# software-mansion/smelter

Hardware: NVIDIA H100
Metric: 4K composited frames/sec (16-input grid) per GPU (higher is better)
Workload: dtype f32 math on u8 planes (f16 resampler scratch)

## Files before the change

### include/smelter_b200.h

```cpp
#ifndef SMELTER_B200_H
#define SMELTER_B200_H

#include <stddef.h>
#include <stdint.h>

#ifdef __cplusplus
extern "C" {
#endif

typedef struct smr_renderer smr_renderer;

typedef enum {
    SMR_OK = 0,
    SMR_ERR_INVALID_ARGUMENT = 1,
    SMR_ERR_CUDA = 2,
    SMR_ERR_OUTPUT_NOT_REGISTERED = 3,
    SMR_ERR_SCENE = 4,
    SMR_ERR_UNSUPPORTED = 5,
    SMR_ERR_OUT_OF_MEMORY = 6,
    SMR_ERR_BUFFER_TOO_SMALL = 7
} smr_status;

typedef enum { SMR_MODE_GPU_OPTIMIZED = 0, SMR_MODE_CPU_OPTIMIZED = 1 } smr_rendering_mode;

typedef struct {
    int32_t cuda_device;
    int32_t rendering_mode;
    uint32_t max_layouts_count;
    uint64_t stream_fallback_timeout_ns;
    uint32_t framerate_num, framerate_den;
} smr_options;

typedef enum {
    SMR_COMPONENT_INPUT_STREAM = 0,
    SMR_COMPONENT_VIEW = 1,
    SMR_COMPONENT_TILES = 2,
    SMR_COMPONENT_RESCALER = 3,
    SMR_COMPONENT_SHADER = 4,
    SMR_COMPONENT_WEB_VIEW = 5,
    SMR_COMPONENT_IMAGE = 6,
    SMR_COMPONENT_TEXT = 7
} smr_component_type;

typedef struct { uint8_t r, g, b, a; } smr_rgba;
typedef struct { float top_left, top_right, bottom_right, bottom_left; } smr_border_radius;
typedef struct { float offset_x, offset_y, blur_radius; smr_rgba color; } smr_box_shadow;
typedef struct { float top, right, bottom, left; } smr_padding;
typedef struct { int32_t has_value; float value; } smr_opt_f32;

typedef enum { SMR_INTERP_LINEAR = 0, SMR_INTERP_BOUNCE = 1, SMR_INTERP_CUBIC_BEZIER = 2 } smr_interpolation_kind;
typedef struct {
    int32_t present;
    uint64_t duration_ns;
    int32_t interpolation_kind;
    double x1, y1, x2, y2;
    int32_t should_interrupt;
} smr_transition;

typedef struct {
    int32_t is_absolute;
    smr_opt_f32 width, height;
    int32_t horizontal_from_right; float horizontal_offset;
    int32_t vertical_from_bottom; float vertical_offset;
    float rotation_degrees;
} smr_position;

typedef enum { SMR_DIRECTION_ROW = 0, SMR_DIRECTION_COLUMN = 1 } smr_direction;
typedef enum { SMR_OVERFLOW_VISIBLE = 0, SMR_OVERFLOW_HIDDEN = 1, SMR_OVERFLOW_FIT = 2 } smr_overflow;
typedef enum { SMR_RESCALE_FIT = 0, SMR_RESCALE_FILL = 1 } smr_rescale_mode;
typedef enum { SMR_HALIGN_LEFT = 0, SMR_HALIGN_RIGHT = 1, SMR_HALIGN_JUSTIFIED = 2, SMR_HALIGN_CENTER = 3 } smr_horizontal_align;
typedef enum { SMR_VALIGN_TOP = 0, SMR_VALIGN_CENTER = 1, SMR_VALIGN_BOTTOM = 2, SMR_VALIGN_JUSTIFIED = 3 } smr_vertical_align;

typedef struct smr_component {
    int32_t type;
    const char *id;
    const struct smr_component *children;
    uint32_t children_len;
    const char *input_id;

    smr_position position;
    smr_transition transition;
    smr_border_radius border_radius;
    float border_width;
    smr_rgba border_color;
    const smr_box_shadow *box_shadow;
    uint32_t box_shadow_len;

    int32_t direction;
    int32_t overflow;
    smr_rgba background_color;
    smr_padding padding;

    int32_t rescale_mode;
    int32_t horizontal_align;
    int32_t vertical_align;

    smr_opt_f32 tiles_width, tiles_height;
    uint32_t tile_aspect_ratio_w, tile_aspect_ratio_h;
    float tiles_margin, tiles_padding;
} smr_component;

typedef enum {
    SMR_FRAME_PLANAR_YUV420 = 0,
    SMR_FRAME_PLANAR_YUVJ420 = 1,
    SMR_FRAME_NV12 = 2,
    SMR_FRAME_BGRA = 3,
    SMR_FRAME_ARGB = 4,
    SMR_FRAME_RGBA8 = 5,
    SMR_FRAME_PLANAR_YUV422 = 6,
    SMR_FRAME_PLANAR_YUV444 = 7,
    SMR_FRAME_UYVY422 = 8,
    SMR_FRAME_YUYV422 = 9
} smr_frame_format;

typedef enum { SMR_MEM_HOST = 0, SMR_MEM_DEVICE = 1 } smr_mem_kind;

typedef struct {
    const char *input_id;
    int32_t format;
    uint32_t width, height;
    uint64_t pts_ns;
    const void *planes[3];
    uint32_t pitch[3];
    int32_t mem_kind;
} smr_input_frame;

typedef enum {
    SMR_OUT_PLANAR_YUV420 = 0,
    SMR_OUT_PLANAR_YUV422 = 1,
    SMR_OUT_PLANAR_YUV444 = 2,
    SMR_OUT_RGBA8 = 3,
    SMR_OUT_NV12 = 4
} smr_output_format;

typedef struct {
    const char *output_id;
    void *planes[3];
    uint32_t pitch[3];
    int32_t mem_kind;
    uint32_t width, height;
    int32_t format;
    uint64_t pts_ns;
} smr_output_frame;

#define SMR_MAX_MASKS 20
typedef struct { float radius[4]; float top, left, width, height; } smr_mask;
typedef struct {
    int32_t type;
    float top, left, width, height, rotation_degrees;
    float border_radius[4];
    smr_rgba color, border_color;
    float border_width, blur_radius;
    int32_t child_index;
    float crop_top, crop_left, crop_width, crop_height;
    int32_t masks_len;
    smr_mask masks[SMR_MAX_MASKS];
} smr_render_layout;

typedef struct {
    uint64_t frames_rendered;
    uint64_t kernel_launches;
    uint64_t h2d_bytes, d2h_bytes;
    uint64_t last_render_kernel_launches;
    uint64_t last_render_direct_tiles;
} smr_stats;

typedef enum {
    SMR_KERNEL_CONVERT = 0,
    SMR_KERNEL_WEIGHTS = 1,
    SMR_KERNEL_RESAMPLE_BOX = 2,
    SMR_KERNEL_RESAMPLE_FIRST = 3,
    SMR_KERNEL_RESAMPLE_LAST = 4,
    SMR_KERNEL_COMPOSITE = 5,
    SMR_KERNEL_OUTPUT = 6,
    SMR_KERNEL_FILL = 7,
    SMR_KERNEL_RESAMPLE_FUSED = 8,
    SMR_KERNEL_CLASSES = 9
} smr_kernel_class;
typedef struct {
    double total_ms[SMR_KERNEL_CLASSES];
    uint64_t launches[SMR_KERNEL_CLASSES];
} smr_kernel_times;

smr_status smr_create(const smr_options *opts, smr_renderer **out);
void smr_destroy(smr_renderer *r);

smr_status smr_register_input(smr_renderer *r, const char *input_id);
smr_status smr_unregister_input(smr_renderer *r, const char *input_id);

smr_status smr_update_scene(smr_renderer *r, const char *output_id, uint32_t width, uint32_t height,
                            int32_t output_format, const smr_component *scene_root);
smr_status smr_unregister_output(smr_renderer *r, const char *output_id);

smr_status smr_render(smr_renderer *r, uint64_t pts_ns, const smr_input_frame *inputs, uint32_t n_inputs,
                      smr_output_frame *outputs, uint32_t n_outputs);

#define SMR_TICKS_IN_FLIGHT 4
smr_status smr_render_begin(smr_renderer *r, uint64_t pts_ns, const smr_input_frame *inputs, uint32_t n_inputs,
                            smr_output_frame *outputs, uint32_t n_outputs);
smr_status smr_render_end(smr_renderer *r);

smr_status smr_preprocess_frame(smr_renderer *r, const smr_input_frame *frame, uint32_t out_width, uint32_t out_height,
                                void *rgba, uint32_t pitch, int32_t mem_kind);

smr_status smr_premultiply_rgba8(smr_renderer *r, const smr_input_frame *frame, void *rgba, uint32_t pitch, int32_t mem_kind);

typedef enum { SMR_GLYPH_COLOR = 0, SMR_GLYPH_MASK = 1 } smr_glyph_content;
typedef struct {
    int32_t x, y;
    uint16_t width, height;
    uint16_t atlas_x, atlas_y;
    smr_rgba color;
    int32_t content;
} smr_glyph;
typedef struct { const void *data; uint32_t width, height, pitch; } smr_atlas;
smr_status smr_render_text(smr_renderer *r, uint32_t width, uint32_t height, smr_rgba background, const smr_glyph *glyphs,
                           uint32_t n_glyphs, const smr_atlas *mask_atlas, const smr_atlas *color_atlas, int32_t color_mode,
                           void *rgba, uint32_t pitch, int32_t mem_kind);

smr_status smr_debug_partition(const int32_t *dst_w, const int32_t *dst_h, uint32_t n_jobs, uint32_t max_blocks,
                               int32_t *pieces, uint32_t pieces_cap, uint32_t *n_pieces, int32_t *begin,
                               uint32_t begin_cap, uint32_t *n_blocks);

smr_status smr_debug_tile_plan(const int32_t *boxes, uint32_t n_layers, uint32_t width, uint32_t height, int32_t sorted,
                               int32_t *owner_layer, uint32_t owner_cap, uint32_t *tiles, uint32_t tiles_cap, uint32_t *n_tiles);

smr_status smr_output_plane_sizes(uint32_t width, uint32_t height, int32_t output_format, size_t sizes[3]);

void smr_component_default(int32_t type, smr_component *out);

smr_status smr_debug_layouts(smr_renderer *r, const char *output_id, uint64_t pts_ns,
                             smr_render_layout *out, uint32_t capacity, uint32_t *n_out,
                             uint32_t *root_width, uint32_t *root_height);

smr_status smr_set_layouts(smr_renderer *r, const char *output_id, uint32_t width, uint32_t height, int32_t format,
                           uint32_t root_width, uint32_t root_height, const char *const *child_ids, uint32_t n_children,
                           const smr_render_layout *layouts, uint32_t n_layouts);

smr_status smr_debug_set_inputs(smr_renderer *r, uint64_t pts_ns, const smr_input_frame *inputs, uint32_t n_inputs);

smr_status smr_comm_get_unique_id(uint8_t id[128]);
smr_status smr_comm_init(smr_renderer *r, const uint8_t id[128], int32_t rank, int32_t nranks);
#define SMR_COMM_POOLED 1u
smr_status smr_comm_broadcast_inputs(smr_renderer *r, const smr_input_frame *frames, uint32_t n,
                                     const int32_t *root_ranks);
smr_status smr_comm_exchange_inputs(smr_renderer *r, const smr_input_frame *frames, uint32_t n, const int32_t *root_ranks,
                                    const uint64_t *consumer_masks, uint32_t flags);
#define SMR_COMM_PEER_DIRECT 2u
smr_status smr_peer_pool_alloc(smr_renderer *r, size_t bytes, void **dev_ptr, uint8_t handle[64]);
smr_status smr_peer_pool_open(smr_renderer *r, const uint8_t handle[64], void **dev_ptr);
smr_status smr_peer_pool_close(smr_renderer *r, void *dev_ptr);
smr_status smr_peer_pool_free(smr_renderer *r, void *dev_ptr);
smr_status smr_comm_pull_inputs(smr_renderer *r, const smr_input_frame *frames, const smr_input_frame *peer_frames, uint32_t n,
                                const int32_t *root_ranks, const uint64_t *consumer_masks);
smr_status smr_comm_destroy(smr_renderer *r);

smr_status smr_host_register(void *ptr, size_t bytes);
smr_status smr_host_unregister(void *ptr);

smr_status smr_get_stats(smr_renderer *r, smr_stats *out);
smr_status smr_set_profiling(smr_renderer *r, int32_t enabled);
smr_status smr_get_kernel_times(smr_renderer *r, smr_kernel_times *out);
void *smr_cuda_stream(smr_renderer *r);
const char *smr_last_error(smr_renderer *r);
const char *smr_version(void);

#ifdef __cplusplus
}
#endif
#endif
```

### smelter_b200/_ffi.py

```python
import ctypes as C
import os

_HERE = os.path.dirname(os.path.abspath(__file__))
LIB_PATH = os.environ.get("SMR_LIB_PATH") or os.path.join(_HERE, "libsmelter_b200.so")

SMR_OK = 0
STATUS_NAMES = {0: "SMR_OK", 1: "SMR_ERR_INVALID_ARGUMENT", 2: "SMR_ERR_CUDA", 3: "SMR_ERR_OUTPUT_NOT_REGISTERED",
                4: "SMR_ERR_SCENE", 5: "SMR_ERR_UNSUPPORTED", 6: "SMR_ERR_OUT_OF_MEMORY", 7: "SMR_ERR_BUFFER_TOO_SMALL"}

MODE_GPU_OPTIMIZED, MODE_CPU_OPTIMIZED = 0, 1
COMPONENT_INPUT_STREAM, COMPONENT_VIEW, COMPONENT_TILES, COMPONENT_RESCALER = 0, 1, 2, 3
COMPONENT_SHADER, COMPONENT_WEB_VIEW, COMPONENT_IMAGE, COMPONENT_TEXT = 4, 5, 6, 7
FRAME_PLANAR_YUV420, FRAME_PLANAR_YUVJ420, FRAME_NV12, FRAME_BGRA, FRAME_ARGB, FRAME_RGBA8 = 0, 1, 2, 3, 4, 5
FRAME_PLANAR_YUV422, FRAME_PLANAR_YUV444, FRAME_UYVY422, FRAME_YUYV422 = 6, 7, 8, 9
MEM_HOST, MEM_DEVICE = 0, 1
OUT_PLANAR_YUV420, OUT_PLANAR_YUV422, OUT_PLANAR_YUV444, OUT_RGBA8, OUT_NV12 = 0, 1, 2, 3, 4
MAX_MASKS = 20


class Options(C.Structure):
    _fields_ = [("cuda_device", C.c_int32), ("rendering_mode", C.c_int32), ("max_layouts_count", C.c_uint32),
                ("stream_fallback_timeout_ns", C.c_uint64), ("framerate_num", C.c_uint32), ("framerate_den", C.c_uint32)]


class Rgba(C.Structure):
    _fields_ = [("r", C.c_uint8), ("g", C.c_uint8), ("b", C.c_uint8), ("a", C.c_uint8)]


class BorderRadius(C.Structure):
    _fields_ = [("top_left", C.c_float), ("top_right", C.c_float), ("bottom_right", C.c_float), ("bottom_left", C.c_float)]


class BoxShadow(C.Structure):
    _fields_ = [("offset_x", C.c_float), ("offset_y", C.c_float), ("blur_radius", C.c_float), ("color", Rgba)]


class Padding(C.Structure):
    _fields_ = [("top", C.c_float), ("right", C.c_float), ("bottom", C.c_float), ("left", C.c_float)]


class OptF32(C.Structure):
    _fields_ = [("has_value", C.c_int32), ("value", C.c_float)]


class Transition(C.Structure):
    _fields_ = [("present", C.c_int32), ("duration_ns", C.c_uint64), ("interpolation_kind", C.c_int32),
                ("x1", C.c_double), ("y1", C.c_double), ("x2", C.c_double), ("y2", C.c_double),
                ("should_interrupt", C.c_int32)]


class Position(C.Structure):
    _fields_ = [("is_absolute", C.c_int32), ("width", OptF32), ("height", OptF32),
                ("horizontal_from_right", C.c_int32), ("horizontal_offset", C.c_float),
                ("vertical_from_bottom", C.c_int32), ("vertical_offset", C.c_float),
                ("rotation_degrees", C.c_float)]


class Component(C.Structure):
    pass


Component._fields_ = [
    ("type", C.c_int32), ("id", C.c_char_p), ("children", C.POINTER(Component)), ("children_len", C.c_uint32),
    ("input_id", C.c_char_p),
    ("position", Position), ("transition", Transition), ("border_radius", BorderRadius),
    ("border_width", C.c_float), ("border_color", Rgba), ("box_shadow", C.POINTER(BoxShadow)),
    ("box_shadow_len", C.c_uint32),
    ("direction", C.c_int32), ("overflow", C.c_int32), ("background_color", Rgba), ("padding", Padding),
    ("rescale_mode", C.c_int32), ("horizontal_align", C.c_int32), ("vertical_align", C.c_int32),
    ("tiles_width", OptF32), ("tiles_height", OptF32),
    ("tile_aspect_ratio_w", C.c_uint32), ("tile_aspect_ratio_h", C.c_uint32),
    ("tiles_margin", C.c_float), ("tiles_padding", C.c_float),
]


class InputFrame(C.Structure):
    _fields_ = [("input_id", C.c_char_p), ("format", C.c_int32), ("width", C.c_uint32), ("height", C.c_uint32),
                ("pts_ns", C.c_uint64), ("planes", C.c_void_p * 3), ("pitch", C.c_uint32 * 3), ("mem_kind", C.c_int32)]


class OutputFrame(C.Structure):
    _fields_ = [("output_id", C.c_char_p), ("planes", C.c_void_p * 3), ("pitch", C.c_uint32 * 3),
                ("mem_kind", C.c_int32), ("width", C.c_uint32), ("height", C.c_uint32), ("format", C.c_int32),
                ("pts_ns", C.c_uint64)]


class Mask(C.Structure):
    _fields_ = [("radius", C.c_float * 4), ("top", C.c_float), ("left", C.c_float), ("width", C.c_float),
                ("height", C.c_float)]


class RenderLayout(C.Structure):
    _fields_ = [("type", C.c_int32), ("top", C.c_float), ("left", C.c_float), ("width", C.c_float),
                ("height", C.c_float), ("rotation_degrees", C.c_float), ("border_radius", C.c_float * 4),
                ("color", Rgba), ("border_color", Rgba), ("border_width", C.c_float), ("blur_radius", C.c_float),
                ("child_index", C.c_int32), ("crop_top", C.c_float), ("crop_left", C.c_float),
                ("crop_width", C.c_float), ("crop_height", C.c_float), ("masks_len", C.c_int32),
                ("masks", Mask * MAX_MASKS)]


class Atlas(C.Structure):
    _fields_ = [("data", C.c_void_p), ("width", C.c_uint32), ("height", C.c_uint32), ("pitch", C.c_uint32)]


GLYPH_COLOR, GLYPH_MASK = 0, 1
GLYPH_DTYPE = [("x", "<i4"), ("y", "<i4"), ("width", "<u2"), ("height", "<u2"), ("atlas_x", "<u2"), ("atlas_y", "<u2"),
               ("color", "u1", (4,)), ("content", "<i4")]


class Stats(C.Structure):
    _fields_ = [("frames_rendered", C.c_uint64), ("kernel_launches", C.c_uint64), ("h2d_bytes", C.c_uint64),
                ("d2h_bytes", C.c_uint64), ("last_render_kernel_launches", C.c_uint64), ("last_render_direct_tiles", C.c_uint64)]


KERNEL_CLASSES = ["convert", "weights", "resample_box", "resample_first", "resample_last", "composite", "output",
                  "fill", "resample_fused"]


class KernelTimes(C.Structure):
    _fields_ = [("total_ms", C.c_double * 9), ("launches", C.c_uint64 * 9)]


EXPORTS = [
    "smr_create", "smr_destroy", "smr_register_input", "smr_unregister_input", "smr_update_scene",
    "smr_unregister_output", "smr_set_layouts", "smr_render", "smr_render_begin", "smr_render_end", "smr_preprocess_frame", "smr_premultiply_rgba8", "smr_render_text", "smr_debug_partition", "smr_debug_tile_plan", "smr_output_plane_sizes",
    "smr_component_default", "smr_debug_layouts", "smr_debug_set_inputs", "smr_get_stats", "smr_set_profiling", "smr_get_kernel_times",
    "smr_comm_get_unique_id", "smr_comm_init", "smr_comm_broadcast_inputs", "smr_comm_exchange_inputs", "smr_comm_pull_inputs", "smr_peer_pool_alloc", "smr_peer_pool_open", "smr_peer_pool_close", "smr_peer_pool_free", "smr_comm_destroy", "smr_host_register", "smr_host_unregister", "smr_cuda_stream", "smr_last_error",
    "smr_version",
]

_lib = None


def lib():
    global _lib
    if _lib is not None:
        return _lib
    if not os.path.exists(LIB_PATH):
        raise ImportError(
            f"{LIB_PATH} is missing: build it with `python -m smelter_b200.build` "
            "(the H100 compositor has no CPU fallback)")
    L = C.CDLL(LIB_PATH)
    vp = C.c_void_p
    L.smr_create.argtypes = [C.POINTER(Options), C.POINTER(vp)]
    L.smr_destroy.argtypes = [vp]
    L.smr_destroy.restype = None
    L.smr_register_input.argtypes = [vp, C.c_char_p]
    L.smr_unregister_input.argtypes = [vp, C.c_char_p]
    L.smr_update_scene.argtypes = [vp, C.c_char_p, C.c_uint32, C.c_uint32, C.c_int32, C.POINTER(Component)]
    L.smr_unregister_output.argtypes = [vp, C.c_char_p]
    for f in (L.smr_render, L.smr_render_begin):
        f.argtypes = [vp, C.c_uint64, C.POINTER(InputFrame), C.c_uint32, C.POINTER(OutputFrame), C.c_uint32]
    L.smr_render_end.argtypes = [vp]
    L.smr_preprocess_frame.argtypes = [vp, C.POINTER(InputFrame), C.c_uint32, C.c_uint32, C.c_void_p, C.c_uint32, C.c_int32]
    L.smr_preprocess_frame.restype = C.c_int32
    L.smr_premultiply_rgba8.argtypes = [vp, C.POINTER(InputFrame), C.c_void_p, C.c_uint32, C.c_int32]
    L.smr_premultiply_rgba8.restype = C.c_int32
    L.smr_render_text.argtypes = [vp, C.c_uint32, C.c_uint32, Rgba, C.c_void_p, C.c_uint32, C.POINTER(Atlas), C.POINTER(Atlas),
                                  C.c_int32, C.c_void_p, C.c_uint32, C.c_int32]
    L.smr_render_text.restype = C.c_int32
    L.smr_debug_partition.argtypes = [C.POINTER(C.c_int32), C.POINTER(C.c_int32), C.c_uint32, C.c_uint32, C.POINTER(C.c_int32),
                                      C.c_uint32, C.POINTER(C.c_uint32), C.POINTER(C.c_int32), C.c_uint32, C.POINTER(C.c_uint32)]
    L.smr_debug_partition.restype = C.c_int32
    L.smr_debug_tile_plan.argtypes = [C.POINTER(C.c_int32), C.c_uint32, C.c_uint32, C.c_uint32, C.c_int32, C.POINTER(C.c_int32), C.c_uint32,
                                      C.POINTER(C.c_uint32), C.c_uint32, C.POINTER(C.c_uint32)]
    L.smr_debug_tile_plan.restype = C.c_int32
    L.smr_output_plane_sizes.argtypes = [C.c_uint32, C.c_uint32, C.c_int32, C.POINTER(C.c_size_t * 3)]
    L.smr_component_default.argtypes = [C.c_int32, C.POINTER(Component)]
    L.smr_component_default.restype = None
    L.smr_debug_layouts.argtypes = [vp, C.c_char_p, C.c_uint64, C.POINTER(RenderLayout), C.c_uint32,
                                    C.POINTER(C.c_uint32), C.POINTER(C.c_uint32), C.POINTER(C.c_uint32)]
    L.smr_debug_set_inputs.argtypes = [vp, C.c_uint64, C.POINTER(InputFrame), C.c_uint32]
    L.smr_get_stats.argtypes = [vp, C.POINTER(Stats)]
    L.smr_comm_get_unique_id.argtypes = [C.POINTER(C.c_uint8 * 128)]
    L.smr_comm_init.argtypes = [vp, C.POINTER(C.c_uint8 * 128), C.c_int32, C.c_int32]
    L.smr_comm_broadcast_inputs.argtypes = [vp, C.POINTER(InputFrame), C.c_uint32, C.POINTER(C.c_int32)]
    L.smr_set_layouts.argtypes = [vp, C.c_char_p, C.c_uint32, C.c_uint32, C.c_int32, C.c_uint32, C.c_uint32,
                                  C.POINTER(C.c_char_p), C.c_uint32, C.POINTER(RenderLayout), C.c_uint32]
    L.smr_host_register.argtypes = [C.c_void_p, C.c_size_t]
    L.smr_host_unregister.argtypes = [C.c_void_p]
    L.smr_comm_exchange_inputs.argtypes = [vp, C.POINTER(InputFrame), C.c_uint32, C.POINTER(C.c_int32), C.POINTER(C.c_uint64),
                                           C.c_uint32]
    L.smr_comm_pull_inputs.argtypes = [vp, C.POINTER(InputFrame), C.POINTER(InputFrame), C.c_uint32, C.POINTER(C.c_int32),
                                       C.POINTER(C.c_uint64)]
    L.smr_peer_pool_alloc.argtypes = [vp, C.c_size_t, C.POINTER(C.c_void_p), C.POINTER(C.c_uint8 * 64)]
    L.smr_peer_pool_open.argtypes = [vp, C.POINTER(C.c_uint8 * 64), C.POINTER(C.c_void_p)]
    L.smr_peer_pool_close.argtypes = [vp, C.c_void_p]
    L.smr_peer_pool_free.argtypes = [vp, C.c_void_p]
    L.smr_comm_destroy.argtypes = [vp]
    L.smr_set_profiling.argtypes = [vp, C.c_int32]
    L.smr_get_kernel_times.argtypes = [vp, C.POINTER(KernelTimes)]
    L.smr_cuda_stream.argtypes = [vp]
    L.smr_cuda_stream.restype = vp
    L.smr_last_error.argtypes = [vp]
    L.smr_last_error.restype = C.c_char_p
    L.smr_version.restype = C.c_char_p
    _lib = L
    return L
```

### smelter_b200/build.py

```python
import os
import subprocess
import sys

HERE = os.path.dirname(os.path.abspath(__file__))
CSRC = os.path.join(HERE, "csrc")
LIB = os.path.join(HERE, "libsmelter_b200.so")
SOURCES = ["kernels.cu", "renderer.cpp", "scene.cpp"]
HEADERS = ["kernels.h", "scene.h", "ptx_helpers.cuh", "resample_tma.cuh", "resample_tma3.cuh", "resample_tma0.cuh", os.path.join("..", "..", "include", "smelter_b200.h")]

NVCC_FLAGS = [
    "-std=c++17", "-O3",
    "-gencode", "arch=compute_90a,code=sm_90a",
    "-lineinfo",
    "-fmad=false",
    "-prec-div=true", "-prec-sqrt=true", "-ftz=false",
    "-Xcompiler", "-fPIC,-ffp-contract=off,-Wall",
    "-ccbin", "/usr/bin/g++",
    "-shared",
]


def needs_build():
    if not os.path.exists(LIB):
        return True
    t = os.path.getmtime(LIB)
    deps = [os.path.join(CSRC, s) for s in SOURCES + HEADERS] + [os.path.abspath(__file__)]
    return any(os.path.getmtime(d) > t for d in deps)


def build(force=False, verbose=False, extra=()):
    if not force and not needs_build():
        return LIB
    nvcc = os.environ.get("NVCC", "/usr/local/cuda/bin/nvcc")
    cmd = [nvcc] + NVCC_FLAGS + list(extra) + ["-o", LIB] + [os.path.join(CSRC, s) for s in SOURCES]
    if verbose:
        print(" ".join(cmd))
    subprocess.check_call(cmd)
    return LIB


if __name__ == "__main__":
    build(force=True, verbose=True, extra=sys.argv[1:])
    print(LIB)
```

### smelter_b200/csrc/kernels.cu

```cuda
#include <cuda_fp16.h>
#include <cuda_runtime.h>

#include <cstdio>
#include <cstdlib>
#include <atomic>
#include <cstring>

#include "kernels.h"

namespace smr {
namespace dev {

#include "ptx_helpers.cuh"

__device__ float c_u8n[256];
__device__ float c_dec[256];
__device__ float c_thr[256];
#define ENC_KEY0 ((127 - 13) << 5)
#define ENC_KEYS ((13 << 5) + 1)
__device__ unsigned char c_enc0[420];
__device__ float c_yl[256];
#define ENC1_KEY0 ((127 - 13) << 8)
#define ENC1_KEYS ((13 << 8) + 1)
__device__ unsigned char c_enc1[ENC1_KEYS + 3];

static thread_local char g_err[256] = {0};
const char *last_launch_error() { return g_err; }
static bool check_launch(const char *what) {
    cudaError_t e = cudaGetLastError();
    if (e != cudaSuccess) {
        snprintf(g_err, sizeof(g_err), "%s: %s", what, cudaGetErrorString(e));
        return false;
    }
    return true;
}

void upload_tables(const float *u8n, const float *dec, const float *thr) {
    float t[256];
    for (int i = 0; i < 255; i++) t[i] = thr[i];
    t[255] = 3.0e38f;
    cudaMemcpyToSymbol(c_u8n, u8n, sizeof(float) * 256);
    cudaMemcpyToSymbol(c_dec, dec, sizeof(float) * 256);
    cudaMemcpyToSymbol(c_thr, t, sizeof(float) * 256);
    float yl[256];
    for (int i = 0; i < 256; i++) {
        volatile float d = u8n[i] - (16.0f / 255.0f);
        volatile float m = d * (1.0f / 0.85882352941f);
        yl[i] = m < 0.0f ? 0.0f : (m > 1.0f ? 1.0f : m);
    }
    cudaMemcpyToSymbol(c_yl, yl, sizeof(float) * 256);
    unsigned char enc0[420] = {0};
    for (int k = 0; k < ENC_KEYS; k++) {
        const uint32_t bits = (uint32_t)(k + ENC_KEY0) << 18;
        float lo;
        memcpy(&lo, &bits, 4);
        int e = 0;
        while (e < 255 && lo >= t[e]) e++;
        enc0[k] = (unsigned char)e;
    }
    cudaMemcpyToSymbol(c_enc0, enc0, sizeof(enc0));
    static unsigned char enc1[ENC1_KEYS + 3];
    for (int k = 0; k < ENC1_KEYS; k++) {
        const uint32_t bits = (uint32_t)(k + ENC1_KEY0) << 15;
        float lo;
        memcpy(&lo, &bits, 4);
        int e = 0;
        while (e < 255 && lo >= t[e]) e++;
        enc1[k] = (unsigned char)e;
        if (k > 0 && enc1[k] - enc1[k - 1] > 1) {
            fprintf(stderr, "smelter_b200: sRGB encode bucket table is too coarse at key %d\n", k);
            abort();
        }
    }
    cudaMemcpyToSymbol(c_enc1, enc1, sizeof(enc1));
}

struct Tables {
    float u8n[256];
    float dec[256];
    float thr[256];
    float yl[256];
};

__device__ __forceinline__ void load_tables(Tables &t) {
    for (int i = threadIdx.y * blockDim.x + threadIdx.x; i < 256; i += blockDim.x * blockDim.y) {
        t.u8n[i] = c_u8n[i];
        t.dec[i] = c_dec[i];
        t.thr[i] = c_thr[i];
        t.yl[i] = c_yl[i];
    }
    __syncthreads();
}

__device__ __forceinline__ float clamp01(float x) { return __saturatef(x); }

__device__ __forceinline__ int unorm8(float x) { return __float2int_rn(clamp01(x) * 255.0f); }

__device__ __forceinline__ int srgb_encode(const Tables &t, float lin) {
    const float x = clamp01(lin);
    const int k = max((__float_as_int(x) >> 15) - ENC1_KEY0, 0);
    const int e = __ldg(c_enc1 + k);
    return e + (x >= t.thr[e] ? 1 : 0);
}

struct LinTap {
    int i0, i1;
    float f;
};

__device__ __forceinline__ LinTap linear_tap(float t, int dim) {
    LinTap r;
    float c = t * (float)dim - 0.5f;
    if (!(c == c)) { r.i0 = r.i1 = 0; r.f = 0.0f; return r; }
    c = fminf(fmaxf(c, -2.0f), (float)dim + 1.0f);
    float fl = floorf(c);
    float f = c - fl;
    r.f = rintf(f * 256.0f) * (1.0f / 256.0f);
    int i0 = (int)fl, i1 = i0 + 1;
    r.i0 = min(max(i0, 0), dim - 1);
    r.i1 = min(max(i1, 0), dim - 1);
    return r;
}

__device__ __forceinline__ float bilerp(float t00, float t10, float t01, float t11, float fx, float fy) {
    float h0 = fmaf(t10, fx, t00 * (1.0f - fx));
    float h1 = fmaf(t11, fx, t01 * (1.0f - fx));
    return fmaf(h1, fy, h0 * (1.0f - fy));
}

__device__ __forceinline__ float div255(float nf, float pow2) {
    const float c = __uint_as_float(0x3b808081u) * pow2, lo = __uint_as_float(0xaf7efeffu) * pow2;
    return fmaf(nf, c, nf * lo);
}
__device__ __forceinline__ float filter_u8(int t00, int t10, int t01, int t11, float fx, float fy) {
    const int wx = (int)(fx * 256.0f), wy = (int)(fy * 256.0f);
    const int n = (t00 * (256 - wx) + t10 * wx) * (256 - wy) + (t01 * (256 - wx) + t11 * wx) * wy;
    return div255((float)n, 1.0f / 65536.0f);
}

__device__ __forceinline__ float sample_plane(const Tables &T, const uint8_t *p, int pitch, int stride, int ch,
                                              const LinTap &ax, const LinTap &ay) {
    const uint8_t *r0 = p + (size_t)ay.i0 * pitch, *r1 = p + (size_t)ay.i1 * pitch;
    const int t00 = __ldg(r0 + ax.i0 * stride + ch), t10 = __ldg(r0 + ax.i1 * stride + ch);
    const int t01 = __ldg(r1 + ax.i0 * stride + ch), t11 = __ldg(r1 + ax.i1 * stride + ch);
    return filter_u8(t00, t10, t01, t11, ax.f, ay.f);
}

#define K16 (16.0f / 255.0f)
#define RCP_Y (1.0f / 0.85882352941f)
#define RCP_C (1.0f / 0.87843137254f)

__device__ __forceinline__ uchar4 yuv_to_rgba8(float y, float u, float v, int full_range) {
    if (!full_range) {
        y = clamp01((y - K16) * RCP_Y);
        u = clamp01((u - K16) * RCP_C);
        v = clamp01((v - K16) * RCP_C);
    }
    float um = u - 0.5f, vm = v - 0.5f;
    float r = fmaf(1.5748f, vm, y);
    float g = fmaf(-0.4681f, vm, fmaf(-0.1873f, um, y));
    float b = fmaf(1.8556f, um, y);
    return make_uchar4((unsigned char)unorm8(r), (unsigned char)unorm8(g), (unsigned char)unorm8(b), 255);
}

__device__ __forceinline__ void yuv_to_rgb8i(float y, float u, float v, int full_range, int &r8, int &g8, int &b8) {
    if (!full_range) {
        y = clamp01((y - K16) * RCP_Y);
        u = clamp01((u - K16) * RCP_C);
        v = clamp01((v - K16) * RCP_C);
    }
    float um = u - 0.5f, vm = v - 0.5f;
    r8 = unorm8(fmaf(1.5748f, vm, y));
    g8 = unorm8(fmaf(-0.4681f, vm, fmaf(-0.1873f, um, y)));
    b8 = unorm8(fmaf(1.8556f, um, y));
}

__device__ __forceinline__ void yuv_to_rgb8n(float yn, float u, float v, int full_range, int &r8, int &g8, int &b8) {
    if (!full_range) {
        u = clamp01((u - K16) * RCP_C);
        v = clamp01((v - K16) * RCP_C);
    }
    float um = u - 0.5f, vm = v - 0.5f;
    r8 = unorm8(fmaf(1.5748f, vm, yn));
    g8 = unorm8(fmaf(-0.4681f, vm, fmaf(-0.1873f, um, yn)));
    b8 = unorm8(fmaf(1.8556f, um, yn));
}

__device__ __forceinline__ uchar4 node_texel(const Tables &T, const Tex &s, int x, int y) {
    switch (s.kind) {
        case TEX_RGBA8:
            return __ldg(reinterpret_cast<const uchar4 *>(s.p0 + (size_t)y * s.pitch0) + x);
        case TEX_BGRA: {
            uchar4 v = __ldg(reinterpret_cast<const uchar4 *>(s.p0 + (size_t)y * s.pitch0) + x);
            return make_uchar4(v.z, v.y, v.x, v.w);
        }
        case TEX_ARGB: {
            uchar4 v = __ldg(reinterpret_cast<const uchar4 *>(s.p0 + (size_t)y * s.pitch0) + x);
            return make_uchar4(v.y, v.z, v.w, v.x);
        }
        case TEX_YUV420:
        case TEX_NV12: {
            int cw = s.width / 2, ch = s.height / 2;
            if (((s.width | s.height) & 1) == 0) {
                int x0 = (x & 1) ? (x >> 1) : max((x >> 1) - 1, 0), x1 = (x & 1) ? min((x >> 1) + 1, cw - 1) : (x >> 1);
                int y0 = (y & 1) ? (y >> 1) : max((y >> 1) - 1, 0), y1 = (y & 1) ? min((y >> 1) + 1, ch - 1) : (y >> 1);
                const int kx = (x & 1) ? 1 : 3, ky = (y & 1) ? 1 : 3;
                float yy = T.u8n[__ldg(s.p0 + (size_t)y * s.pitch0 + x)];
                int nu, nv;
                if (s.kind == TEX_YUV420) {
                    const uint8_t *u0 = s.p1 + (size_t)y0 * s.pitch1, *u1 = s.p1 + (size_t)y1 * s.pitch1;
                    const uint8_t *v0 = s.p2 + (size_t)y0 * s.pitch2, *v1 = s.p2 + (size_t)y1 * s.pitch2;
                    nu = ((int)__ldg(u0 + x0) * (4 - kx) + (int)__ldg(u0 + x1) * kx) * (4 - ky) +
                         ((int)__ldg(u1 + x0) * (4 - kx) + (int)__ldg(u1 + x1) * kx) * ky;
                    nv = ((int)__ldg(v0 + x0) * (4 - kx) + (int)__ldg(v0 + x1) * kx) * (4 - ky) +
                         ((int)__ldg(v1 + x0) * (4 - kx) + (int)__ldg(v1 + x1) * kx) * ky;
                } else {
                    const uchar2 *r0 = reinterpret_cast<const uchar2 *>(s.p1 + (size_t)y0 * s.pitch1);
                    const uchar2 *r1 = reinterpret_cast<const uchar2 *>(s.p1 + (size_t)y1 * s.pitch1);
                    uchar2 a = __ldg(r0 + x0), b = __ldg(r0 + x1), c = __ldg(r1 + x0), d = __ldg(r1 + x1);
                    nu = ((int)a.x * (4 - kx) + (int)b.x * kx) * (4 - ky) + ((int)c.x * (4 - kx) + (int)d.x * kx) * ky;
                    nv = ((int)a.y * (4 - kx) + (int)b.y * kx) * (4 - ky) + ((int)c.y * (4 - kx) + (int)d.y * kx) * ky;
                }
                const float uu = div255((float)nu, 0.0625f), vv = div255((float)nv, 0.0625f);
                return yuv_to_rgba8(yy, uu, vv, s.full_range);
            }
            float tx = ((float)x + 0.5f) / (float)s.width, ty = ((float)y + 0.5f) / (float)s.height;
            LinTap ax = linear_tap(tx, s.width), ay = linear_tap(ty, s.height);
            LinTap cx = linear_tap(tx, cw), cy = linear_tap(ty, ch);
            float yy = sample_plane(T, s.p0, s.pitch0, 1, 0, ax, ay);
            float uu, vv;
            if (s.kind == TEX_YUV420) {
                uu = sample_plane(T, s.p1, s.pitch1, 1, 0, cx, cy);
                vv = sample_plane(T, s.p2, s.pitch2, 1, 0, cx, cy);
            } else {
                uu = sample_plane(T, s.p1, s.pitch1, 2, 0, cx, cy);
                vv = sample_plane(T, s.p1, s.pitch1, 2, 1, cx, cy);
            }
            return yuv_to_rgba8(yy, uu, vv, s.full_range);
        }
        case TEX_YUV422:
        case TEX_YUV444: {
            const int cw = s.kind == TEX_YUV444 ? s.width : s.width / 2, ch = s.height;
            float tx = ((float)x + 0.5f) / (float)s.width, ty = ((float)y + 0.5f) / (float)s.height;
            LinTap ax = linear_tap(tx, s.width), ay = linear_tap(ty, s.height);
            LinTap cx = linear_tap(tx, cw), cy = linear_tap(ty, ch);
            float yy = sample_plane(T, s.p0, s.pitch0, 1, 0, ax, ay);
            float uu = sample_plane(T, s.p1, s.pitch1, 1, 0, cx, cy);
            float vv = sample_plane(T, s.p2, s.pitch2, 1, 0, cx, cy);
            return yuv_to_rgba8(yy, uu, vv, 0);
        }
        case TEX_UYVY:
        case TEX_YUYV: {
            const int dimx = s.width / 2;
            const float eps = 0.0001f, hpw = 0.5f / (float)dimx;
            float tx = ((float)x + 0.5f) / (float)s.width, ty = ((float)y + 0.5f) / (float)s.height;
            float xf = ((tx * (float)dimx - hpw) + eps) * 2.0f;
            unsigned x_pos = xf >= 4294967296.0f ? 0xffffffffu : (xf > 0.0f ? (unsigned)xf : 0u);
            float tcx = (float)(x_pos / 2u) / (float)dimx + hpw;
            LinTap ax = linear_tap(tcx, dimx), ay = linear_tap(ty, s.height);
            float t[4];
#pragma unroll
            for (int c = 0; c < 4; c++) t[c] = sample_plane(T, s.p0, s.pitch0, 4, c, ax, ay);
            const bool second = x_pos & 1u;
            if (s.kind == TEX_YUYV) return yuv_to_rgba8(second ? t[2] : t[0], t[1], t[3], 0);
            return yuv_to_rgba8(second ? t[3] : t[1], t[0], t[2], 0);
        }
        default:
            return make_uchar4(0, 0, 0, 0);
    }
}

__device__ __forceinline__ bool yuv_quad_ok(const Tex &s, int x, int y) {
    return (s.kind == TEX_NV12 || s.kind == TEX_YUV420) && (((s.width | s.height | x | y) & 1) == 0) && x >= 2 &&
           x + 3 <= s.width - 1 && y >= 2 && y + 3 <= s.height - 1;
}
__device__ __forceinline__ void yuv_quad(const Tables &T, const Tex &s, int x, int y, uchar4 &p00, uchar4 &p10,
                                         uchar4 &p01, uchar4 &p11) {
    const int cx = x >> 1, cy = y >> 1;
    unsigned he[3], ho[3];
#pragma unroll
    for (int i = 0; i < 3; i++) {
        unsigned a, b, d;
        if (s.kind == TEX_NV12) {
            const uchar2 *rp = reinterpret_cast<const uchar2 *>(s.p1 + (size_t)(cy - 1 + i) * s.pitch1) + cx;
            const uchar2 ta = __ldg(rp - 1), tb = __ldg(rp), td = __ldg(rp + 1);
            a = ta.x | (ta.y << 16); b = tb.x | (tb.y << 16); d = td.x | (td.y << 16);
        } else {
            const uint8_t *ru = s.p1 + (size_t)(cy - 1 + i) * s.pitch1 + cx, *rv = s.p2 + (size_t)(cy - 1 + i) * s.pitch2 + cx;
            a = __ldg(ru - 1) | (__ldg(rv - 1) << 16); b = __ldg(ru) | (__ldg(rv) << 16); d = __ldg(ru + 1) | (__ldg(rv + 1) << 16);
        }
        he[i] = a + 3u * b;
        ho[i] = 3u * b + d;
    }
    const uchar2 y0 = __ldg(reinterpret_cast<const uchar2 *>(s.p0 + (size_t)y * s.pitch0 + x));
    const uchar2 y1 = __ldg(reinterpret_cast<const uchar2 *>(s.p0 + (size_t)(y + 1) * s.pitch0 + x));
    const unsigned n00 = he[0] + 3u * he[1], n10 = ho[0] + 3u * ho[1], n01 = 3u * he[1] + he[2], n11 = 3u * ho[1] + ho[2];
    p00 = yuv_to_rgba8(T.u8n[y0.x], div255((float)(n00 & 0xffffu), 0.0625f), div255((float)(n00 >> 16), 0.0625f), s.full_range);
    p10 = yuv_to_rgba8(T.u8n[y0.y], div255((float)(n10 & 0xffffu), 0.0625f), div255((float)(n10 >> 16), 0.0625f), s.full_range);
    p01 = yuv_to_rgba8(T.u8n[y1.x], div255((float)(n01 & 0xffffu), 0.0625f), div255((float)(n01 >> 16), 0.0625f), s.full_range);
    p11 = yuv_to_rgba8(T.u8n[y1.y], div255((float)(n11 & 0xffffu), 0.0625f), div255((float)(n11 >> 16), 0.0625f), s.full_range);
}

__global__ void __launch_bounds__(256) k_convert(Tex src, uint8_t *dst, int dst_pitch) {
    __shared__ Tables T;
    load_tables(T);
    int x = blockIdx.x * blockDim.x + threadIdx.x, y = blockIdx.y * blockDim.y + threadIdx.y;
    if (x >= src.width || y >= src.height) return;
    reinterpret_cast<uchar4 *>(dst + (size_t)y * dst_pitch)[x] = node_texel(T, src, x, y);
}

int launch_convert_to_rgba(const Tex &src, uint8_t *dst, int dst_pitch, Stream s) {
    dim3 b(32, 8), g((src.width + 31) / 32, (src.height + 7) / 8);
    k_convert<<<g, b, 0, (cudaStream_t)s>>>(src, dst, dst_pitch);
    return check_launch("k_convert") ? 1 : -1;
}

#define PI_F 3.14159265359f

__device__ __forceinline__ float sin_cr(float x) { return (float)sin((double)x); }
__device__ __forceinline__ float cos_cr(float x) { return (float)cos((double)x); }

__global__ void k_weights(const WeightJob *jobs) {
    const WeightJob J = jobs[blockIdx.y];
    int o = blockIdx.x * blockDim.x + threadIdx.x;
    if (o >= J.n_out) return;
    float kernel_scale = fmaxf(J.scale, 1.0f);
    float inv_k = 1.0f / kernel_scale;
    float support = 3.0f * kernel_scale;
    float center = (J.offset + ((float)o + 0.5f) * J.scale) - 0.5f;
    float first = ceilf(center - support);
    float x0 = (first - center) * inv_k;
    float s1 = sin_cr(PI_F * x0), c1 = cos_cr(PI_F * x0);
    float s3 = sin_cr(PI_F * x0 / 3.0f), c3 = cos_cr(PI_F * x0 / 3.0f);
    float sd1 = sin_cr(PI_F * inv_k), cd1 = cos_cr(PI_F * inv_k);
    float sd3 = sin_cr(PI_F * inv_k / 3.0f), cd3 = cos_cr(PI_F * inv_k / 3.0f);
    const float pi2 = PI_F * PI_F;
    float wsum = 0.0f;
    float *w = J.weights + (size_t)o * J.taps;
    for (int t = 0; t < J.taps; t++) {
        float x = x0 + (float)t * inv_k;
        float wt = 0.0f;
        if (fabsf(x) < 1e-5f) wt = 1.0f;
        else if (fabsf(x) < 3.0f) wt = ((3.0f * s1) * s3) / ((pi2 * x) * x);
        w[t] = wt;
        wsum += wt;
        float ns1 = s1 * cd1 + c1 * sd1;
        c1 = c1 * cd1 - s1 * sd1;
        s1 = ns1;
        float ns3 = s3 * cd3 + c3 * sd3;
        c3 = c3 * cd3 - s3 * sd3;
        s3 = ns3;
    }
    J.inv_wsum[o] = 1.0f / wsum;
    float fc = fminf(fmaxf(first, -1.0e9f), 1.0e9f);
    J.first[o] = (int)fc;
}

int launch_weights(const WeightJob *jobs_dev, const WeightJob *jobs_host, int n, Stream s) {
    if (n <= 0) return 0;
    int max_out = 1;
    for (int i = 0; i < n; i++) max_out = jobs_host[i].n_out > max_out ? jobs_host[i].n_out : max_out;
    dim3 b(128), g((max_out + 127) / 128, n);
    k_weights<<<g, b, 0, (cudaStream_t)s>>>(jobs_dev);
    return check_launch("k_weights") ? 1 : -1;
}

__device__ __forceinline__ float4 rs_load(const Tables &T, const Tex &s, int x, int y) {
    if (s.kind == TEX_F16) {
        const uint2 raw = __ldg(reinterpret_cast<const uint2 *>(s.p0 + (size_t)y * s.pitch0) + x);
        __half2 a = *reinterpret_cast<const __half2 *>(&raw.x), b = *reinterpret_cast<const __half2 *>(&raw.y);
        float2 fa = __half22float2(a), fb = __half22float2(b);
        return make_float4(fa.x, fa.y, fb.x, fb.y);
    }
    uchar4 p = node_texel(T, s, x, y);
    return make_float4(T.dec[p.x], T.dec[p.y], T.dec[p.z], T.u8n[p.w]);
}

__device__ __forceinline__ void rs_store(const Tables &T, const ResampleJob &J, int x, int y, float4 r) {
    if (J.dst_f16) {
        __half2 a = __floats2half2_rn(r.x, r.y), b = __floats2half2_rn(r.z, r.w);
        uint2 raw;
        raw.x = *reinterpret_cast<unsigned int *>(&a);
        raw.y = *reinterpret_cast<unsigned int *>(&b);
        reinterpret_cast<uint2 *>(J.dst + (size_t)y * J.dst_pitch)[x] = raw;
    } else {
        uchar4 o = make_uchar4((unsigned char)srgb_encode(T, r.x), (unsigned char)srgb_encode(T, r.y),
                               (unsigned char)srgb_encode(T, r.z), (unsigned char)unorm8(r.w));
        reinterpret_cast<uchar4 *>(J.dst + (size_t)y * J.dst_pitch)[x] = o;
    }
}

__global__ void __launch_bounds__(256) k_resample(const ResampleJob *jobs) {
    __shared__ Tables T;
    load_tables(T);
    const ResampleJob &J = jobs[blockIdx.z];
    int px = blockIdx.x * blockDim.x + threadIdx.x, py = blockIdx.y * blockDim.y + threadIdx.y;
    if (px >= J.dst_w || py >= J.dst_h) return;
    const Tex &S = J.src;
    if (J.box_fx * J.box_fy > 1) {
        float4 sum = make_float4(0.f, 0.f, 0.f, 0.f);
        for (int dy = 0; dy < J.box_fy; dy++)
            for (int dx = 0; dx < J.box_fx; dx++) {
                int sx = min(px * J.box_fx + dx, S.width - 1), sy = min(py * J.box_fy + dy, S.height - 1);
                float4 t = rs_load(T, S, sx, sy);
                sum.x += t.x; sum.y += t.y; sum.z += t.z; sum.w += t.w;
            }
        float d = (float)((unsigned)J.box_fx * (unsigned)J.box_fy);
        rs_store(T, J, px, py, make_float4(sum.x / d, sum.y / d, sum.z / d, sum.w / d));
        return;
    }
    int o = J.axis == 1 ? py : px;
    int max_src = (J.axis == 1 ? S.height : S.width) - 1;
    int max_perp = (J.axis == 1 ? S.width : S.height) - 1;
    int perp = min(max((J.axis == 1 ? px : py) + J.perp_offset, 0), max_perp);
    const float *w = J.weights + (size_t)o * J.taps;
    int first = __ldg(J.first + o);
    float4 sum = make_float4(0.f, 0.f, 0.f, 0.f);
    for (int t = 0; t < J.taps; t++) {
        float wt = __ldg(w + t);
        if (wt == 0.0f) continue;
        int src = min(max(first + t, 0), max_src);
        float4 tx = J.axis == 1 ? rs_load(T, S, perp, src) : rs_load(T, S, src, perp);
        sum.x = fmaf(tx.x, wt, sum.x);
        sum.y = fmaf(tx.y, wt, sum.y);
        sum.z = fmaf(tx.z, wt, sum.z);
        sum.w = fmaf(tx.w, wt, sum.w);
    }
    float inv = __ldg(J.inv_wsum + o);
    rs_store(T, J, px, py, make_float4(sum.x * inv, sum.y * inv, sum.z * inv, sum.w * inv));
}

int launch_resample(const ResampleJob *jobs_dev, const ResampleJob *jobs_host, int n, Stream s) {
    if (n <= 0) return 0;
    int mw = 1, mh = 1;
    for (int i = 0; i < n; i++) {
        mw = jobs_host[i].dst_w > mw ? jobs_host[i].dst_w : mw;
        mh = jobs_host[i].dst_h > mh ? jobs_host[i].dst_h : mh;
    }
    dim3 b(32, 8), g((mw + 31) / 32, (mh + 7) / 8, n);
    k_resample<<<g, b, 0, (cudaStream_t)s>>>(jobs_dev);
    return check_launch("k_resample") ? 1 : -1;
}

#define W64_TW 64
#define W64_WARPS 8
#define W64_RING 64

__constant__ float c_wint[5][32];
__constant__ float c_winv[5];
__constant__ float2 c_wpair[5][32];

void set_int_weights(int S, const float *weights_dev, const float *inv_dev, int taps, Stream s) {
    cudaMemcpyToSymbolAsync(c_wint, weights_dev, sizeof(float) * taps, sizeof(float) * 32 * S, cudaMemcpyDeviceToDevice, (cudaStream_t)s);
    cudaMemcpyToSymbolAsync(c_winv, inv_dev, sizeof(float), sizeof(float) * S, cudaMemcpyDeviceToDevice, (cudaStream_t)s);
    float *pair = nullptr;
    cudaGetSymbolAddress((void **)&pair, c_wpair);
    pair += 2 * 32 * S;
    cudaMemsetAsync(pair, 0, sizeof(float2) * 32, (cudaStream_t)s);
    cudaMemcpy2DAsync(pair, sizeof(float2), weights_dev, sizeof(float), sizeof(float), taps, cudaMemcpyDeviceToDevice, (cudaStream_t)s);
    if (taps > S)
        cudaMemcpy2DAsync(pair + 2 * S + 1, sizeof(float2), weights_dev, sizeof(float), sizeof(float), taps - S,
                          cudaMemcpyDeviceToDevice, (cudaStream_t)s);
}

template <int S>
struct W64 {
    static constexpr int SS = S == 0 ? 4 : S;
    static constexpr int TAPS = 6 * SS + 1;
    static constexpr int SPAN = (W64_TW - 1) * SS + TAPS + 3;
    static constexpr int ROWLEN = S == 0 ? ((SPAN + 2 + 7) & ~7) : (((SPAN + SPAN / (2 * SS) + 2) + 7) & ~7);
    struct Smem {
        Tables T;
        __half2 ring[W64_RING][3][W64_TW / 2];
        float4 srow[W64_WARPS][ROWLEN];
        float hw[S == 0 ? TAPS * W64_TW : 1];
    };
    static __device__ __forceinline__ int pos(int i) { return S == 0 ? i : i + i / (2 * SS); }
};

__device__ __forceinline__ void prefetch_l2_span(const uint8_t *p, int bytes, const uint8_t *lo, const uint8_t *hi) {
    unsigned long long a = (unsigned long long)(p < lo ? lo : p), e = (unsigned long long)(p + bytes < hi ? p + bytes : hi);
    a = (a + 15ull) & ~15ull;
    if (e <= a + 16ull) return;
    const unsigned size = (unsigned)((e - a) & ~15ull);
    asm volatile("cp.async.bulk.prefetch.L2.global [%0], %1;" ::"l"(a), "r"(size) : "memory");
}

template <int S, int SRC>
__global__ void __launch_bounds__(32 * W64_WARPS, 3) k_resample_fused_int(const FusedJob *jobs, const FusedPiece *pieces,
                                                                            const int *piece_begin) {
    constexpr bool NV12 = SRC == 1, IL = SRC >= 2;
    using K = W64<S>;
    constexpr int TAPS = K::TAPS;
    constexpr int WIN = S + TAPS;
    extern __shared__ __align__(16) unsigned char fs_raw[];
    typename K::Smem &M = *reinterpret_cast<typename K::Smem *>(fs_raw);
    load_tables(M.T);
    const int lane = threadIdx.x, warp = threadIdx.y;
    for (int pi = __ldg(piece_begin + blockIdx.x); pi < __ldg(piece_begin + blockIdx.x + 1); pi++) {
    const FusedPiece P = pieces[pi];
    const FusedJob &J = jobs[P.job];
    const int th = S == 0 ? J.taps_h : TAPS;
    const int ox0 = P.strip * W64_TW;
    const int oy_begin = P.oy_begin, oy_end = P.oy_end;
    const Tex &src = J.src;
    const int W = src.width, H = src.height, chei = H >> 1;
    const int tv = J.taps_v;
    const int xa = __ldg(J.first_h + ox0);
    const int xa_e = xa & ~1;
    const int d0 = xa - xa_e;
    const int oc0 = min(ox0 + 2 * lane, J.dst_w - 1), oc1 = min(ox0 + 2 * lane + 1, J.dst_w - 1);
    int gi0 = 0, gD = 0, npairs_g = 0;
    float inv0, inv1;
    if constexpr (S == 0) {
        const int f0 = __ldg(J.first_h + oc0), f1 = __ldg(J.first_h + oc1);
        gi0 = f0 - xa_e; gD = f1 - f0;
        inv0 = __ldg(J.inv_h + oc0); inv1 = __ldg(J.inv_h + oc1);
        const int o_last = min(ox0 + W64_TW - 1, J.dst_w - 1);
        npairs_g = (min(__ldg(J.first_h + o_last) + th - xa_e, K::SPAN) + 1) >> 1;
        for (int t = warp; t < th; t += W64_WARPS) {
            M.hw[t * W64_TW + 2 * lane] = __ldg(J.w_h + (size_t)oc0 * th + t);
            M.hw[t * W64_TW + 2 * lane + 1] = __ldg(J.w_h + (size_t)oc1 * th + t);
        }
        __syncthreads();
    } else {
        inv0 = inv1 = c_winv[S];
    }
    constexpr int NP = ((W64_TW - 1) * K::SS + TAPS + 2) >> 1, NIT = (NP + 31) / 32;
    const int npairs = S == 0 ? npairs_g : NP;
    const int full_range = src.full_range;
    const float *ytab = full_range ? M.T.u8n : M.T.yl;
    const int p_in_lo = IL ? (xa_e >= 0 ? 0 : (1 - xa_e) >> 1) : (xa_e >= 2 ? 0 : (2 - xa_e + 1) >> 1);
    const int p_in_hi = IL ? (W - 2 - xa_e) >> 1 : (W - 4 - xa_e) >> 1;
    const int p_hi = min(p_in_hi, npairs - 1);
    const int dsh = S == 0 ? 0 : d0;

    int produced_hi = -0x40000000;
    for (int o0 = oy_begin; o0 < oy_end; o0 += W64_WARPS) {
        const int o_l = min(o0 + W64_WARPS - 1, oy_end - 1);
        const int need_lo = min(max(__ldg(J.first_v + o0), 0), H - 1);
        const int need_hi = min(max(__ldg(J.first_v + o_l) + tv - 1, 0), H - 1);
        const int start = max(produced_hi + 1, need_lo);
        {
            const int tid = warp * 32 + lane;
            const int nr = need_hi + 1 + (tid >> 2), part = tid & 3;
            if (tid < 128 && nr < H) {
                const int xb = max(xa_e - 2, 0), span = K::SPAN + 4;
                if (IL) {
                    if (part == 0) prefetch_l2_span(src.p0 + (size_t)nr * src.pitch0 + 2 * xb, 2 * span, src.p0, src.p0 + (size_t)H * src.pitch0);
                } else if (part == 0) {
                    prefetch_l2_span(src.p0 + (size_t)nr * src.pitch0 + xb, span, src.p0, src.p0 + (size_t)H * src.pitch0);
                } else if ((nr & 1) == 0) {
                    const int cyn = min(nr >> 1, chei - 1);
                    if (NV12) {
                        if (part == 1) prefetch_l2_span(src.p1 + (size_t)cyn * src.pitch1 + xb, span, src.p1, src.p1 + (size_t)chei * src.pitch1);
                    } else if (part == 1) {
                        prefetch_l2_span(src.p1 + (size_t)cyn * src.pitch1 + (xb >> 1), span >> 1, src.p1, src.p1 + (size_t)chei * src.pitch1);
                    } else if (part == 2) {
                        prefetch_l2_span(src.p2 + (size_t)cyn * src.pitch2 + (xb >> 1), span >> 1, src.p2, src.p2 + (size_t)chei * src.pitch2);
                    }
                }
            }
        }
        for (int r = start + warp; r <= need_hi; r += W64_WARPS) {
            float4 *row = M.srow[warp];
            {
                const uint8_t *yrow = src.p0 + (size_t)r * src.pitch0;
                const int cy0 = (r & 1) ? (r >> 1) : max((r >> 1) - 1, 0), cy1 = (r & 1) ? min((r >> 1) + 1, chei - 1) : (r >> 1);
                const uint8_t *c0a = IL ? nullptr : src.p1 + (size_t)cy0 * src.pitch1, *c1a = IL ? nullptr : src.p1 + (size_t)cy1 * src.pitch1;
                const uint8_t *c0b = (NV12 || IL) ? nullptr : src.p2 + (size_t)cy0 * src.pitch2;
                const uint8_t *c1b = (NV12 || IL) ? nullptr : src.p2 + (size_t)cy1 * src.pitch2;
                const bool odd = r & 1;
                struct Raw { unsigned y, a0, b0, d0, a1, b1, d1; };
                auto load_raw = [&](int pp, Raw &R) {
                    const int x = xa_e + 2 * pp, cx = x >> 1;
                    if (IL) {
                        R.y = __ldg(reinterpret_cast<const unsigned int *>(yrow) + cx);
                        return;
                    }
                    if (NV12) {
                        const unsigned short *r0 = reinterpret_cast<const unsigned short *>(c0a) + cx;
                        const unsigned short *r1 = reinterpret_cast<const unsigned short *>(c1a) + cx;
                        R.a0 = __ldg(r0 - 1); R.b0 = __ldg(r0); R.d0 = __ldg(r0 + 1);
                        R.a1 = __ldg(r1 - 1); R.b1 = __ldg(r1); R.d1 = __ldg(r1 + 1);
                    } else {
                        R.a0 = __ldg(c0a + cx - 1) | ((unsigned)__ldg(c0b + cx - 1) << 16);
                        R.b0 = __ldg(c0a + cx) | ((unsigned)__ldg(c0b + cx) << 16);
                        R.d0 = __ldg(c0a + cx + 1) | ((unsigned)__ldg(c0b + cx + 1) << 16);
                        R.a1 = __ldg(c1a + cx - 1) | ((unsigned)__ldg(c1b + cx - 1) << 16);
                        R.b1 = __ldg(c1a + cx) | ((unsigned)__ldg(c1b + cx) << 16);
                        R.d1 = __ldg(c1a + cx + 1) | ((unsigned)__ldg(c1b + cx + 1) << 16);
                    }
                    R.y = __ldg(reinterpret_cast<const unsigned short *>(yrow + x));
                };
                auto spread = [&](unsigned c) { return NV12 ? __byte_perm(c, 0, 0x4140) : c; };
                auto put = [&](int i, int r8, int g8, int b8) {
                    row[K::pos(i)] = make_float4(M.T.dec[r8], M.T.dec[g8], M.T.dec[b8], 0.0f);
                };
                auto convert_store = [&](const Raw &R, int p) {
                    if constexpr (IL) {
                        const unsigned t = R.y;
                        const unsigned ub = SRC == 2 ? (t & 0xffu) : ((t >> 8) & 0xffu), vb = SRC == 2 ? ((t >> 16) & 0xffu) : (t >> 24);
                        const unsigned y0 = SRC == 2 ? ((t >> 8) & 0xffu) : (t & 0xffu), y1 = SRC == 2 ? (t >> 24) : ((t >> 16) & 0xffu);
                        const float u = M.T.u8n[ub], v = M.T.u8n[vb];
                        const int i = 2 * p - dsh;
                        int r8, g8, b8;
                        yuv_to_rgb8n(M.T.yl[y0], u, v, 0, r8, g8, b8);
                        if (i >= 0) put(i, r8, g8, b8);
                        yuv_to_rgb8n(M.T.yl[y1], u, v, 0, r8, g8, b8);
                        put(i + 1, r8, g8, b8);
                        return;
                    }
                    const unsigned a0 = spread(R.a0), b0 = 3u * spread(R.b0), e0 = spread(R.d0);
                    const unsigned a1 = spread(R.a1), b1 = 3u * spread(R.b1), e1 = spread(R.d1);
                    const unsigned he0 = a0 + b0, ho0 = b0 + e0, he1 = a1 + b1, ho1 = b1 + e1;
                    const unsigned ne = odd ? 3u * he0 + he1 : he0 + 3u * he1;
                    const unsigned no = odd ? 3u * ho0 + ho1 : ho0 + 3u * ho1;
                    const float ue = div255((float)(ne & 0xffffu), 0.0625f), ve = div255((float)(ne >> 16), 0.0625f);
                    const float uo = div255((float)(no & 0xffffu), 0.0625f), vo = div255((float)(no >> 16), 0.0625f);
                    const int i = 2 * p - dsh;
                    int r8, g8, b8;
                    auto luma = [&](unsigned yb) {
                        const float yn = div255((float)yb, 1.0f);
                        return full_range ? yn : clamp01((yn - K16) * RCP_Y);
                    };
                    yuv_to_rgb8n(luma(R.y & 0xffu), ue, ve, full_range, r8, g8, b8);
                    if (i >= 0) put(i, r8, g8, b8);
                    yuv_to_rgb8n(luma(R.y >> 8), uo, vo, full_range, r8, g8, b8);
                    put(i + 1, r8, g8, b8);
                };
                auto inside = [&](int pp) { return pp >= p_in_lo && pp <= p_hi; };
                auto border = [&](int p) {
                    const int x = xa_e + 2 * p, i = 2 * p - dsh;
                    const uchar4 pe = node_texel(M.T, src, min(max(x, 0), W - 1), r);
                    const uchar4 po = node_texel(M.T, src, min(max(x + 1, 0), W - 1), r);
                    if (i >= 0) put(i, pe.x, pe.y, pe.z);
                    put(i + 1, po.x, po.y, po.z);
                };
                Raw cur, nxt;
                bool ok = inside(lane);
                if (ok) load_raw(lane, cur);
                if constexpr (S != 0) {
#pragma unroll
                    for (int it = 0; it < NIT; it++) {
                        const int p = lane + 32 * it;
                        const bool ok_n = it + 1 < NIT && inside(p + 32);
                        if (ok_n) load_raw(p + 32, nxt);
                        if (ok) convert_store(cur, p);
                        cur = nxt; ok = ok_n;
                    }
                } else {
                    for (int p = lane; p < npairs; p += 32) {
                        const bool ok_n = inside(p + 32);
                        if (ok_n) load_raw(p + 32, nxt);
                        if (ok) convert_store(cur, p);
                        cur = nxt; ok = ok_n;
                    }
                }
                if (p_in_lo > 0 || p_hi < npairs - 1)
                    for (int p = lane; p < npairs; p += 32)
                        if (!inside(p)) border(p);
            }
            __syncwarp();
            {
                __half2 *ringrow = &M.ring[r & (W64_RING - 1)][0][0];
                float r0 = 0.f, g0 = 0.f, b0 = 0.f, r1 = 0.f, g1 = 0.f, b1 = 0.f;
                if constexpr (S == 0) {
                    const float *w0 = M.hw + 2 * lane, *w1 = M.hw + 2 * lane + 1 - gD * W64_TW;
                    const int win = th + gD;
                    const float4 *sp = row + gi0;
#pragma unroll 4
                    for (int j = 0; j < win; j++) {
                        const float4 v = sp[j];
                        if (j < th) { const float w = w0[j * W64_TW]; r0 = fmaf(v.x, w, r0); g0 = fmaf(v.y, w, g0); b0 = fmaf(v.z, w, b0); }
                        if (j >= gD) { const float w = w1[j * W64_TW]; r1 = fmaf(v.x, w, r1); g1 = fmaf(v.y, w, g1); b1 = fmaf(v.z, w, b1); }
                    }
                } else {
                    const float4 *sp = row + (2 * S + 1) * lane;
#pragma unroll
                    for (int j = 0; j < WIN; j++) {
                        const float4 v = sp[K::pos(j)];
                        if (j < TAPS) { const float w = c_wint[S][j]; r0 = fmaf(v.x, w, r0); g0 = fmaf(v.y, w, g0); b0 = fmaf(v.z, w, b0); }
                        if (j >= S) { const float w = c_wint[S][j - S]; r1 = fmaf(v.x, w, r1); g1 = fmaf(v.y, w, g1); b1 = fmaf(v.z, w, b1); }
                    }
                }
                ringrow[lane] = __floats2half2_rn(r0 * inv0, r1 * inv1);
                ringrow[W64_TW / 2 + lane] = __floats2half2_rn(g0 * inv0, g1 * inv1);
                ringrow[W64_TW + lane] = __floats2half2_rn(b0 * inv0, b1 * inv1);
            }
            __syncwarp();
        }
        produced_hi = max(produced_hi, need_hi);
        __syncthreads();
        const int oy = o0 + warp;
        if (oy < oy_end) {
            const int fv = __ldg(J.first_v + oy);
            const float *wv = J.w_v + (size_t)oy * tv;
            float r0 = 0.f, g0 = 0.f, b0 = 0.f, r1 = 0.f, g1 = 0.f, b1 = 0.f;
            const bool inside = fv >= 0 && fv + tv - 1 <= H - 1;
            for (int t = 0; t < tv; t++) {
                const float wt = __ldg(wv + t);
                const int row = inside ? fv + t : min(max(fv + t, 0), H - 1);
                const __half2 *p = &M.ring[row & (W64_RING - 1)][0][0];
                const float2 vr = __half22float2(p[lane]), vg = __half22float2(p[W64_TW / 2 + lane]), vb = __half22float2(p[W64_TW + lane]);
                r0 = fmaf(vr.x, wt, r0); r1 = fmaf(vr.y, wt, r1);
                g0 = fmaf(vg.x, wt, g0); g1 = fmaf(vg.y, wt, g1);
                b0 = fmaf(vb.x, wt, b0); b1 = fmaf(vb.y, wt, b1);
            }
            const float inv_v = __ldg(J.inv_v + oy);
            const int ox = ox0 + 2 * lane;
            uchar4 oa = make_uchar4((unsigned char)srgb_encode(M.T, r0 * inv_v), (unsigned char)srgb_encode(M.T, g0 * inv_v),
                                    (unsigned char)srgb_encode(M.T, b0 * inv_v), 255);
            uchar4 ob = make_uchar4((unsigned char)srgb_encode(M.T, r1 * inv_v), (unsigned char)srgb_encode(M.T, g1 * inv_v),
                                    (unsigned char)srgb_encode(M.T, b1 * inv_v), 255);
            uchar4 *drow = reinterpret_cast<uchar4 *>(J.dst + (size_t)oy * J.dst_pitch);
            if (ox + 1 < J.dst_w && (J.dst_pitch & 7) == 0) {
                uint2 pk;
                pk.x = *reinterpret_cast<unsigned int *>(&oa);
                pk.y = *reinterpret_cast<unsigned int *>(&ob);
                *reinterpret_cast<uint2 *>(drow + ox) = pk;
            } else {
                if (ox < J.dst_w) drow[ox] = oa;
                if (ox + 1 < J.dst_w) drow[ox + 1] = ob;
            }
        }
        __syncthreads();
    }
    }
}

template <int S, int SRC>
static bool launch_fused_int(const FusedJob *jobs_dev, const FusedPiece *pieces, const int *piece_begin, int nblocks,
                             cudaStream_t s) {
    static std::atomic<unsigned long long> done{0};
    int dev = 0;
    cudaGetDevice(&dev);
    const unsigned long long bit = 1ull << (dev & 63);
    if (!(done.load(std::memory_order_acquire) & bit)) {
        cudaFuncSetAttribute(k_resample_fused_int<S, SRC>, cudaFuncAttributeMaxDynamicSharedMemorySize,
                             (int)sizeof(typename W64<S>::Smem));
        done.fetch_or(bit, std::memory_order_release);
    }
    k_resample_fused_int<S, SRC><<<nblocks, dim3(32, W64_WARPS), sizeof(typename W64<S>::Smem), s>>>(jobs_dev, pieces, piece_begin);
    return check_launch("k_resample_fused_int");
}

template <int S>
static bool launch_fused_src(int src, const FusedJob *jobs_dev, const FusedPiece *pieces_dev, const int *piece_begin_dev,
                             int nblocks, cudaStream_t st) {
    switch (src) {
        case 0: return launch_fused_int<S, 0>(jobs_dev, pieces_dev, piece_begin_dev, nblocks, st);
        case 1: return launch_fused_int<S, 1>(jobs_dev, pieces_dev, piece_begin_dev, nblocks, st);
        case 2: return launch_fused_int<S, 2>(jobs_dev, pieces_dev, piece_begin_dev, nblocks, st);
        default: return launch_fused_int<S, 3>(jobs_dev, pieces_dev, piece_begin_dev, nblocks, st);
    }
}

}
}
namespace smr {
namespace dev {
__device__ __forceinline__ float to_y(float r, float g, float b) {
    float y = fmaf(b, 0.0722f, fmaf(g, 0.7152f, r * 0.2126f));
    return fmaf(y, 0.85882352941f, K16);
}
__device__ __forceinline__ float to_u(float r, float g, float b) {
    float u = fmaf(b, 0.5f, fmaf(g, -0.3854f, r * -0.1146f));
    return fmaf(u + 0.5f, 0.87843137254f, K16);
}
__device__ __forceinline__ float to_v(float r, float g, float b) {
    float v = fmaf(b, -0.0458f, fmaf(g, -0.4542f, r * 0.5f));
    return fmaf(v + 0.5f, 0.87843137254f, K16);
}

__device__ __forceinline__ void emit_yuv_2x2(const FusedJob &J, int X, int Y, uint32_t p00, uint32_t p10, uint32_t p01, uint32_t p11) {
    using namespace tma;
    const float2 m23 = splat(-8388608.0f);
    const float2 c = splat(__uint_as_float(0x3b808081u)), lo = splat(__uint_as_float(0xaf7efeffu));
    auto pairf = [&](uint32_t a, uint32_t b, uint32_t sel) {
        return add2(make_float2(__uint_as_float(__byte_perm(a, 0x4B000000u, sel)), __uint_as_float(__byte_perm(b, 0x4B000000u, sel))), m23);
    };
    auto unit = [&](float2 n) { return fma2(n, c, mul2(n, lo)); };
    auto store2 = [&](float2 x01) -> uint32_t {
        const float2 q = add2_after_mul(mul2(x01, splat(255.0f)), splat(12582912.0f));
        return (__float_as_uint(q.x) & 0xffu) | ((__float_as_uint(q.y) & 0xffu) << 8);
    };
    auto lum2 = [&](uint32_t a, uint32_t b) -> uint32_t {
        const float2 r = unit(pairf(a, b, 0x7540u)), g = unit(pairf(a, b, 0x7541u)), bl = unit(pairf(a, b, 0x7542u));
        const float2 y = fma2(bl, splat(0.0722f), fma2(g, splat(0.7152f), mul2(r, splat(0.2126f))));
        return store2(make_float2(__saturatef(fmaf(y.x, 0.85882352941f, K16)), __saturatef(fmaf(y.y, 0.85882352941f, K16))));
    };
    *reinterpret_cast<unsigned short *>(J.out0 + (size_t)Y * J.out_pitch0 + X) = (unsigned short)lum2(p00, p10);
    *reinterpret_cast<unsigned short *>(J.out0 + (size_t)(Y + 1) * J.out_pitch0 + X) = (unsigned short)lum2(p01, p11);
    const uint32_t m = 0x00ff00ffu;
    const uint32_t srb = (p00 & m) + (p10 & m) + (p01 & m) + (p11 & m);
    const uint32_t sga = ((p00 >> 8) & m) + ((p10 >> 8) & m) + ((p01 >> 8) & m) + ((p11 >> 8) & m);
    const float2 c4 = splat(__uint_as_float(0x3b808081u) * 0.25f), lo4 = splat(__uint_as_float(0xaf7efeffu) * 0.25f);
    const float2 nrg = add2(make_float2(__uint_as_float(__byte_perm(srb, 0x4B000000u, 0x7610u)), __uint_as_float(__byte_perm(sga, 0x4B000000u, 0x7610u))), m23);
    const float nb = __uint_as_float(__byte_perm(srb, 0x4B000000u, 0x7632u)) - 8388608.0f;
    const float2 rg = fma2(nrg, c4, mul2(nrg, lo4));
    const float b = fmaf(nb, c4.x, nb * lo4.x);
    float2 uv = mul2(splat(rg.x), make_float2(-0.1146f, 0.5f));
    uv = fma2(splat(rg.y), make_float2(-0.3854f, -0.4542f), uv);
    uv = fma2(splat(b), make_float2(0.5f, -0.0458f), uv);
    uv = add2(uv, splat(0.5f));
    const uint32_t cuv = store2(make_float2(__saturatef(fmaf(uv.x, 0.87843137254f, K16)), __saturatef(fmaf(uv.y, 0.87843137254f, K16))));
    if (J.out_format == 4) {
        *reinterpret_cast<unsigned short *>(J.out1 + (size_t)(Y >> 1) * J.out_pitch1 + X) = (unsigned short)cuv;
    } else {
        J.out1[(size_t)(Y >> 1) * J.out_pitch1 + (X >> 1)] = (unsigned char)(cuv & 0xffu);
        J.out2[(size_t)(Y >> 1) * J.out_pitch2 + (X >> 1)] = (unsigned char)(cuv >> 8);
    }
}

#include "resample_tma.cuh"
#include "resample_tma3.cuh"
#include "resample_tma0.cuh"

template <int SRC, int WINP, int BOX>
static bool launch_tma0(const FusedJob *jobs_dev, const FusedPiece *pieces, const int *piece_begin, int nblocks, cudaStream_t s) {
    static std::atomic<unsigned long long> done{0};
    int dev = 0;
    cudaGetDevice(&dev);
    const unsigned long long bit = 1ull << (dev & 63);
    if (!(done.load(std::memory_order_acquire) & bit)) {
        cudaFuncSetAttribute(tma_any::k_resample_tma0<SRC, WINP, BOX>, cudaFuncAttributeMaxDynamicSharedMemorySize, tma_any::Cfg::SMEM);
        done.fetch_or(bit, std::memory_order_release);
    }
    const int grid = (nblocks + tma_any::kGroups - 1) / tma_any::kGroups;
    tma_any::k_resample_tma0<SRC, WINP, BOX><<<grid, dim3(32, tma::kWarps * tma_any::kGroups), tma_any::Cfg::SMEM, s>>>(jobs_dev, pieces, piece_begin, nblocks);
    return check_launch("k_resample_tma0");
}

template <int WINP>
static bool launch_tma0_src(int src, int box, const FusedJob *jobs_dev, const FusedPiece *pieces, const int *piece_begin, int nblocks,
                            cudaStream_t s) {
    if (box) return src == 1 ? launch_tma0<1, WINP, 1>(jobs_dev, pieces, piece_begin, nblocks, s)
                             : launch_tma0<0, WINP, 1>(jobs_dev, pieces, piece_begin, nblocks, s);
    return src == 1 ? launch_tma0<1, WINP, 0>(jobs_dev, pieces, piece_begin, nblocks, s)
                    : launch_tma0<0, WINP, 0>(jobs_dev, pieces, piece_begin, nblocks, s);
}

template <int S, int SRC>
static bool launch_tma3(const FusedJob *jobs_dev, const FusedPiece *pieces, const int *piece_begin, int nblocks, cudaStream_t s) {
    static std::atomic<unsigned long long> done{0};
    int dev = 0;
    cudaGetDevice(&dev);
    const unsigned long long bit = 1ull << (dev & 63);
    if (!(done.load(std::memory_order_acquire) & bit)) {
        cudaFuncSetAttribute(tma_int::k_resample_tma3<S, SRC>, cudaFuncAttributeMaxDynamicSharedMemorySize, tma_int::Cfg<S>::SMEM);
        done.fetch_or(bit, std::memory_order_release);
    }
    const int grid = (nblocks + tma_int::kGroups - 1) / tma_int::kGroups;
    tma_int::k_resample_tma3<S, SRC><<<grid, dim3(32, tma::kWarps * tma_int::kGroups), tma_int::Cfg<S>::SMEM, s>>>(jobs_dev, pieces, piece_begin, nblocks);
    return check_launch("k_resample_tma3");
}

int launch_resample_fused(const FusedKernel &k, int src, const FusedJob *jobs_dev, const FusedPiece *pieces_dev,
                          const int *piece_begin_dev, int nblocks, Stream s) {
    if (nblocks <= 0) return 0;
    cudaStream_t st = (cudaStream_t)s;
    bool ok = false;
    static_assert(tma_int::Cfg<4>::NOUT == kTmaStripCols4 && tma_int::Cfg<2>::NOUT == kTmaStripCols2 &&
                  tma_int::Cfg<4>::RROWS == kTmaRing4 && tma_int::Cfg<2>::RROWS == kTmaRing2, "integer-ratio kernel");
    static_assert(tma_any::kGroups == kTma0Groups && tma_any::Cfg::MAXT == kTma0MaxTaps && tma_any::Cfg::WINP_MAX == kTma0Window[3] &&
                  tma_any::Cfg::RROWS == kTmaRing4, "any-ratio kernel");
    static_assert(tma::kLumaBox == 2 * kTmaLumaBoxW && tma::kChunkRows == kTmaLumaBoxH && tma::kNv12Box == 2 * kTmaNv12BoxW &&
                  tma::kPlanarBox == kTmaPlanarBoxW && tma::kChromaRows == kTmaChromaBoxH, "TMA boxes");
    switch (k.kind) {
        case FusedKernel::TMA_ANY:
            switch (k.window) {
                case 0: ok = launch_tma0_src<kTma0Window[0]>(src, k.box, jobs_dev, pieces_dev, piece_begin_dev, nblocks, st); break;
                case 1: ok = launch_tma0_src<kTma0Window[1]>(src, k.box, jobs_dev, pieces_dev, piece_begin_dev, nblocks, st); break;
                case 2: ok = launch_tma0_src<kTma0Window[2]>(src, k.box, jobs_dev, pieces_dev, piece_begin_dev, nblocks, st); break;
                default: ok = launch_tma0_src<kTma0Window[3]>(src, k.box, jobs_dev, pieces_dev, piece_begin_dev, nblocks, st); break;
            }
            break;
        case FusedKernel::TMA_INT:
            if (k.ratio == 4) ok = src == 1 ? launch_tma3<4, 1>(jobs_dev, pieces_dev, piece_begin_dev, nblocks, st)
                                            : launch_tma3<4, 0>(jobs_dev, pieces_dev, piece_begin_dev, nblocks, st);
            else ok = src == 1 ? launch_tma3<2, 1>(jobs_dev, pieces_dev, piece_begin_dev, nblocks, st)
                               : launch_tma3<2, 0>(jobs_dev, pieces_dev, piece_begin_dev, nblocks, st);
            break;
        default:
            switch (k.ratio) {
                case 2: ok = launch_fused_src<2>(src, jobs_dev, pieces_dev, piece_begin_dev, nblocks, st); break;
                case 3: ok = launch_fused_src<3>(src, jobs_dev, pieces_dev, piece_begin_dev, nblocks, st); break;
                case 4: ok = launch_fused_src<4>(src, jobs_dev, pieces_dev, piece_begin_dev, nblocks, st); break;
                default: ok = launch_fused_src<0>(src, jobs_dev, pieces_dev, piece_begin_dev, nblocks, st); break;
            }
    }
    return ok ? 1 : -1;
}

__device__ __forceinline__ void half_row_convert(const uint32_t (&yw)[2], const uint32_t (&v)[6], float nk16, float rcp_y, float rcp_c,
                                                 int (&sums)[4][3]) {
#pragma unroll
    for (int p = 0; p < 4; p++) {
        float2 qr, qg, qb;
        tma::convert_pair(yw, v, p, nk16, rcp_y, rcp_c, qr, qg, qb);
        sums[p][0] += (int)(__float_as_uint(qr.x) & 0xffu) + (int)(__float_as_uint(qr.y) & 0xffu);
        sums[p][1] += (int)(__float_as_uint(qg.x) & 0xffu) + (int)(__float_as_uint(qg.y) & 0xffu);
        sums[p][2] += (int)(__float_as_uint(qb.x) & 0xffu) + (int)(__float_as_uint(qb.y) & 0xffu);
    }
}

template <bool NV12>
__device__ __forceinline__ void half_row_sums(const Tex &S, int x0, int r, float nk16, float rcp_y, float rcp_c, int (&sums)[4][3]) {
    const uint8_t *yrow = S.p0 + (size_t)r * S.pitch0 + x0;
    const uint32_t yw[2] = {__ldg(reinterpret_cast<const uint32_t *>(yrow)), __ldg(reinterpret_cast<const uint32_t *>(yrow) + 1)};
    const int ch = r >> 1, cl = (r & 1) ? ch + 1 : ch - 1, cx = x0 >> 1;
    uint32_t v[6];
#pragma unroll
    for (int k = 0; k < 6; k++) {
        uint32_t h, l;
        if (NV12) {
            const uint32_t th = __ldg(reinterpret_cast<const unsigned short *>(S.p1 + (size_t)ch * S.pitch1) + (cx - 1 + k));
            const uint32_t tl = __ldg(reinterpret_cast<const unsigned short *>(S.p1 + (size_t)cl * S.pitch1) + (cx - 1 + k));
            h = __byte_perm(th, 0, 0x4140); l = __byte_perm(tl, 0, 0x4140);
        } else {
            h = __ldg(S.p1 + (size_t)ch * S.pitch1 + cx - 1 + k) | ((uint32_t)__ldg(S.p2 + (size_t)ch * S.pitch2 + cx - 1 + k) << 16);
            l = __ldg(S.p1 + (size_t)cl * S.pitch1 + cx - 1 + k) | ((uint32_t)__ldg(S.p2 + (size_t)cl * S.pitch2 + cx - 1 + k) << 16);
        }
        v[k] = 3u * h + l;
    }
    half_row_convert(yw, v, nk16, rcp_y, rcp_c, sums);
}

__device__ __forceinline__ void half_pair_sums_nv12(const Tex &S, int x0, int r, float nk16, float rcp_y, float rcp_c, int (&sums)[4][3]) {
    const int ch = r >> 1;
    auto spread_row = [&](int crow, uint32_t (&t)[6]) {
        const uint32_t *w = reinterpret_cast<const uint32_t *>(S.p1 + (size_t)crow * S.pitch1 + x0 - 4);
        const uint32_t w0 = __ldg(w), w1 = __ldg(w + 1), w2 = __ldg(w + 2), w3 = __ldg(w + 3);
        t[0] = __byte_perm(w0, 0, 0x4342); t[1] = __byte_perm(w1, 0, 0x4140); t[2] = __byte_perm(w1, 0, 0x4342);
        t[3] = __byte_perm(w2, 0, 0x4140); t[4] = __byte_perm(w2, 0, 0x4342); t[5] = __byte_perm(w3, 0, 0x4140);
    };
    uint32_t th[6], tl[6], v[6];
    spread_row(ch, th);
#pragma unroll
    for (int k = 0; k < 6; k++) th[k] *= 3u;
#pragma unroll
    for (int half = 0; half < 2; half++) {
        spread_row(half ? ch + 1 : ch - 1, tl);
#pragma unroll
        for (int k = 0; k < 6; k++) v[k] = th[k] + tl[k];
        const uint32_t *yrow = reinterpret_cast<const uint32_t *>(S.p0 + (size_t)(r + half) * S.pitch0 + x0);
        const uint32_t yw[2] = {__ldg(yrow), __ldg(yrow + 1)};
        half_row_convert(yw, v, nk16, rcp_y, rcp_c, sums);
    }
}

__device__ __forceinline__ float smoothstep_f(float e0, float e1, float x) {
    float t = clamp01((x - e0) / (e1 - e0));
    return (t * t) * (3.0f - 2.0f * t);
}

__device__ __forceinline__ float rounded_rect_sdf(float dx, float dy, float sx, float sy, const float *radius) {
    float hx = sx / 2.0f, hy = sy / 2.0f;
    float rx, ry;
    if (dx < 0.0f) { rx = radius[0]; ry = radius[3]; } else { rx = radius[1]; ry = radius[2]; }
    if (dy < 0.0f) rx = ry;
    float qx = (fabsf(dx) - hx) + rx, qy = (fabsf(dy) - hy) + rx;
    float mx = fmaxf(qx, 0.0f), my = fmaxf(qy, 0.0f);
    return (fminf(fmaxf(qx, qy), 0.0f) + sqrtf(mx * mx + my * my)) - rx;
}

__device__ __forceinline__ bool quad_covers(const LayerDev &L, int px, int py) {
    if (px < L.px0 || px >= L.px1 || py < L.py0 || py >= L.py1) return false;
    if (!L.rotated) return true;
    long long X = (long long)px * 256 + 128, Y = (long long)py * 256 + 128;
#pragma unroll
    for (int i = 0; i < 4; i++) {
        int j = (i + 1) & 3;
        long long dx = L.vx[j] - L.vx[i], dy = L.vy[j] - L.vy[i];
        long long e = dx * (Y - L.vy[i]) - dy * (X - L.vx[i]);
        bool top_left = (dy < 0) || (dy == 0 && dx > 0);
        if (e < 0 || (e == 0 && !top_left)) return false;
    }
    return true;
}

__device__ __forceinline__ float4 sample_node(const Tables &T, const Tex *tex, int mode, float tx, float ty,
                                              bool &exact, uchar4 &texel) {
    exact = false;
    if (tex == nullptr || tex->kind == TEX_NONE) return make_float4(0.f, 0.f, 0.f, 0.f);
    const Tex &S = *tex;
    LinTap ax = linear_tap(tx, S.width), ay = linear_tap(ty, S.height);
    const float *lut = mode == 0 ? T.dec : T.u8n;
    if (ax.f == 1.0f) { ax.i0 = ax.i1; ax.f = 0.0f; }
    if (ay.f == 1.0f) { ay.i0 = ay.i1; ay.f = 0.0f; }
    uchar4 p00 = node_texel(T, S, ax.i0, ay.i0);
    if (ax.f == 0.0f && ay.f == 0.0f) {
        exact = true;
        texel = p00;
        return make_float4(lut[p00.x], lut[p00.y], lut[p00.z], T.u8n[p00.w]);
    }
    uchar4 p10, p01, p11;
    if (ax.i1 == ax.i0 + 1 && ay.i1 == ay.i0 + 1 && yuv_quad_ok(S, ax.i0, ay.i0)) {
        yuv_quad(T, S, ax.i0, ay.i0, p00, p10, p01, p11);
    } else {
        p10 = ax.f != 0.0f ? node_texel(T, S, ax.i1, ay.i0) : p00;
        p01 = ay.f != 0.0f ? node_texel(T, S, ax.i0, ay.i1) : p00;
        p11 = (ax.f != 0.0f && ay.f != 0.0f) ? node_texel(T, S, ax.i1, ay.i1) : (ax.f != 0.0f ? p10 : p01);
    }
    float4 r;
    if (mode != 0) {
        r.x = filter_u8(p00.x, p10.x, p01.x, p11.x, ax.f, ay.f);
        r.y = filter_u8(p00.y, p10.y, p01.y, p11.y, ax.f, ay.f);
        r.z = filter_u8(p00.z, p10.z, p01.z, p11.z, ax.f, ay.f);
        r.w = filter_u8(p00.w, p10.w, p01.w, p11.w, ax.f, ay.f);
        return r;
    }
    r.x = bilerp(lut[p00.x], lut[p10.x], lut[p01.x], lut[p11.x], ax.f, ay.f);
    r.y = bilerp(lut[p00.y], lut[p10.y], lut[p01.y], lut[p11.y], ax.f, ay.f);
    r.z = bilerp(lut[p00.z], lut[p10.z], lut[p01.z], lut[p11.z], ax.f, ay.f);
    r.w = bilerp(T.u8n[p00.w], T.u8n[p10.w], T.u8n[p01.w], T.u8n[p11.w], ax.f, ay.f);
    return r;
}

__device__ __forceinline__ float4 shade(const Tables &T, const CompositeJob &J, const LayerDev &L, int px, int py,
                                        bool &pass, uchar4 &texel) {
    pass = false;
    float pcx = (float)px + 0.5f, pcy = (float)py + 0.5f;
    float lx, ly, u, v;
    if (!L.rotated) {
        lx = (pcx - L.left) - L.width * 0.5f;
        ly = L.height * 0.5f - (pcy - L.top);
        u = (pcx - L.left) / L.width;
        v = (pcy - L.top) / L.height;
    } else {
        float dx = pcx - L.cx, dyu = L.cy - pcy;
        lx = dx * L.cs + dyu * L.sn;
        ly = dyu * L.cs - dx * L.sn;
        u = lx / L.width + 0.5f;
        v = 0.5f - ly / L.height;
    }
    float mask_alpha = 1.0f;
    for (int i = 0; i < L.mask_count; i++) {
        const MaskDev &m = J.masks[L.mask_begin + i];
        float d = rounded_rect_sdf((m.left + m.width / 2.0f) - pcx, (m.top + m.height / 2.0f) - pcy, m.width,
                                   m.height, m.radius);
        mask_alpha = mask_alpha * smoothstep_f(-0.5f, 0.5f, -d);
    }
    float edge = -rounded_rect_sdf(lx, ly, L.content_w, L.content_h, L.border_radius);
    float4 src = make_float4(0.f, 0.f, 0.f, 0.f);
    if (L.type == 0) {
        float tx = u * L.crop_sx + L.crop_ox;
        float ty = v * L.crop_sy + L.crop_oy;
        bool exact;
        float4 sample = sample_node(T, L.tex >= 0 ? &J.textures[L.tex] : nullptr, J.mode, tx, ty, exact, texel);
        float bw = L.border_width;
        if (bw < 1.0f) {
            float ca = smoothstep_f(-0.5f, 0.5f, edge);
            pass = exact && ca == 1.0f && mask_alpha == 1.0f && texel.w == 255;
            src = make_float4((sample.x * ca) * mask_alpha, (sample.y * ca) * mask_alpha,
                              (sample.z * ca) * mask_alpha, (sample.w * ca) * mask_alpha);
        } else if (mask_alpha < 0.01f) {
        } else if (edge > bw / 2.0f) {
            float ba = smoothstep_f(bw - 0.5f, bw + 0.5f, edge);
            float ib = 1.0f - ba;
            src = make_float4((L.border_color[0] * ib + sample.x * ba) * mask_alpha,
                              (L.border_color[1] * ib + sample.y * ba) * mask_alpha,
                              (L.border_color[2] * ib + sample.z * ba) * mask_alpha,
                              (L.border_color[3] * ib + sample.w * ba) * mask_alpha);
        } else {
            float ca = smoothstep_f(-0.5f, 0.5f, edge);
            src = make_float4((L.border_color[0] * ca) * mask_alpha, (L.border_color[1] * ca) * mask_alpha,
                              (L.border_color[2] * ca) * mask_alpha, (L.border_color[3] * ca) * mask_alpha);
        }
    } else if (L.type == 1) {
        float bw = L.border_width;
        if (bw < 1.0f) {
            float ca = smoothstep_f(-0.5f, 0.5f, edge);
            src = make_float4((L.color[0] * ca) * mask_alpha, (L.color[1] * ca) * mask_alpha,
                              (L.color[2] * ca) * mask_alpha, (L.color[3] * ca) * mask_alpha);
        } else if (edge > bw / 2.0f) {
            float ba = smoothstep_f(bw, bw + 1.0f, edge);
            float ib = 1.0f - ba;
            src = make_float4((L.border_color[0] * ib + L.color[0] * ba) * mask_alpha,
                              (L.border_color[1] * ib + L.color[1] * ba) * mask_alpha,
                              (L.border_color[2] * ib + L.color[2] * ba) * mask_alpha,
                              (L.border_color[3] * ib + L.color[3] * ba) * mask_alpha);
        } else {
            float ca = smoothstep_f(-0.5f, 0.5f, edge);
            src = make_float4((L.border_color[0] * ca) * mask_alpha, (L.border_color[1] * ca) * mask_alpha,
                              (L.border_color[2] * ca) * mask_alpha, (L.border_color[3] * ca) * mask_alpha);
        }
    } else {
        float br = L.blur_radius;
        float ba = smoothstep_f(-br / 2.0f, br / 2.0f, edge) * mask_alpha;
        src = make_float4(L.color[0] * ba, L.color[1] * ba, L.color[2] * ba, L.color[3] * ba);
    }
    return src;
}

__device__ __forceinline__ uchar4 blend(const Tables &T, int mode, uchar4 dst, float4 s) {
    s.x = clamp01(s.x); s.y = clamp01(s.y); s.z = clamp01(s.z); s.w = clamp01(s.w);
    if (s.x == 0.0f && s.y == 0.0f && s.z == 0.0f && s.w == 0.0f) return dst;
    float ia = 1.0f - s.w;
    uchar4 o;
    if (ia == 0.0f) {
        if (mode == 0) {
            o.x = (unsigned char)srgb_encode(T, s.x);
            o.y = (unsigned char)srgb_encode(T, s.y);
            o.z = (unsigned char)srgb_encode(T, s.z);
        } else {
            o.x = (unsigned char)unorm8(s.x);
            o.y = (unsigned char)unorm8(s.y);
            o.z = (unsigned char)unorm8(s.z);
        }
        o.w = 255;
        return o;
    }
    if (mode == 0) {
        o.x = (unsigned char)srgb_encode(T, fmaf(T.dec[dst.x], ia, s.x));
        o.y = (unsigned char)srgb_encode(T, fmaf(T.dec[dst.y], ia, s.y));
        o.z = (unsigned char)srgb_encode(T, fmaf(T.dec[dst.z], ia, s.z));
    } else {
        o.x = (unsigned char)unorm8(fmaf(T.u8n[dst.x], ia, s.x));
        o.y = (unsigned char)unorm8(fmaf(T.u8n[dst.y], ia, s.y));
        o.z = (unsigned char)unorm8(fmaf(T.u8n[dst.z], ia, s.z));
    }
    o.w = (unsigned char)unorm8(fmaf(T.u8n[dst.w], ia, s.w));
    return o;
}

__device__ __forceinline__ bool rect_alpha_one(float pcx, float pcy, float left, float top, float w, float h,
                                               float rmax, float shr) {
    const float hx = w * 0.5f, hy = h * 0.5f;
    const float dx = fabsf(pcx - (left + hx)), dy = fabsf(pcy - (top + hy));
    const bool inside = dx <= hx - shr && dy <= hy - shr;
    const bool corner = dx > hx - rmax - 2.0f && dy > hy - rmax - 2.0f;
    return inside && !corner;
}

__device__ __noinline__ uchar4 shade_blend(const Tables &T, const CompositeJob &J, const LayerDev &L, int X, int Y,
                                           uchar4 dst) {
    if (!L.rotated && L.type != 2) {
        const float pcx = (float)X + 0.5f, pcy = (float)Y + 0.5f;
        const float rmax = fmaxf(fmaxf(L.border_radius[0], L.border_radius[1]), fmaxf(L.border_radius[2], L.border_radius[3]));
        const float shr = 2.0f + (L.border_width >= 1.0f ? L.border_width + 1.0f : 0.0f);
        bool one = rect_alpha_one(pcx, pcy, L.left, L.top, L.content_w, L.content_h, fmaxf(rmax, 0.0f), shr);
        for (int i = 0; one && i < L.mask_count; i++) {
            const MaskDev &m = J.masks[L.mask_begin + i];
            const float mr = fmaxf(fmaxf(m.radius[0], m.radius[1]), fmaxf(m.radius[2], m.radius[3]));
            one = rect_alpha_one(pcx, pcy, m.left, m.top, m.width, m.height, fmaxf(mr, 0.0f), 2.0f);
        }
        if (one) {
            if (L.type == 1) {
                if (L.fast & FAST_CONST) return *reinterpret_cast<const uchar4 *>(&L.const_bytes);
                return blend(T, J.mode, dst, make_float4(L.color[0], L.color[1], L.color[2], L.color[3]));
            }
            bool exact;
            uchar4 texel;
            float4 sample;
            if (L.fast & FAST_IDENT) {
                texel = node_texel(T, J.textures[L.tex], X + L.tx_off, Y + L.ty_off);
                exact = true;
                const float *lut = J.mode == 0 ? T.dec : T.u8n;
                sample = make_float4(lut[texel.x], lut[texel.y], lut[texel.z], T.u8n[texel.w]);
            } else {
                const float u = (pcx - L.left) / L.width, v = (pcy - L.top) / L.height;
                sample = sample_node(T, L.tex >= 0 ? &J.textures[L.tex] : nullptr, J.mode, u * L.crop_sx + L.crop_ox,
                                     v * L.crop_sy + L.crop_oy, exact, texel);
            }
            if (exact && texel.w == 255) return texel;
            return blend(T, J.mode, dst, sample);
        }
    }
    bool pass;
    uchar4 texel;
    float4 src = shade(T, J, L, X, Y, pass, texel);
    return pass ? texel : blend(T, J.mode, dst, src);
}

#ifndef SMR_COMPOSITE_BLOCKS
#define SMR_COMPOSITE_BLOCKS 3
#endif
#define CT_W 4
#define CT_H 2
#define CB_X 32
#define CB_Y 8
#define CT_ITERS 1
#define MAX_TILE_LAYERS 1024
#define SM_LAYERS 40
// ... 599 lines not shown
```

### smelter_b200/csrc/kernels.h

```cpp
#pragma once

#include <cstddef>
#include <cstdint>

namespace smr {
namespace dev {

enum TexKind : int32_t {
    TEX_NONE = 0,
    TEX_RGBA8 = 1,
    TEX_YUV420 = 2,
    TEX_NV12 = 3,
    TEX_F16 = 4,
    TEX_BGRA = 5,
    TEX_ARGB = 6,
    TEX_YUV422 = 7,
    TEX_YUV444 = 8,
    TEX_UYVY = 9,
    TEX_YUYV = 10,
};
inline
#ifdef __CUDACC__
__host__ __device__
#endif
void chroma_dims(int out_format, int w, int h, int &cw, int &ch) {
    cw = out_format == 2 ? w : w / 2;
    ch = (out_format == 1 || out_format == 2) ? h : h / 2;
}

struct Tex {
    int32_t kind = TEX_NONE;
    int32_t width = 0, height = 0;
    int32_t full_range = 0;
    const uint8_t *p0 = nullptr, *p1 = nullptr, *p2 = nullptr;
    int32_t pitch0 = 0, pitch1 = 0, pitch2 = 0;
};

struct MaskDev {
    float radius[4];
    float top, left, width, height;
};

struct alignas(16) LayerDev {
    int32_t type;
    int32_t rotated;
    float left, top, width, height;
    float content_w, content_h;
    float cx, cy, cs, sn;
    int32_t px0, px1, py0, py1;
    long long vx[4], vy[4];
    float border_radius[4];
    float color[4];
    float border_color[4];
    float border_width, blur_radius;
    int32_t tex;
    float crop_sx, crop_ox, crop_sy, crop_oy;
    int32_t mask_begin, mask_count;
    int32_t ix0, ix1, iy0, iy1;
    int32_t jx0, jx1, jy0, jy1;
    int32_t fast;
    int32_t tx_off, ty_off;
    uint32_t const_bytes;
};
enum : int32_t { FAST_IDENT = 1, FAST_CONST = 2, FAST_LUT = 4, FAST_OPAQUE = 8, FAST_SAMPLE = 16, FAST_HALF = 32 };

struct CompositeJob {
    int32_t width, height;
    int32_t mode;
    int32_t n_layers;
    const LayerDev *layers;
    const uint32_t *tile_list;
    const MaskDev *masks;
    const Tex *textures;
    int32_t out_format;
    uint8_t *out0, *out1, *out2;
    int32_t out_pitch0, out_pitch1, out_pitch2;
    const uint8_t *direct_map;
    int32_t map_w;
    int32_t n_tiles;
};
constexpr int kDirectTileW = 128, kDirectTileH = 16;

struct ResampleJob {
    Tex src;
    int32_t axis;
    int32_t perp_offset;
    int32_t taps;
    int32_t dst_w, dst_h;
    int32_t dst_f16;
    uint8_t *dst;
    int32_t dst_pitch;
    const float *weights;
    const float *inv_wsum;
    const int32_t *first;
    int32_t box_fx, box_fy;
};

struct FusedJob {
    Tex src;
    int32_t dst_w, dst_h;
    uint8_t *dst;
    int32_t dst_pitch;
    int32_t taps_h, taps_v;
    const float *w_h, *inv_h;
    const int32_t *first_h;
    const float *w_v, *inv_v;
    const int32_t *first_v;
    const void *tm0, *tm1, *tm2;
    int32_t v_same;
    int32_t strip_cols;
    const uint8_t *lane_perm;
    const uint8_t *direct_map;
    int32_t direct_id;
    int32_t map_w;
    int32_t fx, fy;
    int32_t out_format;
    uint8_t *out0, *out1, *out2;
    int32_t out_pitch0, out_pitch1, out_pitch2;
};
struct FusedPiece {
    int32_t job, strip, oy_begin, oy_end;
};
constexpr int kFusedStripCols = 64, kFusedWarps = 8, kFusedRing = 64, kFusedSpan = 280, kFusedMaxTaps = 25;
constexpr int kTmaStripCols4 = 58, kTmaStripCols2 = 122, kTmaRing4 = 54, kTmaRing2 = 28;
constexpr int kTmaLumaBoxW = 136, kTmaLumaBoxH = 32, kTmaNv12BoxW = 144, kTmaPlanarBoxW = 160, kTmaChromaBoxH = 18;
constexpr int kTma0Groups = 2, kTma0MaxSpan = 256, kTma0MaxTaps = 25;
constexpr int kTma0Window[4] = {20, 25, 29, 33};

struct FusedKernel {
    enum Kind : int32_t {
        LDG,
        TMA_INT,
        TMA_ANY,
    } kind = LDG;
    int32_t ratio = 0, window = 0, box = 0;
    bool operator==(const FusedKernel &o) const { return kind == o.kind && ratio == o.ratio && window == o.window && box == o.box; }
};
struct FusedShape { int strip_cols, groups_per_sm, row_gran; };
inline FusedShape fused_shape(const FusedKernel &k, const FusedJob &j) {
    switch (k.kind) {
        case FusedKernel::TMA_INT: return {k.ratio == 4 ? kTmaStripCols4 : kTmaStripCols2, 3, 2};
        case FusedKernel::TMA_ANY: return {j.strip_cols, kTma0Groups, 8};
        default: return {kFusedStripCols, 3, 8};
    }
}

struct WeightJob {
    float scale, offset;
    int32_t n_out, taps;
    float *weights;
    float *inv_wsum;
    int32_t *first;
};

struct OutputJob {
    Tex src;
    int32_t out_w, out_h;
    int32_t out_format;
    uint8_t *out0, *out1, *out2;
    int32_t out_pitch0, out_pitch1, out_pitch2;
};

struct GlyphDev {
    int32_t x, y;
    uint16_t w, h, ax, ay;
    uint8_t color[4];
    int32_t content;
};
struct TextJob {
    int32_t width, height;
    int32_t mode;
    int32_t color_mode;
    int32_t n_glyphs;
    float bg[4];
    const GlyphDev *glyphs;
    const uint8_t *mask; int32_t mask_w, mask_h, mask_pitch;
    const uint8_t *color; int32_t color_w, color_h, color_pitch;
    uint8_t *out; int32_t out_pitch;
};

void upload_tables(const float *u8n, const float *srgb_dec, const float *srgb_enc_thr);

typedef void *Stream;

int launch_convert_to_rgba(const Tex &src, uint8_t *dst, int dst_pitch, Stream s);
int launch_weights(const WeightJob *jobs_dev, const WeightJob *jobs_host, int n_jobs, Stream s);
int launch_resample(const ResampleJob *jobs_dev, const ResampleJob *jobs_host, int n_jobs, Stream s);
inline int fused_source_class(int tex_kind) {
    return tex_kind == TEX_YUV420 ? 0 : tex_kind == TEX_NV12 ? 1 : tex_kind == TEX_UYVY ? 2 : tex_kind == TEX_YUYV ? 3 : -1;
}
int launch_preprocess(const Tex &src, int mode, int rescale, uint8_t *out, int out_pitch, int out_w, int out_h, Stream s);
int launch_text(const TextJob &job, Stream s);
int launch_resample_fused(const FusedKernel &k, int src, const FusedJob *jobs_dev, const FusedPiece *pieces_dev,
                          const int *piece_begin_dev, int nblocks, Stream s);
void set_int_weights(int S, const float *weights_dev, const float *inv_dev, int taps, Stream s);
int launch_composite(const CompositeJob *jobs_dev, const CompositeJob *jobs_host, const LayerDev *layers0_host, int n, Stream s);
int launch_output(const OutputJob &job, Stream s);
int launch_fill_yuv(uint8_t *p0, uint8_t *p1, uint8_t *p2, int pitch0, int pitch1, int pitch2, int w, int h,
                    int out_format, uint8_t y, uint8_t u, uint8_t v, Stream s);
const char *last_launch_error();

}
}
```

### smelter_b200/csrc/renderer.cpp

```cpp
#include <cuda.h>
#include <cuda_runtime.h>
#include <dlfcn.h>

#include <algorithm>
#include <array>
#include <cmath>
#include <cstdio>
#include <cstring>
#include <deque>
#include <map>
#include <memory>
#include <mutex>
#include <string>
#include <tuple>
#include <vector>

#include "../../include/smelter_b200.h"
#include "kernels.h"
#include "scene.h"

namespace smr {

#define CUDA_OK(expr)                                                                        \
    do {                                                                                     \
// ... 1326 lines not shown
                                     std::vector<std::optional<Resolution>> &child_res) {
    for (const std::string &id : (o.flat ? o.flat_children : node.child_input_ids)) {
        auto it = inputs_.find(id);
        Input *in = it != inputs_.end() && it->second.has_frame ? &it->second : nullptr;
        child_in.push_back(in);
        child_res.push_back(in ? std::optional<Resolution>(in->res) : std::nullopt);
    }
    return o.flat ? o.flat_root : node.layout_resolution(pts);
}

std::vector<RenderLayout> Renderer::output_layouts(const Output &o, OutputNode &node, uint64_t pts,
                                                   const std::vector<std::optional<Resolution>> &child_res, Resolution root) {
    return o.flat ? o.flat_layouts : node.layouts(pts, child_res).flatten(child_res, root);
}

smr_status Renderer::child_texture(Input &in, RenderLayout &l, int &tex_index, int &tex_w, int &tex_h) {
    tex_index = in.raw_tex; tex_w = in.tex.width; tex_h = in.tex.height;
    if (opts_.rendering_mode != SMR_MODE_GPU_OPTIMIZED) return SMR_OK;
    float rw = std::round(l.width), rh = std::round(l.height);
    int dw = rw >= 1.0f ? (rw > 16384.0f ? 16384 : (int)rw) : 1;
    int dh = rh >= 1.0f ? (rh > 16384.0f ? 16384 : (int)rh) : 1;
    AxisMapping hm{0, l.crop.left, l.crop.width, dw}, vm{1, l.crop.top, l.crop.height, dh};
    KernelPass passes[2];
    if (plan_passes(hm, vm, passes) == 0) return SMR_OK;
    uint32_t cb[4];
    memcpy(&cb[0], &l.crop.left, 4); memcpy(&cb[1], &l.crop.top, 4);
    memcpy(&cb[2], &l.crop.width, 4); memcpy(&cb[3], &l.crop.height, 4);
    auto key = std::make_tuple(in.raw_tex, cb[0], cb[1], cb[2], cb[3], dw, dh);
    auto hit = plan_.resample_cache.find(key);
    if (hit != plan_.resample_cache.end()) {
        tex_index = hit->second;
    } else if (int fused_tex = try_fused_resample(in, hm, vm, dw, dh); fused_tex != -1) {
        if (fused_tex < -1) return SMR_ERR_CUDA;
        tex_index = fused_tex;
        plan_.resample_cache[key] = tex_index;
    } else {
        int src_tex = materialised_input(in);
        int levels[2] = {hm.predecimate_levels(), vm.predecimate_levels()};
        int fac[2] = {1 << levels[0], 1 << levels[1]};
        int cur_w = in.tex.width, cur_h = in.tex.height;
        size_t cur_off = SIZE_MAX;
        if (fac[0] != 1 || fac[1] != 1) {
            int rwid = (cur_w + fac[0] - 1) / fac[0], rhei = (cur_h + fac[1] - 1) / fac[1];
            size_t off = frame_alloc((size_t)rwid * rhei * 8);
            dev::ResampleJob j{};
            j.box_fx = fac[0]; j.box_fy = fac[1];
            j.dst_w = rwid; j.dst_h = rhei; j.dst_f16 = 1; j.dst_pitch = rwid * 8;
            plan_.stages[0].push_back({j, src_tex, SIZE_MAX, off});
            cur_w = rwid; cur_h = rhei; cur_off = off;
        }
        AxisMapping rh_ = hm.on_reduced_source(levels[0]), rv_ = vm.on_reduced_source(levels[1]);
        int np = plan_passes(rh_, rv_, passes);
        if (np == 0) { set_error("resampler planning failed"); return SMR_ERR_INVALID_ARGUMENT; }
        size_t dst_off = frame_alloc((size_t)dw * dh * 4);
        for (int pi = 0; pi < np; pi++) {
            const KernelPass &kp = passes[pi];
            bool last = pi == np - 1;
            WeightEntry we;
            smr_status st = get_weights(kp, we);
            if (st != SMR_OK) return st;
            dev::ResampleJob j{};
            j.axis = kp.mapping.axis; j.perp_offset = kp.perp_offset; j.taps = we.taps;
            j.weights = we.weights; j.inv_wsum = we.inv; j.first = we.first;
            j.box_fx = j.box_fy = 1;
            size_t out_off;
            if (last) {
                j.dst_w = dw; j.dst_h = dh; j.dst_f16 = 0; j.dst_pitch = dw * 4;
                out_off = dst_off;
            } else {
                j.dst_w = kp.mapping.axis == 0 ? kp.mapping.dst_len : cur_w;
                j.dst_h = kp.mapping.axis == 1 ? kp.mapping.dst_len : cur_h;
                j.dst_f16 = 1; j.dst_pitch = j.dst_w * 8;
                out_off = frame_alloc((size_t)j.dst_w * j.dst_h * 8);
            }
            if (cur_off != SIZE_MAX) {
                j.src.kind = dev::TEX_F16; j.src.width = cur_w; j.src.height = cur_h; j.src.pitch0 = cur_w * 8;
            }
            plan_.stages[last ? 2 : 1].push_back({j, cur_off == SIZE_MAX ? src_tex : -1, cur_off, out_off});
            if (!last) { cur_w = j.dst_w; cur_h = j.dst_h; cur_off = out_off; }
        }
        dev::Tex t;
        t.kind = dev::TEX_RGBA8; t.width = dw; t.height = dh; t.pitch0 = dw * 4;
        tex_index = add_texture(t, false, dst_off);
        plan_.resample_cache[key] = tex_index;
    }
    tex_w = dw; tex_h = dh;
    l.crop = {0.0f, 0.0f, (float)dw, (float)dh};
    return SMR_OK;
}

smr_status Renderer::plan_output(Output &o, smr_output_frame &of, uint64_t pts) {
    const int mode = opts_.rendering_mode;
    of.width = (uint32_t)o.res.width; of.height = (uint32_t)o.res.height;
    of.format = o.format; of.pts_ns = pts;

    size_t row_bytes[3], rows[3];
    out_plane_layout(o.format, of.width, of.height, row_bytes, rows);
    uint8_t *dst[3] = {nullptr, nullptr, nullptr};
    int pitch[3] = {0, 0, 0};
    for (int p = 0; p < 3; p++) {
        if (!row_bytes[p]) continue;
        if (!of.planes[p]) { set_error("output plane pointer is null"); return SMR_ERR_INVALID_ARGUMENT; }
        size_t user_pitch = of.pitch[p] ? of.pitch[p] : row_bytes[p];
        if (user_pitch < row_bytes[p]) { set_error("output plane pitch is smaller than a row"); return SMR_ERR_INVALID_ARGUMENT; }
        if (of.mem_kind == SMR_MEM_DEVICE) {
            dst[p] = (uint8_t *)of.planes[p];
            pitch[p] = (int)user_pitch;
        } else {
            size_t dp = (row_bytes[p] + 15) & ~(size_t)15;
            DevBuf &stage = o.planes[slot_][p];
            CUDA_OK(stage.ensure(dp * rows[p]));
            dst[p] = stage.p;
            pitch[p] = (int)dp;
            plan_.d2h.push_back({of.planes[p], user_pitch, dst[p], dp, row_bytes[p], rows[p]});
            stats_.d2h_bytes += row_bytes[p] * rows[p];
        }
    }
    auto push_fill = [&]() {
        Fill f;
        for (int p = 0; p < 3; p++) { f.p[p] = dst[p]; f.pitch[p] = pitch[p]; }
        f.w = (int)of.width; f.h = (int)of.height; f.fmt = o.format;
        black_yuv(f.yuv);
        plan_.fills.push_back(f);
    };
    auto push_output_job = [&](int src_tex) {
        dev::OutputJob j;
        j.out_w = (int)of.width; j.out_h = (int)of.height; j.out_format = o.format;
        j.out0 = dst[0]; j.out1 = dst[1]; j.out2 = dst[2];
        j.out_pitch0 = pitch[0]; j.out_pitch1 = pitch[1]; j.out_pitch2 = pitch[2];
        plan_.outputs.push_back({j, src_tex});
    };

    if (!o.flat && o.node.root_is_input) {
        auto it = inputs_.find(o.node.root_input_id);
        if (it == inputs_.end() || !it->second.has_frame) { push_fill(); return SMR_OK; }
        Input &in = it->second;
        if (o.format == SMR_OUT_RGBA8 && (in.res.width != o.res.width || in.res.height != o.res.height)) {
            set_error("RGBA output of a pass-through root must match the input resolution");
            return SMR_ERR_UNSUPPORTED;
        }
        const bool same = in.res.width == o.res.width && in.res.height == o.res.height;
        const bool fused_fmt = o.format == SMR_OUT_PLANAR_YUV420 || o.format == SMR_OUT_NV12;
        if (same && (o.format == SMR_OUT_RGBA8 || (fused_fmt && (of.width % 2 == 0) && (of.height % 2 == 0)))) {
            RenderLayout l;
            l.kind = RenderLayout::ChildNode;
            l.width = (float)of.width; l.height = (float)of.height;
            l.crop = {0.0f, 0.0f, (float)of.width, (float)of.height};
            dev::LayerDev d;
            bool skip;
            prepare_layer(l, (int)of.width, (int)of.height, in.raw_tex, (int)of.width, (int)of.height, d, skip);
            CompositeRec pc;
            memset(&pc.job, 0, sizeof(pc.job));
            pc.job.width = (int)of.width; pc.job.height = (int)of.height; pc.job.mode = mode;
            pc.job.n_layers = skip ? 0 : 1;
            pc.layers_off = param_put(&d, sizeof(d));
            pc.masks_off = param_alloc(sizeof(dev::MaskDev));
            pc.job.out_format = o.format;
            pc.job.out0 = dst[0]; pc.job.out1 = dst[1]; pc.job.out2 = dst[2];
            pc.job.out_pitch0 = pitch[0]; pc.job.out_pitch1 = pitch[1]; pc.job.out_pitch2 = pitch[2];
            plan_.composites.push_back(pc);
            return SMR_OK;
        }
        push_output_job(in.raw_tex);
        return SMR_OK;
    }

    std::vector<Input *> child_in;
    std::vector<std::optional<Resolution>> child_res;
    const Resolution root = output_children(o, o.node, pts, child_in, child_res);
    if (root.width == 0 || root.height == 0 || root.width > 16384 || root.height > 16384) { push_fill(); return SMR_OK; }
    std::vector<RenderLayout> layouts = output_layouts(o, o.node, pts, child_res, root);
    if (layouts.size() > opts_.max_layouts_count) layouts.resize(opts_.max_layouts_count);

    const int W = (int)root.width, H = (int)root.height;
    std::vector<dev::LayerDev> layers;
    std::vector<dev::MaskDev> masks;
    for (RenderLayout &l : layouts) {
        int tex_index = -1, tex_w = 1, tex_h = 1;
        Input *in = l.kind == RenderLayout::ChildNode && l.index < child_in.size() ? child_in[l.index] : nullptr;
        if (in) {
            smr_status st = child_texture(*in, l, tex_index, tex_w, tex_h);
            if (st != SMR_OK) return st;
        }
        dev::LayerDev d;
        bool skip;
        prepare_layer(l, W, H, tex_index, tex_w, tex_h, d, skip);
        if (skip) continue;
        d.mask_begin = (int)masks.size();
        size_t nm = std::min<size_t>(l.masks.size(), SMR_MAX_MASKS);
        for (size_t i = 0; i < nm; i++) {
            const Mask &m = l.masks[i];
            dev::MaskDev md;
            md.radius[0] = m.radius.top_left; md.radius[1] = m.radius.top_right;
            md.radius[2] = m.radius.bottom_right; md.radius[3] = m.radius.bottom_left;
            md.top = m.top; md.left = m.left; md.width = m.width; md.height = m.height;
            masks.push_back(md);
        }
        d.mask_count = (int)nm;
        layers.push_back(d);
    }

    CompositeRec pc;
    memset(&pc.job, 0, sizeof(pc.job));
    pc.job.width = W; pc.job.height = H; pc.job.mode = mode;
    pc.job.n_layers = (int)layers.size();
    pc.layers_off = param_put(layers.data(), sizeof(dev::LayerDev) * layers.size());
    pc.masks_off = param_put(masks.data(), sizeof(dev::MaskDev) * masks.size());

    bool same_size = (size_t)W == o.res.width && (size_t)H == o.res.height;
    bool fused_fmt = o.format == SMR_OUT_PLANAR_YUV420 || o.format == SMR_OUT_NV12;
    bool fusable = same_size && (o.format == SMR_OUT_RGBA8 || (fused_fmt && (W % 2 == 0) && (H % 2 == 0)));
    if (fusable) {
        pc.job.out_format = o.format;
        pc.job.out0 = dst[0]; pc.job.out1 = dst[1]; pc.job.out2 = dst[2];
        pc.job.out_pitch0 = pitch[0]; pc.job.out_pitch1 = pitch[1]; pc.job.out_pitch2 = pitch[2];
        if (fused_fmt) plan_tiles(o, pc, layers, W, H);
        plan_.composites.push_back(pc);
    } else {
        if (o.format == SMR_OUT_RGBA8) { set_error("RGBA output must match the root layout resolution"); return SMR_ERR_UNSUPPORTED; }
        pc.out_frame_off = frame_alloc((size_t)W * H * 4);
        pc.job.out_format = -1;
        pc.job.out_pitch0 = W * 4;
        plan_.composites.push_back(pc);
        dev::Tex t;
        t.kind = dev::TEX_RGBA8; t.width = W; t.height = H; t.pitch0 = W * 4;
        push_output_job(add_texture(t, false, pc.out_frame_off));
    }
    return SMR_OK;
}

smr_status Renderer::render_begin(uint64_t pts, const smr_input_frame *in, uint32_t n_in, smr_output_frame *out,
                                  uint32_t n_out) {
    if ((n_in && !in) || (n_out && !out)) return SMR_ERR_INVALID_ARGUMENT;
    std::lock_guard<std::mutex> g(mu_);
    if (host_only_) { set_error("host-only handle (cuda_device = -1) cannot render: no CPU fallback"); return SMR_ERR_CUDA; }
    CUDA_OK(cudaSetDevice(opts_.cuda_device));
    if (profiling_ && !inflight_.empty()) drain();
    tick_++;
    slot_ = (int)(tick_ % kTicksInFlight);
    for (int s : inflight_)
        if (s == slot_) CUDA_OK(cudaEventSynchronize(tick_done_[s]));
    while ((int)inflight_.size() >= kTicksInFlight) {
        CUDA_OK(cudaEventSynchronize(tick_done_[inflight_.front()]));
        inflight_.pop_front();
    }
    uploaded_ = false;
    rollback_weights();
    plan_.clear();
    param_used_ = 0; frame_used_ = 0;
    uint64_t launches = 0;
    cudaStream_t done_on = stream_;

    struct WeightGuard {
        Renderer *r; bool armed = true;
        ~WeightGuard() { if (armed) r->rollback_weights(); }
    } weight_guard{this};
    smr_status st = select_inputs(pts, in, n_in, [&](Input &I, const smr_input_frame *f) {
        I.node_tex = I.raw_tex = -1;
        return f ? upload_input(I, *f) : SMR_OK;
    });
    if (st != SMR_OK) return st;
    for (uint32_t i = 0; i < n_out; i++) {
        if (!out[i].output_id) return SMR_ERR_INVALID_ARGUMENT;
        auto it = outputs_.find(out[i].output_id);
        if (it == outputs_.end()) {
            set_error(std::string("Output \"") + out[i].output_id + "\" does not exist, register it first");
            return SMR_ERR_OUTPUT_NOT_REGISTERED;
        }
        st = plan_output(it->second, out[i], pts);
        if (st != SMR_OK) return st;
    }

    CUDA_OK(cudaEventRecord(tick_start_, stream_));
    tick_started_ = true;
    if (comm_pending_) {
        CUDA_OK(cudaStreamWaitEvent(stream_, comm_done_, 0));
        comm_pending_ = false;
    }
    if (uploaded_) {
        CUDA_OK(cudaEventRecord(h2d_done_[slot_], copy_stream_));
        CUDA_OK(cudaStreamWaitEvent(stream_, h2d_done_[slot_], 0));
        CUDA_OK(cudaEventRecord(h2d_done2_[slot_], copy_stream2_));
        CUDA_OK(cudaStreamWaitEvent(stream_, h2d_done2_[slot_], 0));
    }
    if (frame_used_ + 512 > frame_dev_.cap && !inflight_.empty()) CUDA_OK(cudaStreamSynchronize(stream_));
    CUDA_OK(frame_dev_.ensure(frame_used_ + 512));
    uint8_t *fb = frame_dev_.p;
    for (TexRec &t : plan_.tex)
        if (t.frame_off != SIZE_MAX) t.tex.p0 = fb + t.frame_off;
    for (auto &stage : plan_.stages)
        for (StageRec &r : stage) {
            if (r.src_tex >= 0) r.job.src = plan_.tex[r.src_tex].tex;
            else r.job.src.p0 = fb + r.src_off;
            r.job.dst = fb + r.dst_off;
        }
    for (OutputRec &r : plan_.outputs) r.job.src = plan_.tex[r.src_tex].tex;
    for (FusedRec &f : plan_.fused) {
        f.job.src = plan_.tex[f.src_tex].tex;
        f.job.dst = fb + f.dst_off;
    }
    for (CompositeRec &c : plan_.composites)
        if (c.out_frame_off != SIZE_MAX) c.job.out0 = fb + c.out_frame_off;

    struct FusedLaunch { dev::FusedKernel kernel; int src; size_t pieces_off, begin_off; int nblocks; };
    std::vector<FusedLaunch> fused_launches;
    {
        std::vector<std::pair<dev::FusedKernel, int>> kernels;
        for (const FusedRec &f : plan_.fused) {
            std::pair<dev::FusedKernel, int> v{f.kernel, dev::fused_source_class(f.job.src.kind)};
            if (std::find(kernels.begin(), kernels.end(), v) == kernels.end()) kernels.push_back(v);
        }
        for (auto &v : kernels) {
            std::vector<int> idx, widths, heights, cols;
            dev::FusedShape shape{};
            for (size_t ji = 0; ji < plan_.fused.size(); ji++) {
                const FusedRec &f = plan_.fused[ji];
                if (!(f.kernel == v.first) || dev::fused_source_class(f.job.src.kind) != v.second) continue;
                shape = dev::fused_shape(f.kernel, f.job);
                idx.push_back((int)ji); widths.push_back(f.job.dst_w); heights.push_back(f.job.dst_h); cols.push_back(shape.strip_cols);
            }
            std::vector<dev::FusedPiece> pieces;
            std::vector<int> begin;
            partition_fused_rows(idx.data(), widths.data(), heights.data(), (int)idx.size(), sm_count_ * shape.groups_per_sm, pieces,
                                 begin, dev::kFusedStripCols, cols.data(), shape.row_gran);
            if (pieces.empty()) continue;
            for (const dev::FusedPiece &pp : pieces)
                if (plan_.fused[pp.job].direct_off != SIZE_MAX && ((pp.oy_begin | pp.oy_end) & 1)) {
                    plan_.fused[pp.job].direct_off = SIZE_MAX;
                    for (CompositeRec &pc : plan_.composites)
                        for (size_t t = 0; t < pc.direct_owner.size(); t++)
                            if (pc.direct_owner[t] == pp.job) {
                                pc.direct_owner[t] = -1;
                                pc.list.push_back((uint32_t)(t % (size_t)pc.job.map_w) | ((uint32_t)(t / (size_t)pc.job.map_w) << 16));
                            }
                }
            fused_launches.push_back({v.first, v.second, param_put(pieces.data(), sizeof(dev::FusedPiece) * pieces.size()),
                                      param_put(begin.data(), sizeof(int) * begin.size()), (int)begin.size() - 1});
        }
    }
    const size_t tex_off = param_put_all(plan_.tex, &TexRec::tex);
    size_t stage_off[3];
    for (int s = 0; s < 3; s++) stage_off[s] = param_put_all(plan_.stages[s], &StageRec::job);
    const size_t wj_off = param_put(plan_.weight_jobs.data(), sizeof(dev::WeightJob) * plan_.weight_jobs.size());
    const size_t tm_off = param_put(plan_.tmaps.data(), sizeof(CUtensorMap) * plan_.tmaps.size());
    uint64_t direct_tiles = 0;
    for (CompositeRec &pc : plan_.composites) {
        if (pc.direct_off != SIZE_MAX) {
            bool any = false;
            for (size_t t = 0; t < pc.direct_owner.size(); t++) {
                param_host_[pc.direct_off + t] = pc.direct_owner[t] >= 0 ? (uint8_t)(pc.direct_owner[t] + 1) : 0;
                any = any || pc.direct_owner[t] >= 0;
                direct_tiles += pc.direct_owner[t] >= 0 ? 1 : 0;
            }
            if (!any) pc.direct_off = SIZE_MAX;
        }
        if (pc.use_list) {
            pc.list_off = param_put(pc.list.data(), sizeof(uint32_t) * pc.list.size());
            pc.job.n_tiles = (int)pc.list.size();
        }
    }
    const size_t fj_off = param_put_all(plan_.fused, &FusedRec::job);
    const size_t cj_off = param_put_all(plan_.composites, &CompositeRec::job);
    CUDA_OK(param_pinned_[slot_].ensure(param_used_));
    CUDA_OK(param_dev_[slot_].ensure(param_used_));
    uint8_t *pd = param_dev_[slot_].p;
    auto dev_ptr = [&](size_t off) -> uint8_t * { return off != SIZE_MAX ? pd + off : nullptr; };
    dev::FusedJob *fj = reinterpret_cast<dev::FusedJob *>(param_host_.data() + fj_off);
    for (size_t i = 0; i < plan_.fused.size(); i++) {
        const FusedRec &f = plan_.fused[i];
        if (f.tmap_idx >= 0) {
            const uint8_t *m = pd + tm_off + sizeof(CUtensorMap) * (size_t)f.tmap_idx;
            fj[i].tm0 = m; fj[i].tm1 = m + sizeof(CUtensorMap); fj[i].tm2 = m + 2 * sizeof(CUtensorMap);
        }
        fj[i].direct_map = dev_ptr(f.direct_off);
    }
    dev::CompositeJob *cj = reinterpret_cast<dev::CompositeJob *>(param_host_.data() + cj_off);
    for (size_t i = 0; i < plan_.composites.size(); i++) {
        const CompositeRec &c = plan_.composites[i];
        cj[i].layers = (const dev::LayerDev *)(pd + c.layers_off);
        cj[i].masks = (const dev::MaskDev *)(pd + c.masks_off);
        cj[i].textures = (const dev::Tex *)(pd + tex_off);
        cj[i].direct_map = dev_ptr(c.direct_off);
        cj[i].tile_list = (const uint32_t *)dev_ptr(c.list_off);
    }
    memcpy(param_pinned_[slot_].p, param_host_.data(), param_used_);
    CUDA_OK(cudaMemcpyAsync(pd, param_pinned_[slot_].p, param_used_, cudaMemcpyHostToDevice, stream_));

    auto launched = [&](int n) -> bool { if (n < 0) return false; launches += (uint64_t)n; return true; };
    prof_mark(-1);
    for (auto &cv : plan_.convert_jobs) {
        const dev::Tex &src = plan_.tex[cv.first].tex;
        if (!launched(dev::launch_convert_to_rgba(src, fb + cv.second, src.width * 4, stream_))) goto fail;
        prof_mark(SMR_KERNEL_CONVERT);
    }
    if (!launched(dev::launch_weights((const dev::WeightJob *)(pd + wj_off), plan_.weight_jobs.data(), (int)plan_.weight_jobs.size(),
                                      stream_))) goto fail;
    if (!plan_.weight_jobs.empty()) prof_mark(SMR_KERNEL_WEIGHTS);
    for (auto &pw : pending_int_weights_) dev::set_int_weights(pw.first, pw.second.weights, pw.second.inv, pw.second.taps, stream_);
    pending_int_weights_.clear();
    new_weight_keys_.clear();
    weight_guard.armed = false;
    for (const FusedLaunch &fl : fused_launches) {
        if (!launched(dev::launch_resample_fused(fl.kernel, fl.src, (const dev::FusedJob *)(pd + fj_off),
                                                 (const dev::FusedPiece *)(pd + fl.pieces_off), (const int *)(pd + fl.begin_off),
                                                 fl.nblocks, stream_))) goto fail;
        prof_mark(SMR_KERNEL_RESAMPLE_FUSED);
    }
    for (int s = 0; s < 3; s++) {
        if (!launched(dev::launch_resample((const dev::ResampleJob *)(pd + stage_off[s]),
                                           (const dev::ResampleJob *)(param_host_.data() + stage_off[s]), (int)plan_.stages[s].size(),
                                           stream_))) goto fail;
        if (!plan_.stages[s].empty()) prof_mark(SMR_KERNEL_RESAMPLE_BOX + s);
    }
    if (!plan_.composites.empty()) {
        if (!launched(dev::launch_composite((const dev::CompositeJob *)(pd + cj_off), cj,
                                            (const dev::LayerDev *)(param_host_.data() + plan_.composites[0].layers_off),
                                            (int)plan_.composites.size(), stream_))) goto fail;
        prof_mark(SMR_KERNEL_COMPOSITE);
    }
    for (OutputRec &o : plan_.outputs) {
        if (!launched(dev::launch_output(o.job, stream_))) goto fail;
        prof_mark(SMR_KERNEL_OUTPUT);
    }
    for (Fill &f : plan_.fills) {
        if (!launched(dev::launch_fill_yuv(f.p[0], f.p[1], f.p[2], f.pitch[0], f.pitch[1], f.pitch[2], f.w, f.h, f.fmt,
                                           f.yuv[0], f.yuv[1], f.yuv[2], stream_))) goto fail;
        prof_mark(SMR_KERNEL_FILL);
    }
    if (!plan_.d2h.empty() && !profiling_) {
        CUDA_OK(cudaEventRecord(kernels_done_[slot_], stream_));
        CUDA_OK(cudaStreamWaitEvent(d2h_stream_, kernels_done_[slot_], 0));
        done_on = d2h_stream_;
    }
    for (PendingCopy &c : plan_.d2h)
        if (c.dpitch == c.width && c.spitch == c.width)
            CUDA_OK(cudaMemcpyAsync(c.dst, c.src, c.width * c.height, cudaMemcpyDeviceToHost, done_on));
        else
            CUDA_OK(cudaMemcpy2DAsync(c.dst, c.dpitch, c.src, c.spitch, c.width, c.height, cudaMemcpyDeviceToHost, done_on));
    stats_.kernel_launches += launches;
    stats_.last_render_kernel_launches = launches;
    stats_.last_render_direct_tiles = direct_tiles;
    stats_.frames_rendered += n_out;
    CUDA_OK(cudaEventRecord(tick_done_[slot_], done_on));
    inflight_.push_back(slot_);
    return SMR_OK;
fail:
    set_error(dev::last_launch_error());
    cudaStreamSynchronize(stream_);
    return SMR_ERR_CUDA;
}

smr_status Renderer::debug_set_inputs(uint64_t pts, const smr_input_frame *in, uint32_t n_in) {
    if (n_in && !in) return SMR_ERR_INVALID_ARGUMENT;
    std::lock_guard<std::mutex> g(mu_);
    return select_inputs(pts, in, n_in, [](Input &, const smr_input_frame *) { return SMR_OK; });
}

smr_status Renderer::render_end() {
    std::lock_guard<std::mutex> g(mu_);
    if (inflight_.empty()) return SMR_OK;
    CUDA_OK(cudaSetDevice(opts_.cuda_device));
    int s = inflight_.front();
    inflight_.pop_front();
    CUDA_OK(cudaEventSynchronize(tick_done_[s]));
    if (inflight_.empty()) fold_profile();
    return SMR_OK;
}

smr_status Renderer::render_end_all() {
    std::lock_guard<std::mutex> g(mu_);
    if (inflight_.empty()) return SMR_OK;
    CUDA_OK(cudaSetDevice(opts_.cuda_device));
    while (!inflight_.empty()) {
        int s = inflight_.front();
        inflight_.pop_front();
        CUDA_OK(cudaEventSynchronize(tick_done_[s]));
    }
    fold_profile();
    return SMR_OK;
}

void Renderer::fold_profile() {
    for (size_t i = 1; i < prof_marks_.size(); i++) {
        int k = prof_marks_[i].second;
        if (k < 0) continue;
        float ms = 0.0f;
        if (cudaEventElapsedTime(&ms, prof_marks_[i - 1].first, prof_marks_[i].first) == cudaSuccess) {
            prof_.total_ms[k] += ms;
            prof_.launches[k] += 1;
        }
    }
    prof_marks_.clear();
}

void Renderer::prof_mark(int kernel_class) {
    if (!profiling_) return;
    if (kernel_class == -1) { prof_marks_.clear(); prof_next_event_ = 0; }
    if (prof_next_event_ >= prof_events_.size()) {
        cudaEvent_t e;
        if (cudaEventCreate(&e) != cudaSuccess) return;
        prof_events_.push_back(e);
    }
    cudaEvent_t e = prof_events_[prof_next_event_++];
    cudaEventRecord(e, stream_);
    prof_marks_.push_back({e, kernel_class});
}

smr_status Renderer::comm_init(const uint8_t *id, int rank, int nranks) {
    std::lock_guard<std::mutex> g(mu_);
    if (host_only_) { set_error("host-only handle has no device"); return SMR_ERR_CUDA; }
    if (!id || nranks < 1 || rank < 0 || rank >= nranks) return SMR_ERR_INVALID_ARGUMENT;
    std::string err;
    if (!nccl_load(err)) { set_error(err); return SMR_ERR_UNSUPPORTED; }
    CUDA_OK(cudaSetDevice(opts_.cuda_device));
    NcclId nid;
    memcpy(nid.b, id, 128);
    int rc = g_nccl.CommInitRank(&nccl_comm_, nranks, nid, rank);
    if (rc != 0) { set_error(std::string("ncclCommInitRank: ") + (g_nccl.GetErrorString ? g_nccl.GetErrorString(rc) : "error")); return SMR_ERR_CUDA; }
    comm_rank_ = rank; comm_size_ = nranks;
    return SMR_OK;
}

smr_status Renderer::comm_exchange(const smr_input_frame *frames, uint32_t n, const int32_t *roots, const uint64_t *consumers,
                                   uint32_t flags) {
    std::lock_guard<std::mutex> g(mu_);
    if (!nccl_comm_) { set_error("smr_comm_init was not called"); return SMR_ERR_INVALID_ARGUMENT; }
    if (n && (!frames || !roots)) return SMR_ERR_INVALID_ARGUMENT;
    if (comm_size_ > 64 && consumers) { set_error("consumer masks cover at most 64 ranks"); return SMR_ERR_UNSUPPORTED; }
    CUDA_OK(cudaSetDevice(opts_.cuda_device));
    if (tick_started_) CUDA_OK(cudaStreamWaitEvent(comm_stream_, tick_start_, 0));
    if (flags & SMR_COMM_PEER_DIRECT) {
        smr_status st = comm_tick_barrier();
        if (st != SMR_OK) return st;
        CUDA_OK(cudaEventRecord(comm_done_, comm_stream_));
        comm_pending_ = true;
        return SMR_OK;
    }
    const uint64_t all = comm_size_ >= 64 ? ~0ull : ((1ull << comm_size_) - 1ull);
    struct Run { uint8_t *p; size_t bytes; int root; uint64_t mask; };
    std::vector<Run> runs;
    for (uint32_t i = 0; i < n; i++) {
        const smr_input_frame &f = frames[i];
        if (f.mem_kind != SMR_MEM_DEVICE) { set_error("the exchange needs device-resident planes"); return SMR_ERR_INVALID_ARGUMENT; }
        if (roots[i] < 0 || roots[i] >= comm_size_) return SMR_ERR_INVALID_ARGUMENT;
        const uint64_t mask = ((consumers ? consumers[i] : all) | (1ull << roots[i])) & all;
        FrameView v;
        if (smr_status st = read_frame(f, v); st != SMR_OK) return st;
        for (const FrameView::Plane &P : v.plane) {
            if (!P.p) continue;
            const size_t bytes = P.span();
            uint8_t *ptr = (uint8_t *)P.p;
            if ((flags & SMR_COMM_POOLED) && !runs.empty() && runs.back().root == roots[i] && runs.back().mask == mask &&
                runs.back().p + runs.back().bytes == ptr)
                runs.back().bytes += bytes;
            else
                runs.push_back({ptr, bytes, roots[i], mask});
        }
    }
    int rc = g_nccl.GroupStart();
    for (size_t i = 0; i < runs.size() && rc == 0; i++) {
        const Run &R = runs[i];
        if (R.mask == all) {
            rc = g_nccl.Broadcast(R.p, R.p, R.bytes,  1, R.root, nccl_comm_, comm_stream_);
        } else if (comm_rank_ == R.root) {
            for (int k = 0; k < comm_size_ && rc == 0; k++)
                if (k != R.root && ((R.mask >> k) & 1ull)) rc = g_nccl.Send(R.p, R.bytes, 1, k, nccl_comm_, comm_stream_);
        } else if ((R.mask >> comm_rank_) & 1ull) {
            rc = g_nccl.Recv(R.p, R.bytes, 1, R.root, nccl_comm_, comm_stream_);
        }
    }
    int rc2 = g_nccl.GroupEnd();
    if (rc == 0) rc = rc2;
    if (rc != 0) { set_error(std::string("NCCL exchange: ") + (g_nccl.GetErrorString ? g_nccl.GetErrorString(rc) : "error")); return SMR_ERR_CUDA; }
    CUDA_OK(cudaEventRecord(comm_done_, comm_stream_));
    comm_pending_ = true;
    return SMR_OK;
}

smr_status Renderer::comm_tick_barrier() {
    if (!barrier_word_) {
        CUDA_OK(cudaMalloc(&barrier_word_, 256));
        CUDA_OK(cudaMemsetAsync(barrier_word_, 0, 256, comm_stream_));
    }
    int rc = g_nccl.AllReduce(barrier_word_, barrier_word_, 1,  2,  0, nccl_comm_, comm_stream_);
    if (rc != 0) { set_error(std::string("NCCL barrier: ") + (g_nccl.GetErrorString ? g_nccl.GetErrorString(rc) : "error")); return SMR_ERR_CUDA; }
    return SMR_OK;
}

smr_status Renderer::comm_pull(const smr_input_frame *frames, const smr_input_frame *peer_frames, uint32_t n, const int32_t *roots,
                               const uint64_t *consumers) {
    std::lock_guard<std::mutex> g(mu_);
    if (!nccl_comm_) { set_error("smr_comm_init was not called"); return SMR_ERR_INVALID_ARGUMENT; }
    if (n && (!frames || !peer_frames || !roots)) return SMR_ERR_INVALID_ARGUMENT;
    CUDA_OK(cudaSetDevice(opts_.cuda_device));
    if (tick_started_) CUDA_OK(cudaStreamWaitEvent(comm_stream_, tick_start_, 0));
    smr_status st = comm_tick_barrier();
    if (st != SMR_OK) return st;
    struct Run { uint8_t *dst; const uint8_t *src; size_t bytes; };
    std::vector<Run> runs;
    for (uint32_t i = 0; i < n; i++) {
        const smr_input_frame &f = frames[i], &pf = peer_frames[i];
        if (roots[i] < 0 || roots[i] >= comm_size_) return SMR_ERR_INVALID_ARGUMENT;
        if (roots[i] == comm_rank_) continue;
        if (consumers && !((consumers[i] >> comm_rank_) & 1ull)) continue;
        if (f.mem_kind != SMR_MEM_DEVICE || pf.mem_kind != SMR_MEM_DEVICE) { set_error("the exchange needs device-resident planes"); return SMR_ERR_INVALID_ARGUMENT; }
        if (pf.format != f.format || pf.width != f.width || pf.height != f.height) { set_error("peer frame geometry differs"); return SMR_ERR_INVALID_ARGUMENT; }
        FrameView v, pv;
        st = read_frame(f, v);
        if (st == SMR_OK) st = read_frame(pf, pv);
        if (st != SMR_OK) return st;
        for (int p = 0; p < 3; p++) {
            if (!v.plane[p].p) continue;
            if (v.plane[p].pitch != pv.plane[p].pitch) { set_error("peer frame pitch differs"); return SMR_ERR_INVALID_ARGUMENT; }
            const size_t bytes = v.plane[p].span();
            uint8_t *d = (uint8_t *)v.plane[p].p;
            const uint8_t *sp = pv.plane[p].p;
            if (!runs.empty() && runs.back().dst + runs.back().bytes == d && runs.back().src + runs.back().bytes == sp) runs.back().bytes += bytes;
            else runs.push_back({d, sp, bytes});
        }
    }
    for (const Run &R : runs) CUDA_OK(cudaMemcpyAsync(R.dst, R.src, R.bytes, cudaMemcpyDeviceToDevice, comm_stream_));
    CUDA_OK(cudaEventRecord(comm_done_, comm_stream_));
    comm_pending_ = true;
    return SMR_OK;
}

smr_status Renderer::peer_pool_alloc(size_t bytes, void **dev_ptr, uint8_t handle[64]) {
    std::lock_guard<std::mutex> g(mu_);
    if (!dev_ptr || !handle || !bytes) return SMR_ERR_INVALID_ARGUMENT;
    static_assert(sizeof(cudaIpcMemHandle_t) == 64, "handle size of the C ABI");
    CUDA_OK(cudaSetDevice(opts_.cuda_device));
    void *p = nullptr;
    CUDA_OK(cudaMalloc(&p, bytes));
    cudaIpcMemHandle_t h;
    if (cudaIpcGetMemHandle(&h, p) != cudaSuccess) { cudaGetLastError(); cudaFree(p); set_error("cudaIpcGetMemHandle failed"); return SMR_ERR_CUDA; }
    memcpy(handle, &h, 64);
    peer_own_.push_back(p);
    *dev_ptr = p;
    return SMR_OK;
}

smr_status Renderer::peer_pool_open(const uint8_t handle[64], void **dev_ptr) {
    std::lock_guard<std::mutex> g(mu_);
    if (!dev_ptr || !handle) return SMR_ERR_INVALID_ARGUMENT;
    CUDA_OK(cudaSetDevice(opts_.cuda_device));
    cudaIpcMemHandle_t h;
    memcpy(&h, handle, 64);
    void *p = nullptr;
    cudaError_t e = cudaIpcOpenMemHandle(&p, h, cudaIpcMemLazyEnablePeerAccess);
    if (e != cudaSuccess) { cudaGetLastError(); set_error(std::string("cudaIpcOpenMemHandle: ") + cudaGetErrorString(e)); return SMR_ERR_CUDA; }
    peer_opened_.push_back(p);
    *dev_ptr = p;
    return SMR_OK;
}

smr_status Renderer::peer_pool_close(void *dev_ptr) {
    std::lock_guard<std::mutex> g(mu_);
    auto it = std::find(peer_opened_.begin(), peer_opened_.end(), dev_ptr);
    if (it == peer_opened_.end()) return SMR_ERR_INVALID_ARGUMENT;
    CUDA_OK(cudaSetDevice(opts_.cuda_device));
    cudaStreamSynchronize(stream_);
    if (comm_stream_) cudaStreamSynchronize(comm_stream_);
    tmap_cache_.clear();
    cudaIpcCloseMemHandle(dev_ptr);
    peer_opened_.erase(it);
    return SMR_OK;
}

smr_status Renderer::peer_pool_free(void *dev_ptr) {
    std::lock_guard<std::mutex> g(mu_);
    auto it = std::find(peer_own_.begin(), peer_own_.end(), dev_ptr);
    if (it == peer_own_.end()) return SMR_ERR_INVALID_ARGUMENT;
    CUDA_OK(cudaSetDevice(opts_.cuda_device));
    cudaStreamSynchronize(stream_);
    if (comm_stream_) cudaStreamSynchronize(comm_stream_);
    tmap_cache_.clear();
    cudaFree(dev_ptr);
    peer_own_.erase(it);
    return SMR_OK;
}

smr_status Renderer::comm_destroy() {
    std::lock_guard<std::mutex> g(mu_);
    if (nccl_comm_) {
        cudaSetDevice(opts_.cuda_device);
        cudaStreamSynchronize(comm_stream_);
        cudaStreamSynchronize(stream_);
        g_nccl.CommDestroy(nccl_comm_);
        nccl_comm_ = nullptr;
    }
    return SMR_OK;
}

smr_status Renderer::set_profiling(int enabled) {
    std::lock_guard<std::mutex> g(mu_);
    if (!host_only_) { cudaSetDevice(opts_.cuda_device); drain(); }
    profiling_ = enabled != 0;
    memset(&prof_, 0, sizeof(prof_));
    return SMR_OK;
}

smr_status Renderer::debug_layouts(const char *output_id, uint64_t pts, smr_render_layout *out, uint32_t cap,
                                   uint32_t *n, uint32_t *rw, uint32_t *rh) {
    if (!output_id || !n) return SMR_ERR_INVALID_ARGUMENT;
    std::lock_guard<std::mutex> g(mu_);
    auto it = outputs_.find(output_id);
    if (it == outputs_.end()) { set_error("output not registered"); return SMR_ERR_OUTPUT_NOT_REGISTERED; }
    Output &o = it->second;
    *n = 0;
    if (!o.flat && o.node.root_is_input) { if (rw) *rw = 0; if (rh) *rh = 0; return SMR_OK; }
    OutputNode copy = o.node;
    std::vector<Input *> child_in;
    std::vector<std::optional<Resolution>> child_res;
    const Resolution root = output_children(o, copy, pts, child_in, child_res);
    if (rw) *rw = (uint32_t)root.width;
    if (rh) *rh = (uint32_t)root.height;
    std::vector<RenderLayout> layouts = output_layouts(o, copy, pts, child_res, root);
    *n = (uint32_t)layouts.size();
    if (!out) return SMR_OK;
    if (cap < layouts.size()) return SMR_ERR_BUFFER_TOO_SMALL;
    for (size_t i = 0; i < layouts.size(); i++) {
        const RenderLayout &l = layouts[i];
        smr_render_layout &d = out[i];
        memset(&d, 0, sizeof(d));
        d.type = (int)l.kind;
        d.top = l.top; d.left = l.left; d.width = l.width; d.height = l.height;
        d.rotation_degrees = l.rotation_degrees;
        d.border_radius[0] = l.border_radius.top_left; d.border_radius[1] = l.border_radius.top_right;
        d.border_radius[2] = l.border_radius.bottom_right; d.border_radius[3] = l.border_radius.bottom_left;
        d.color = {l.color.r, l.color.g, l.color.b, l.color.a};
        d.border_color = {l.border_color.r, l.border_color.g, l.border_color.b, l.border_color.a};
        d.border_width = l.border_width; d.blur_radius = l.blur_radius;
        d.child_index = (int)l.index;
        d.crop_top = l.crop.top; d.crop_left = l.crop.left; d.crop_width = l.crop.width; d.crop_height = l.crop.height;
        d.masks_len = (int)std::min<size_t>(l.masks.size(), SMR_MAX_MASKS);
        for (int m = 0; m < d.masks_len; m++) {
            const Mask &mk = l.masks[m];
            d.masks[m].radius[0] = mk.radius.top_left; d.masks[m].radius[1] = mk.radius.top_right;
            d.masks[m].radius[2] = mk.radius.bottom_right; d.masks[m].radius[3] = mk.radius.bottom_left;
            d.masks[m].top = mk.top; d.masks[m].left = mk.left; d.masks[m].width = mk.width; d.masks[m].height = mk.height;
        }
    }
    return SMR_OK;
}

}

struct smr_renderer {
    smr::Renderer impl;
    explicit smr_renderer(const smr_options &o) : impl(o) {}
};

static thread_local std::string g_create_error;

extern "C" {

smr_status smr_create(const smr_options *opts, smr_renderer **out) {
    if (!opts || !out) return SMR_ERR_INVALID_ARGUMENT;
    *out = nullptr;
    smr_renderer *r = nullptr;
    try { r = new smr_renderer(*opts); } catch (...) { return SMR_ERR_OUT_OF_MEMORY; }
    smr_status st;
    try { st = r->impl.init(); } catch (...) { st = SMR_ERR_OUT_OF_MEMORY; }
    if (st != SMR_OK) {
        g_create_error = r->impl.last_error();
        delete r;
        return st;
    }
    *out = r;
    return SMR_OK;
}

void smr_destroy(smr_renderer *r) { delete r; }

#define SMR_GUARD(call)                                                       \
    if (!r) return SMR_ERR_INVALID_ARGUMENT;                                  \
    try { return call; }                                                      \
    catch (const std::bad_alloc &) { return SMR_ERR_OUT_OF_MEMORY; }          \
    catch (...) { r->impl.set_error("internal error"); return SMR_ERR_INVALID_ARGUMENT; }

smr_status smr_register_input(smr_renderer *r, const char *id) { SMR_GUARD(r->impl.register_input(id)) }
smr_status smr_unregister_input(smr_renderer *r, const char *id) { SMR_GUARD(r->impl.unregister_input(id)) }
smr_status smr_update_scene(smr_renderer *r, const char *output_id, uint32_t w, uint32_t h, int32_t fmt,
                            const smr_component *root) { SMR_GUARD(r->impl.update_scene(output_id, w, h, fmt, root)) }
smr_status smr_unregister_output(smr_renderer *r, const char *id) { SMR_GUARD(r->impl.unregister_output(id)) }
smr_status smr_set_layouts(smr_renderer *r, const char *output_id, uint32_t w, uint32_t h, int32_t fmt, uint32_t root_w,
                           uint32_t root_h, const char *const *child_ids, uint32_t n_children, const smr_render_layout *layouts,
                           uint32_t n) { SMR_GUARD(r->impl.set_layouts(output_id, w, h, fmt, root_w, root_h, child_ids, n_children, layouts, n)) }
smr_status smr_render_begin(smr_renderer *r, uint64_t pts, const smr_input_frame *in, uint32_t n_in,
                            smr_output_frame *out, uint32_t n_out) { SMR_GUARD(r->impl.render_begin(pts, in, n_in, out, n_out)) }
smr_status smr_render_end(smr_renderer *r) { SMR_GUARD(r->impl.render_end()) }
smr_status smr_debug_partition(const int32_t *dst_w, const int32_t *dst_h, uint32_t n_jobs, uint32_t max_blocks,
                               int32_t *pieces, uint32_t pieces_cap, uint32_t *n_pieces, int32_t *begin, uint32_t begin_cap,
                               uint32_t *n_blocks) {
    if ((n_jobs && (!dst_w || !dst_h)) || !n_pieces || !n_blocks) return SMR_ERR_INVALID_ARGUMENT;
    std::vector<int> idx(n_jobs);
    for (uint32_t i = 0; i < n_jobs; i++) idx[i] = (int)i;
    std::vector<smr::dev::FusedPiece> pc;
    std::vector<int> bg;
    smr::partition_fused_rows(idx.data(), dst_w, dst_h, (int)n_jobs, (int)max_blocks, pc, bg);
    *n_pieces = (uint32_t)pc.size();
    *n_blocks = bg.empty() ? 0 : (uint32_t)bg.size() - 1;
    if (pc.size() > pieces_cap || bg.size() > begin_cap) return SMR_ERR_BUFFER_TOO_SMALL;
    for (size_t i = 0; i < pc.size(); i++) {
        pieces[4 * i] = pc[i].job; pieces[4 * i + 1] = pc[i].strip; pieces[4 * i + 2] = pc[i].oy_begin; pieces[4 * i + 3] = pc[i].oy_end;
    }
    for (size_t i = 0; i < bg.size(); i++) begin[i] = bg[i];
    return SMR_OK;
}
smr_status smr_preprocess_frame(smr_renderer *r, const smr_input_frame *f, uint32_t ow, uint32_t oh, void *rgba, uint32_t pitch,
                                int32_t mem_kind) { SMR_GUARD(r->impl.preprocess_frame(f, ow, oh, rgba, pitch, mem_kind)) }
smr_status smr_premultiply_rgba8(smr_renderer *r, const smr_input_frame *f, void *rgba, uint32_t pitch, int32_t mem_kind) {
    SMR_GUARD(r->impl.preprocess_frame(f, 0, 0, rgba, pitch, mem_kind, true))
}
smr_status smr_render_text(smr_renderer *r, uint32_t w, uint32_t h, smr_rgba bg, const smr_glyph *glyphs, uint32_t n,
                           const smr_atlas *mask, const smr_atlas *color, int32_t color_mode, void *rgba, uint32_t pitch, int32_t mem_kind) {
    SMR_GUARD(r->impl.render_text(w, h, bg, glyphs, n, mask, color, color_mode, rgba, pitch, mem_kind))
}
smr_status smr_render(smr_renderer *r, uint64_t pts, const smr_input_frame *in, uint32_t n_in, smr_output_frame *out,
                      uint32_t n_out) {
    if (!r) return SMR_ERR_INVALID_ARGUMENT;
    smr_status st = smr_render_begin(r, pts, in, n_in, out, n_out);
    if (st != SMR_OK) return st;
    SMR_GUARD(r->impl.render_end_all())
}
smr_status smr_debug_layouts(smr_renderer *r, const char *output_id, uint64_t pts, smr_render_layout *out, uint32_t cap,
                             uint32_t *n, uint32_t *rw, uint32_t *rh) { SMR_GUARD(r->impl.debug_layouts(output_id, pts, out, cap, n, rw, rh)) }
smr_status smr_debug_set_inputs(smr_renderer *r, uint64_t pts, const smr_input_frame *in, uint32_t n_in) { SMR_GUARD(r->impl.debug_set_inputs(pts, in, n_in)) }
smr_status smr_comm_get_unique_id(uint8_t id[128]) {
    if (!id) return SMR_ERR_INVALID_ARGUMENT;
    std::string err;
    if (!smr::nccl_load(err)) { g_create_error = err; return SMR_ERR_UNSUPPORTED; }
    smr::NcclId nid;
    if (smr::g_nccl.GetUniqueId(&nid) != 0) { g_create_error = "ncclGetUniqueId failed"; return SMR_ERR_CUDA; }
    memcpy(id, nid.b, 128);
    return SMR_OK;
}
smr_status smr_comm_init(smr_renderer *r, const uint8_t id[128], int32_t rank, int32_t nranks) { SMR_GUARD(r->impl.comm_init(id, rank, nranks)) }
smr_status smr_comm_broadcast_inputs(smr_renderer *r, const smr_input_frame *frames, uint32_t n, const int32_t *root_ranks) { SMR_GUARD(r->impl.comm_exchange(frames, n, root_ranks, nullptr, 0)) }
smr_status smr_comm_exchange_inputs(smr_renderer *r, const smr_input_frame *frames, uint32_t n, const int32_t *root_ranks,
                                    const uint64_t *consumer_masks, uint32_t flags) { SMR_GUARD(r->impl.comm_exchange(frames, n, root_ranks, consumer_masks, flags)) }
smr_status smr_comm_pull_inputs(smr_renderer *r, const smr_input_frame *frames, const smr_input_frame *peer_frames, uint32_t n,
                                const int32_t *root_ranks, const uint64_t *consumer_masks) { SMR_GUARD(r->impl.comm_pull(frames, peer_frames, n, root_ranks, consumer_masks)) }
smr_status smr_peer_pool_alloc(smr_renderer *r, size_t bytes, void **dev_ptr, uint8_t handle[64]) { SMR_GUARD(r->impl.peer_pool_alloc(bytes, dev_ptr, handle)) }
smr_status smr_peer_pool_open(smr_renderer *r, const uint8_t handle[64], void **dev_ptr) { SMR_GUARD(r->impl.peer_pool_open(handle, dev_ptr)) }
smr_status smr_peer_pool_close(smr_renderer *r, void *dev_ptr) { SMR_GUARD(r->impl.peer_pool_close(dev_ptr)) }
smr_status smr_peer_pool_free(smr_renderer *r, void *dev_ptr) { SMR_GUARD(r->impl.peer_pool_free(dev_ptr)) }
smr_status smr_comm_destroy(smr_renderer *r) { SMR_GUARD(r->impl.comm_destroy()) }
smr_status smr_set_profiling(smr_renderer *r, int32_t enabled) { SMR_GUARD(r->impl.set_profiling(enabled)) }
smr_status smr_get_kernel_times(smr_renderer *r, smr_kernel_times *out) {
    if (!r || !out) return SMR_ERR_INVALID_ARGUMENT;
    r->impl.kernel_times(out);
    return SMR_OK;
}
smr_status smr_get_stats(smr_renderer *r, smr_stats *out) {
    if (!r || !out) return SMR_ERR_INVALID_ARGUMENT;
    r->impl.stats(out);
    return SMR_OK;
}
void *smr_cuda_stream(smr_renderer *r) { return r ? r->impl.stream() : nullptr; }
smr_status smr_host_register(void *ptr, size_t bytes) {
    if (!ptr || !bytes) return SMR_ERR_INVALID_ARGUMENT;
    cudaError_t e = cudaHostRegister(ptr, bytes, cudaHostRegisterPortable);
    if (e == cudaErrorHostMemoryAlreadyRegistered) { cudaGetLastError(); return SMR_OK; }
    if (e != cudaSuccess) { cudaGetLastError(); return SMR_ERR_CUDA; }
    return SMR_OK;
}
smr_status smr_host_unregister(void *ptr) {
    if (!ptr) return SMR_ERR_INVALID_ARGUMENT;
    if (cudaHostUnregister(ptr) != cudaSuccess) { cudaGetLastError(); return SMR_ERR_CUDA; }
    return SMR_OK;
}
const char *smr_last_error(smr_renderer *r) { return r ? r->impl.last_error() : g_create_error.c_str(); }
const char *smr_version(void) { return "smelter_b200 0.1 (sm_90a)"; }

smr_status smr_debug_tile_plan(const int32_t *boxes, uint32_t n_layers, uint32_t width, uint32_t height, int32_t sorted,
                               int32_t *owner_layer, uint32_t owner_cap, uint32_t *tiles, uint32_t tiles_cap, uint32_t *n_tiles) {
    static_assert(sizeof(smr::TileLayerBox) == 14 * sizeof(int32_t), "14 ints per layer");
    if ((n_layers && !boxes) || !n_tiles || width == 0 || height == 0 || width > 16384 * 4 || height > 16384 * 4) return SMR_ERR_INVALID_ARGUMENT;
    try {
        std::vector<int> owner;
        std::vector<uint32_t> list;
        smr::plan_tiles_core(reinterpret_cast<const smr::TileLayerBox *>(boxes), (int)n_layers, (int)width, (int)height, sorted != 0, owner, list);
        *n_tiles = (uint32_t)list.size();
        if (owner_layer) {
            if (owner_cap < owner.size()) return SMR_ERR_BUFFER_TOO_SMALL;
            for (size_t i = 0; i < owner.size(); i++) owner_layer[i] = owner[i];
        }
        if (tiles) {
            if (tiles_cap < list.size()) return SMR_ERR_BUFFER_TOO_SMALL;
            memcpy(tiles, list.data(), sizeof(uint32_t) * list.size());
        }
        return SMR_OK;
    } catch (...) { return SMR_ERR_OUT_OF_MEMORY; }
}
smr_status smr_output_plane_sizes(uint32_t w, uint32_t h, int32_t fmt, size_t sizes[3]) {
    if (!sizes) return SMR_ERR_INVALID_ARGUMENT;
    if (fmt < SMR_OUT_PLANAR_YUV420 || fmt > SMR_OUT_NV12) return SMR_ERR_UNSUPPORTED;
    size_t rb[3], rows[3];
    smr::out_plane_layout(fmt, w, h, rb, rows);
    for (int i = 0; i < 3; i++) sizes[i] = rb[i] * rows[i];
    return SMR_OK;
}

void smr_component_default(int32_t type, smr_component *c) {
    if (!c) return;
    memset(c, 0, sizeof(*c));
    c->type = type;
    c->direction = SMR_DIRECTION_ROW;
    c->overflow = SMR_OVERFLOW_HIDDEN;
    c->rescale_mode = SMR_RESCALE_FIT;
    c->horizontal_align = SMR_HALIGN_CENTER;
    c->vertical_align = SMR_VALIGN_CENTER;
    c->tile_aspect_ratio_w = 16;
    c->tile_aspect_ratio_h = 9;
}

}
```

### smelter_b200/csrc/resample_tma.cuh

```cuda
#pragma once

namespace tma {

constexpr int kWarps = 8;
constexpr int kChunkRows = 32;
constexpr int kLumaBox = 272, kNv12Box = 288, kPlanarBox = 160, kChromaRows = 18;
constexpr int kLumaBytes = kLumaBox * kChunkRows;
constexpr int kChromaBytesNv12 = ((kNv12Box * kChromaRows + 127) / 128) * 128;
constexpr int kChromaBytesPlanar = ((kPlanarBox * kChromaRows + 127) / 128) * 128;
constexpr int kStageBytes = kLumaBytes + 2 * kChromaBytesPlanar;
static_assert(kLumaBytes % 128 == 0, "chroma destination alignment");
static_assert(kStageBytes >= kLumaBytes + kChromaBytesNv12, "stage size");
constexpr int kDecRep = 32;
constexpr float kMagicRound = 12582912.0f;
constexpr uint32_t kMagicBits = 0x4B400000u;
constexpr int kThrOff = 256 * kDecRep * 4;
constexpr int kBarOff = kThrOff + 256 * 4;
constexpr int kKaddrOff = kBarOff + 64;
constexpr int kStashOff = kBarOff + 128;
constexpr int kStashBytes = 1024;
constexpr int kTailBytes = kStashOff + kStashBytes;

template <int S> constexpr int kStripCols = S == 4 ? kTmaStripCols4 : kTmaStripCols2;
template <int S> constexpr int kLead = S == 2 ? 1 : 0;

struct Chunk {
    int valid;
    int job, ox0;
    int x0;
    int r0, nrows;
    int last;
    int o0, oy_end;
};

template <int S, int BX>
struct ChunkIter {
    const FusedJob *jobs;
    const FusedPiece *pieces;
    int pi, pend;
    int job, ox0, x0, oy_end, onext, ocur;
    int produced_hi, rnext, rhi;
    int H, tv, fv0;
    int in_group, vs;
    __device__ __forceinline__ void init(const FusedJob *j, const FusedPiece *p, int b, int e) {
        jobs = j; pieces = p; pi = b - 1; pend = e; in_group = false; onext = 0; oy_end = 0;
        job = ox0 = x0 = ocur = 0; produced_hi = rnext = rhi = 0; H = tv = fv0 = 0; vs = false;
    }
    __device__ __forceinline__ Chunk next() {
        constexpr int rows = kChunkRows / BX;
        Chunk c;
        c.valid = 0; c.job = c.ox0 = c.x0 = c.r0 = c.nrows = c.last = c.o0 = c.oy_end = 0;
        if (!(in_group && rnext <= rhi)) {
            if (onext >= oy_end) {
                pi++;
                if (pi >= pend) return c;
                const FusedPiece P = pieces[pi];
                const FusedJob &J = jobs[P.job];
                job = P.job; ox0 = P.strip * (S ? kStripCols<S> : J.strip_cols); onext = P.oy_begin; oy_end = P.oy_end;
                x0 = S ? __ldg(J.first_h + ox0) - kLead<S> : __ldg(J.first_h + ox0) & ~1;
                H = J.src.height / BX; tv = J.taps_v; vs = J.v_same != 0;
                fv0 = __ldg(J.first_v);
                produced_hi = -0x40000000;
            }
            ocur = onext;
            const int o_l = min(ocur + kWarps - 1, oy_end - 1);
            const int f_lo = (S && vs) ? fv0 + S * ocur : __ldg(jobs[job].first_v + ocur);
            const int f_hi = (S && vs) ? fv0 + S * o_l : __ldg(jobs[job].first_v + o_l);
            const int need_lo = min(max(f_lo, 0), H - 1);
            const int need_hi = min(max(f_hi + tv - 1, 0), H - 1);
            rnext = max(produced_hi + 1, need_lo);
            rhi = need_hi;
            produced_hi = max(produced_hi, need_hi);
            onext += kWarps;
            in_group = true;
        }
        c.valid = 1; c.job = job; c.ox0 = ox0; c.x0 = x0; c.o0 = ocur; c.oy_end = oy_end;
        c.r0 = rnext;
        c.nrows = max(0, min(rows, rhi - rnext + 1));
        rnext += rows;
        c.last = rnext > rhi;
        return c;
    }
};

template <class It>
struct Stash { It it; Chunk nxt; };
template <class It, int GROUPS>
__device__ __forceinline__ Stash<It> *stash_slots(unsigned char *tail, int grp) {
    static_assert(sizeof(Stash<It>) * 2 * GROUPS <= kStashBytes, "stash");
    return reinterpret_cast<Stash<It> *>(tail + kStashOff) + 2 * grp;
}

__device__ __forceinline__ void group_sync(int g) { asm volatile("bar.sync %0, 256;" ::"r"(g + 1) : "memory"); }

template <int GROUPS, class Extra>
__device__ __forceinline__ uint32_t setup_block(unsigned char *tail, Extra extra) {
    float *s_dec = reinterpret_cast<float *>(tail), *s_thr = reinterpret_cast<float *>(tail + kThrOff);
    volatile uint32_t *s_kaddr = reinterpret_cast<volatile uint32_t *>(tail + kKaddrOff);
    const int btid = threadIdx.y * 32 + threadIdx.x, bn = 32 * kWarps * GROUPS;
    for (int i = btid; i < 256 * kDecRep; i += bn) s_dec[i] = c_dec[i / kDecRep];
    for (int i = btid; i < 256; i += bn) s_thr[i] = c_thr[i];
    if (btid == 0) {
        *s_kaddr = smem_u32(s_dec) - (kMagicBits << 7);
        for (int g = 0; g < GROUPS; g++) {
            mbar_init(smem_u32(tail + kBarOff) + 16u * (uint32_t)g, 1);
            mbar_init(smem_u32(tail + kBarOff) + 16u * (uint32_t)g + 8, 1);
        }
        asm volatile("fence.mbarrier_init.release.cluster;" ::: "memory");
    }
    extra();
    __syncthreads();
    return *s_kaddr + 4u * (uint32_t)threadIdx.x;
}

__device__ __forceinline__ int luma_tile_x(int x0) { return x0 & ~15; }
template <bool NV12>
__device__ __forceinline__ int chroma_tile_x(int x0) { return NV12 ? ((x0 - 2) & ~15) : (((x0 >> 1) - 1) & ~15); }

template <bool NV12, int BX>
__device__ __forceinline__ void issue(const FusedJob *jobs, const Chunk &c, uint32_t dst, uint32_t bar) {
    if (!c.valid || c.nrows == 0) return;
    const FusedJob &J = jobs[c.job];
    const int x0 = c.x0 * BX, sr0 = c.r0 * BX;
    const int cyb = (sr0 >> 1) - 1;
    const int xt = luma_tile_x(x0), xc = chroma_tile_x<NV12>(x0);
    if (NV12) {
        mbar_expect_tx(bar, kLumaBox * kChunkRows + kNv12Box * kChromaRows);
        tma_load_2d(dst, J.tm0, xt >> 1, sr0, bar);
        tma_load_2d(dst + kLumaBytes, J.tm1, xc >> 1, cyb, bar);
    } else {
        mbar_expect_tx(bar, kLumaBox * kChunkRows + 2 * kPlanarBox * kChromaRows);
        tma_load_2d(dst, J.tm0, xt >> 1, sr0, bar);
        tma_load_2d(dst + kLumaBytes, J.tm1, xc, cyb, bar);
        tma_load_2d(dst + kLumaBytes + kChromaBytesPlanar, J.tm2, xc, cyb, bar);
    }
}

template <bool NV12>
__device__ __forceinline__ void replicate_edges(unsigned char *st, int x0, int lrows, int W, int tid, int grp) {
    const int xt = luma_tile_x(x0), xc = chroma_tile_x<NV12>(x0);
    const int cw = W >> 1;
    if (!(xt < 0 || xt + kLumaBox > W || xc < 0 || (NV12 ? xc + kNv12Box > W : xc + kPlanarBox > cw))) return;
    const int sub = tid & 7;
    {
        const int bl = min(max(0, -xt), kLumaBox - 1), br = min(max(W - xt, 1), kLumaBox);
        for (int row = tid >> 3; row < lrows; row += 32) {
            unsigned char *lr = st + row * kLumaBox;
            const unsigned char vl = lr[bl], vr = lr[br - 1];
            for (int j = sub; j < bl; j += 8) lr[j] = vl;
            for (int j = br + sub; j < kLumaBox; j += 8) lr[j] = vr;
        }
    }
    if (NV12) {
        const int c0 = xc >> 1, nt = kNv12Box / 2;
        const int tl = min(max(0, -c0), nt - 1), tr = min(max(cw - c0, 1), nt);
        for (int row = tid >> 3; row < kChromaRows; row += 32) {
            unsigned short *cr = reinterpret_cast<unsigned short *>(st + kLumaBytes + row * kNv12Box);
            const unsigned short vl = cr[tl], vr = cr[tr - 1];
            for (int j = sub; j < tl; j += 8) cr[j] = vl;
            for (int j = tr + sub; j < nt; j += 8) cr[j] = vr;
        }
    } else {
        const int nt = kPlanarBox;
        const int tl = min(max(0, -xc), nt - 1), tr = min(max(cw - xc, 1), nt);
        for (int row = tid >> 3; row < 2 * kChromaRows; row += 32) {
            unsigned char *cr = st + kLumaBytes + (row >= kChromaRows ? kChromaBytesPlanar + (row - kChromaRows) * kPlanarBox : row * kPlanarBox);
            const unsigned char vl = cr[tl], vr = cr[tr - 1];
            for (int j = sub; j < tl; j += 8) cr[j] = vl;
            for (int j = tr + sub; j < nt; j += 8) cr[j] = vr;
        }
    }
    fence_proxy_async();
    group_sync(grp);
}

template <bool NV12>
struct LaneWords {
    uint32_t l_off, l_sh, c_off, c_sh;
    __device__ __forceinline__ LaneWords(int x0, int lane) {
        const int dl = x0 - luma_tile_x(x0), dc = (NV12 ? x0 - 2 : (x0 >> 1) - 1) - chroma_tile_x<NV12>(x0);
        l_off = (uint32_t)((dl & ~3) + lane * 8); l_sh = (uint32_t)(dl & 3) * 8u;
        c_off = (uint32_t)((dc & ~3) + lane * (NV12 ? 8 : 4)); c_sh = (uint32_t)(dc & 3) * 8u;
    }
};

template <bool NV12>
__device__ __forceinline__ void fetch_row(uint32_t sb, const LaneWords<NV12> &lw, int r, int sr0, int chei, uint32_t (&yw)[2],
                                          uint32_t (&v)[6]) {
    {
        const uint32_t la = sb + (uint32_t)((r - sr0) * kLumaBox) + lw.l_off;
        uint32_t w0, w1, w2;
        if (lw.l_off & 4u) { w0 = lds32v(la); lds64v(la + 4, w1, w2); }
        else { lds64v(la, w0, w1); w2 = lds32v(la + 8); }
        yw[0] = __funnelshift_r(w0, w1, lw.l_sh);
        yw[1] = __funnelshift_r(w1, w2, lw.l_sh);
    }
    const int cyb = (sr0 >> 1) - 1;
    const int ch = r >> 1;
    const int cl = (r & 1) ? min(ch + 1, chei - 1) : max(ch - 1, 0);
    const uint32_t c_off = lw.c_off, c_sh = lw.c_sh;
    if (NV12) {
        const uint32_t bh = sb + kLumaBytes + (uint32_t)((ch - cyb) * kNv12Box) + c_off;
        const uint32_t bl = sb + kLumaBytes + (uint32_t)((cl - cyb) * kNv12Box) + c_off;
        uint32_t h0, h1, h2, h3, l0, l1, l2, l3;
        if (c_off & 4u) {
            h0 = lds32v(bh); lds64v(bh + 4, h1, h2); h3 = lds32v(bh + 12);
            l0 = lds32v(bl); lds64v(bl + 4, l1, l2); l3 = lds32v(bl + 12);
        } else {
            lds64v(bh, h0, h1); lds64v(bh + 8, h2, h3);
            lds64v(bl, l0, l1); lds64v(bl + 8, l2, l3);
        }
        const uint32_t ph0 = __funnelshift_r(h0, h1, c_sh), ph1 = __funnelshift_r(h1, h2, c_sh), ph2 = __funnelshift_r(h2, h3, c_sh);
        const uint32_t pl0 = __funnelshift_r(l0, l1, c_sh), pl1 = __funnelshift_r(l1, l2, c_sh), pl2 = __funnelshift_r(l2, l3, c_sh);
        v[0] = 3u * __byte_perm(ph0, 0, 0x4140) + __byte_perm(pl0, 0, 0x4140);
        v[1] = 3u * __byte_perm(ph0, 0, 0x4342) + __byte_perm(pl0, 0, 0x4342);
        v[2] = 3u * __byte_perm(ph1, 0, 0x4140) + __byte_perm(pl1, 0, 0x4140);
        v[3] = 3u * __byte_perm(ph1, 0, 0x4342) + __byte_perm(pl1, 0, 0x4342);
        v[4] = 3u * __byte_perm(ph2, 0, 0x4140) + __byte_perm(pl2, 0, 0x4140);
        v[5] = 3u * __byte_perm(ph2, 0, 0x4342) + __byte_perm(pl2, 0, 0x4342);
    } else {
        const uint32_t uh = sb + kLumaBytes + (uint32_t)((ch - cyb) * kPlanarBox) + c_off;
        const uint32_t ul = sb + kLumaBytes + (uint32_t)((cl - cyb) * kPlanarBox) + c_off;
        const uint32_t vh = uh + kChromaBytesPlanar, vl = ul + kChromaBytesPlanar;
        auto eight = [&](uint32_t a, uint32_t &q0, uint32_t &q1) {
            const uint32_t w0 = lds32v(a), w1 = lds32v(a + 4), w2 = lds32v(a + 8);
            q0 = __funnelshift_r(w0, w1, c_sh); q1 = __funnelshift_r(w1, w2, c_sh);
        };
        uint32_t uh0, uh1, ul0, ul1, vh0, vh1, vl0, vl1;
        eight(uh, uh0, uh1); eight(ul, ul0, ul1); eight(vh, vh0, vh1); eight(vl, vl0, vl1);
        v[0] = 3u * (__byte_perm(uh0, vh0, 0x0400) & 0x00ff00ffu) + (__byte_perm(ul0, vl0, 0x0400) & 0x00ff00ffu);
        v[1] = 3u * (__byte_perm(uh0, vh0, 0x0501) & 0x00ff00ffu) + (__byte_perm(ul0, vl0, 0x0501) & 0x00ff00ffu);
        v[2] = 3u * (__byte_perm(uh0, vh0, 0x0602) & 0x00ff00ffu) + (__byte_perm(ul0, vl0, 0x0602) & 0x00ff00ffu);
        v[3] = 3u * (__byte_perm(uh0, vh0, 0x0703) & 0x00ff00ffu) + (__byte_perm(ul0, vl0, 0x0703) & 0x00ff00ffu);
        v[4] = 3u * (__byte_perm(uh1, vh1, 0x0400) & 0x00ff00ffu) + (__byte_perm(ul1, vl1, 0x0400) & 0x00ff00ffu);
        v[5] = 3u * (__byte_perm(uh1, vh1, 0x0501) & 0x00ff00ffu) + (__byte_perm(ul1, vl1, 0x0501) & 0x00ff00ffu);
    }
}

__device__ __forceinline__ void convert_pair(const uint32_t (&yw)[2], const uint32_t (&v)[6], int p, float nk16, float rcp_y,
                                             float rcp_c, float2 &qr, float2 &qg, float2 &qb) {
    const uint32_t ne = v[p] + 3u * v[p + 1], no = 3u * v[p + 1] + v[p + 2];
    const float m23 = -8388608.0f;
    float2 nu = add2(make_float2(__uint_as_float(__byte_perm(ne, 0x4B000000u, 0x7610)),
                                 __uint_as_float(__byte_perm(no, 0x4B000000u, 0x7610))), splat(m23));
    float2 nv = add2(make_float2(__uint_as_float(__byte_perm(ne, 0x4B000000u, 0x7632)),
                                 __uint_as_float(__byte_perm(no, 0x4B000000u, 0x7632))), splat(m23));
    const uint32_t ywd = yw[p >> 1];
    float2 ny = add2(make_float2(__uint_as_float(__byte_perm(ywd, 0x4B000000u, (p & 1) ? 0x7642 : 0x7640)),
                                 __uint_as_float(__byte_perm(ywd, 0x4B000000u, (p & 1) ? 0x7643 : 0x7641))), splat(m23));
    const float c1 = __uint_as_float(0x3b808081u), lo1 = __uint_as_float(0xaf7efeffu);
    const float c16 = __uint_as_float(0x39808081u), lo16 = __uint_as_float(0xad7efeffu);
    float2 y = fma2(ny, splat(c1), mul2(ny, splat(lo1)));
    float2 u = fma2(nu, splat(c16), mul2(nu, splat(lo16)));
    float2 w = fma2(nv, splat(c16), mul2(nv, splat(lo16)));
    y = add2(y, splat(nk16)); u = add2(u, splat(nk16)); w = add2(w, splat(nk16));
    y = make_float2(__saturatef(y.x * rcp_y), __saturatef(y.y * rcp_y));
    u = make_float2(__saturatef(u.x * rcp_c), __saturatef(u.y * rcp_c));
    w = make_float2(__saturatef(w.x * rcp_c), __saturatef(w.y * rcp_c));
    const float2 um = add2(u, splat(-0.5f)), vm = add2(w, splat(-0.5f));
    const float2 gi = fma2(splat(-0.1873f), um, y);
    const float2 rr = make_float2(__saturatef(fmaf(1.5748f, vm.x, y.x)), __saturatef(fmaf(1.5748f, vm.y, y.y)));
    const float2 gg = make_float2(__saturatef(fmaf(-0.4681f, vm.x, gi.x)), __saturatef(fmaf(-0.4681f, vm.y, gi.y)));
    const float2 bb = make_float2(__saturatef(fmaf(1.8556f, um.x, y.x)), __saturatef(fmaf(1.8556f, um.y, y.y)));
    qr = add2_after_mul(mul2(rr, splat(255.0f)), splat(kMagicRound));
    qg = add2_after_mul(mul2(gg, splat(255.0f)), splat(kMagicRound));
    qb = add2_after_mul(mul2(bb, splat(255.0f)), splat(kMagicRound));
}

__device__ __forceinline__ void convert_run(const uint32_t (&yw)[2], const uint32_t (&v)[6], float nk16, float rcp_y, float rcp_c,
                                            uint32_t kaddr, float2 (&prg)[8], float (&pb)[8]) {
#pragma unroll
    for (int p = 0; p < 4; p++) {
        float2 qr, qg, qb;
        convert_pair(yw, v, p, nk16, rcp_y, rcp_c, qr, qg, qb);
        prg[2 * p] = make_float2(lds_tab((__float_as_uint(qr.x) << 7) + kaddr), lds_tab((__float_as_uint(qg.x) << 7) + kaddr));
        prg[2 * p + 1] = make_float2(lds_tab((__float_as_uint(qr.y) << 7) + kaddr), lds_tab((__float_as_uint(qg.y) << 7) + kaddr));
        pb[2 * p] = lds_tab((__float_as_uint(qb.x) << 7) + kaddr);
        pb[2 * p + 1] = lds_tab((__float_as_uint(qb.y) << 7) + kaddr);
    }
}

template <int OUT, class ColOf>
__device__ __forceinline__ void encode_store(const FusedJob &J, const float2 (&acc)[3 * OUT / 2], int oy, const float *s_thr,
                                             int ox0, int strip_cols, ColOf col_of, uint32_t (&px)[OUT]) {
    const float inv_v = __ldg(J.inv_v + oy);
#pragma unroll
    for (int j = 0; j < OUT; j++) {
        const float rv = (j & 1) ? acc[j / 2].y : acc[j / 2].x;
        const float gv = (j & 1) ? acc[(OUT + j) / 2].y : acc[(OUT + j) / 2].x;
        const float bv = (j & 1) ? acc[(2 * OUT + j) / 2].y : acc[(2 * OUT + j) / 2].x;
        auto enc = [&](float lin) -> uint32_t {
            const float x = clamp01(lin);
            const int k = max((__float_as_int(x) >> 15) - ENC1_KEY0, 0);
            const uint32_t e = __ldg(c_enc1 + k);
            return e + (x >= s_thr[e] ? 1u : 0u);
        };
        px[j] = enc(rv * inv_v) | (enc(gv * inv_v) << 8) | (enc(bv * inv_v) << 16) | 0xff000000u;
    }
    uint32_t *drow = reinterpret_cast<uint32_t *>(J.dst + (size_t)oy * J.dst_pitch);
    const int ncols = min(strip_cols, J.dst_w - ox0);
#pragma unroll
    for (int j = 0; j < OUT; j += 2) {
        const int col = col_of(j);
        if (col >= 0 && col + 1 < ncols) {
            *reinterpret_cast<uint2 *>(drow + ox0 + col) = make_uint2(px[j], px[j + 1]);
        } else if (col >= 0 && col < ncols) {
            drow[ox0 + col] = px[j];
        }
    }
}

}
```

### smelter_b200/csrc/resample_tma3.cuh

```cuda
#pragma once

namespace tma_int {
using namespace tma;

constexpr int kGroups = 3;

template <int S>
struct Cfg {
    static constexpr int P = 8;
    static constexpr int OUT = P / S;
    static constexpr int TAPS = 6 * S + 1;
    static constexpr int A = kLead<S>;
    static constexpr int NST = (A + S * (OUT - 1) + TAPS + P - 1) / P;
    static __host__ __device__ constexpr int last_stage(int j) { return (A + S * j + TAPS - 1) / P; }
    static __host__ __device__ constexpr int nout() {
        int m = 1 << 30;
        for (int j = 0; j < OUT; j++) {
            int c = OUT * (32 - last_stage(j)) + j;
            m = c < m ? c : m;
        }
        return m;
    }
    static constexpr int NOUT = nout();
    static constexpr int RROWS = S == 4 ? 54 : 28;
    static constexpr int RROW_BYTES = 32 * 3 * OUT * 4;
    static constexpr int RING_BYTES = RROWS * RROW_BYTES;
    static constexpr int GROUP_BYTES = kStageBytes + RING_BYTES;
    static constexpr int SMEM = kGroups * GROUP_BYTES + kTailBytes;
};

template <int S, int SRC>
__global__ void __launch_bounds__(32 * kWarps * kGroups, 1) k_resample_tma3(const FusedJob *jobs, const FusedPiece *pieces, const int *piece_begin,
                                                                            int n_virtual_blocks) {
    using K = Cfg<S>;
    using It = ChunkIter<S, 1>;
    constexpr int P = K::P, OUT = K::OUT, TAPS = K::TAPS, A = K::A, NST = K::NST;
    constexpr bool NV12 = SRC == 1;
    extern __shared__ __align__(128) unsigned char smem_all[];
    const int lane = threadIdx.x, warp = threadIdx.y % kWarps, grp = threadIdx.y / kWarps, tid = warp * 32 + lane;
    unsigned char *tail = smem_all + kGroups * K::GROUP_BYTES;
    const float *s_thr = reinterpret_cast<const float *>(tail + kThrOff);
    unsigned char *smem = smem_all + (size_t)grp * K::GROUP_BYTES;
    const uint32_t stage0 = smem_u32(smem);
    float *ring = reinterpret_cast<float *>(smem + kStageBytes);
    const uint32_t bar0 = smem_u32(tail + kBarOff) + 16u * (uint32_t)grp;
    const uint32_t kaddr = setup_block<kGroups>(tail, [] {});
    const int vb = blockIdx.x * kGroups + grp;
    if (vb >= n_virtual_blocks) return;

    Stash<It> *stash = stash_slots<It, kGroups>(tail, grp);
    uint32_t step = 0;
    It it;
    it.init(jobs, pieces, __ldg(piece_begin + vb), __ldg(piece_begin + vb + 1));

    Chunk cur = it.next();
    if (!cur.valid) return;
    if (tid == 0) issue<NV12, 1>(jobs, cur, stage0, bar0);
    uint32_t nchunk = 0;

    while (cur.valid) {
        Stash<It> *const parked = stash + (step & 1u);
        {
            const Chunk nxt = it.next();
            if (tid == 0) { parked->it = it; parked->nxt = nxt; }
        }
        const bool cur_tma = cur.nrows > 0;
        const FusedJob &J = jobs[cur.job];
        const int W = J.src.width, H = J.src.height, chei = H >> 1;
        const bool full_range = J.src.full_range != 0;
        const float nk16 = full_range ? 0.0f : -K16, rcp_y = full_range ? 1.0f : RCP_Y, rcp_c = full_range ? 1.0f : RCP_C;
        const uint32_t sb = stage0;
        if (cur_tma) {
            mbar_wait(bar0, nchunk & 1u);
            replicate_edges<NV12>(smem, cur.x0, cur.nrows, W, tid, grp);
            const LaneWords<NV12> lw(cur.x0, lane);
            for (int r = cur.r0 + warp; r < cur.r0 + cur.nrows; r += kWarps) {
                uint32_t yw[2], v[6];
                fetch_row<NV12>(sb, lw, r, cur.r0, chei, yw, v);
                float2 prg[P];
                float pb[P];
                convert_run(yw, v, nk16, rcp_y, rcp_c, kaddr, prg, pb);
                float2 arg[OUT];
                float ab[OUT];
#pragma unroll
                for (int j = 0; j < OUT; j++) { arg[j] = make_float2(0.f, 0.f); ab[j] = 0.f; }
#pragma unroll
                for (int s = 0; s < NST; s++) {
#pragma unroll
                    for (int i = 0; i < P; i++) {
#pragma unroll
                        for (int j = 0; j < OUT; j++) {
                            const int t = P * s + i - A - S * j;
                            if (t >= 0 && t < TAPS) arg[j] = fma2(prg[i], splat(c_wint[S][t]), arg[j]);
                        }
#pragma unroll
                        for (int j = 0; j < OUT; j += 2) {
                            const int t0 = P * s + i - A - S * j, t1 = t0 - S;
                            const bool a0 = t0 >= 0 && t0 < TAPS, a1 = t1 >= 0 && t1 < TAPS;
                            if (a0 && a1) {
                                const float2 d = fma2(splat(pb[i]), c_wpair[S][a0 ? t0 : 0], make_float2(ab[j], ab[j + 1]));
                                ab[j] = d.x; ab[j + 1] = d.y;
                            } else if (a0) {
                                ab[j] = fmaf(pb[i], c_wint[S][a0 ? t0 : 0], ab[j]);
                            } else if (a1) {
                                ab[j + 1] = fmaf(pb[i], c_wint[S][a1 ? t1 : 0], ab[j + 1]);
                            }
                        }
                    }
                    if (s + 1 < NST) {
#pragma unroll
                        for (int j = 0; j < OUT; j++)
                            if (K::last_stage(j) > s) {
                                arg[j].x = __shfl_up_sync(0xffffffffu, arg[j].x, 1);
                                arg[j].y = __shfl_up_sync(0xffffffffu, arg[j].y, 1);
                                ab[j] = __shfl_up_sync(0xffffffffu, ab[j], 1);
                            }
                    }
                }
                {
                    const float inv = c_winv[S];
                    float *dst = ring + (size_t)(r % K::RROWS) * (K::RROW_BYTES / 4) + lane * 3 * OUT;
#pragma unroll
                    for (int j = 0; j < OUT; j += 2) {
                        const float2 fr = __half22float2(__floats2half2_rn(arg[j].x * inv, arg[j + 1].x * inv));
                        const float2 fg = __half22float2(__floats2half2_rn(arg[j].y * inv, arg[j + 1].y * inv));
                        const float2 fb = __half22float2(__floats2half2_rn(ab[j] * inv, ab[j + 1] * inv));
                        *reinterpret_cast<float2 *>(dst + j) = fr;
                        *reinterpret_cast<float2 *>(dst + OUT + j) = fg;
                        *reinterpret_cast<float2 *>(dst + 2 * OUT + j) = fb;
                    }
                }
            }
            nchunk++;
        }
        group_sync(grp);
        if (tid == 0) issue<NV12, 1>(jobs, parked->nxt, stage0, bar0);
        if (cur.last) {
            const int tv = J.taps_v;
            const float *lbase = ring + lane * 3 * OUT;
            constexpr int ROWF = K::RROW_BYTES / 4;
            const int row_end = min(cur.o0 + kWarps, cur.oy_end);
            auto col_of = [&](int j) { return OUT * (lane - K::last_stage(j)) + j; };
            auto owned = [&](int oa, bool (&own)[OUT / 2]) {
                const int ncols = min(K::NOUT, J.dst_w - cur.ox0);
#pragma unroll
                for (int j = 0; j < OUT; j += 2) {
                    const int col = col_of(j);
                    own[j / 2] = false;
                    if (J.direct_map == nullptr || col < 0 || col >= ncols || oa >= row_end) continue;
                    const int X = J.fx + cur.ox0 + col, Y = J.fy + oa;
                    own[j / 2] = (int)__ldg(J.direct_map + (Y / kDirectTileH) * J.map_w + X / kDirectTileW) == J.direct_id;
                }
            };
            auto emit = [&](const uint32_t (&pa)[OUT], const uint32_t (&pb)[OUT], int oa, const bool (&own)[OUT / 2]) {
#pragma unroll
                for (int j = 0; j < OUT; j += 2) {
                    if (!own[j / 2]) continue;
                    emit_yuv_2x2(J, J.fx + cur.ox0 + col_of(j), J.fy + oa, pa[j], pa[j + 1], pb[j], pb[j + 1]);
                }
            };
            auto one_row = [&](int oy, uint32_t (&px)[OUT]) {
                const int fv = __ldg(J.first_v + oy);
                const float *wv = J.w_v + (size_t)oy * tv;
                float2 acc[3 * OUT / 2];
#pragma unroll
                for (int k = 0; k < 3 * OUT / 2; k++) acc[k] = make_float2(0.f, 0.f);
                for (int t = 0; t < tv; t++) {
                    const float wt = __ldg(wv + t);
                    const int row = min(max(fv + t, 0), H - 1);
                    const float *p = lbase + (row % K::RROWS) * ROWF;
#pragma unroll
                    for (int k = 0; k < 3 * OUT / 2; k++) acc[k] = fma2(*reinterpret_cast<const float2 *>(p + 2 * k), splat(wt), acc[k]);
                }
                encode_store<OUT>(J, acc, oy, s_thr, cur.ox0, K::NOUT, col_of, px);
            };
            if (J.v_same) {
                if (warp < kWarps / 2) {
                    const int oa = cur.o0 + 2 * warp, ob = oa + 1;
                    const int fa = __ldg(J.first_v) + S * oa;
                    bool own[OUT / 2];
                    owned(oa, own);
                    if (ob < row_end && fa >= 0 && fa + S + TAPS - 1 <= H - 1) {
                        float2 aa[3 * OUT / 2], bb2[3 * OUT / 2];
#pragma unroll
                        for (int k = 0; k < 3 * OUT / 2; k++) { aa[k] = make_float2(0.f, 0.f); bb2[k] = make_float2(0.f, 0.f); }
                        const int slot0 = fa % K::RROWS, nwrap = K::RROWS - slot0;
                        const float *p0 = lbase + slot0 * ROWF;
#pragma unroll
                        for (int u = 0; u < TAPS + S; u++) {
                            const float *p = p0 + (u >= nwrap ? (u - K::RROWS) * ROWF : u * ROWF);
                            float2 v[3 * OUT / 2];
#pragma unroll
                            for (int k = 0; k < 3 * OUT / 2; k++) v[k] = *reinterpret_cast<const float2 *>(p + 2 * k);
                            if (u < TAPS) {
#pragma unroll
                                for (int k = 0; k < 3 * OUT / 2; k++) aa[k] = fma2(v[k], splat(c_wint[S][u < TAPS ? u : 0]), aa[k]);
                            }
                            if (u >= S) {
#pragma unroll
                                for (int k = 0; k < 3 * OUT / 2; k++) bb2[k] = fma2(v[k], splat(c_wint[S][u >= S ? u - S : 0]), bb2[k]);
                            }
                        }
                        uint32_t pa[OUT], pb[OUT];
                        encode_store<OUT>(J, aa, oa, s_thr, cur.ox0, K::NOUT, col_of, pa);
                        encode_store<OUT>(J, bb2, ob, s_thr, cur.ox0, K::NOUT, col_of, pb);
                        emit(pa, pb, oa, own);
                    } else {
                        uint32_t pa[OUT], pb[OUT];
                        if (oa < row_end) one_row(oa, pa);
                        if (ob < row_end) { one_row(ob, pb); emit(pa, pb, oa, own); }
                    }
                }
            } else {
                const int oy = cur.o0 + warp;
                uint32_t pz[OUT];
                if (oy < row_end) one_row(oy, pz);
            }
            group_sync(grp);
        }
        cur = parked->nxt; it = parked->it; step++;
    }
}

}
```

Before: 1714.

## Bake integer-ratio resample weights as constexpr and add a shared-memory luma table

Replaces the constant-memory integer-ratio filter weights with compile-time constexpr tables, so the FMA coefficients become immediates, and drops the paired-weight constant array. Hoists the full-range flag to a kernel argument, splitting fused launches by range, and precomputes a per-block shared-memory luma lookup table that replaces per-pixel Y normalisation arithmetic. Adds a debug export for checking weights against the device generator. The hardcoded weights only hold for the specific Lanczos kernel and offsets, and the table adds shared memory per block, which could hurt occupancy.

```diff
diff --git a/include/smelter_b200.h b/include/smelter_b200.h
--- a/include/smelter_b200.h
+++ b/include/smelter_b200.h
@@ -221,6 +221,9 @@
 smr_status smr_debug_partition(const int32_t *dst_w, const int32_t *dst_h, uint32_t n_jobs, uint32_t max_blocks,
                                int32_t *pieces, uint32_t pieces_cap, uint32_t *n_pieces, int32_t *begin,
                                uint32_t begin_cap, uint32_t *n_blocks);
+
+smr_status smr_debug_weights(float scale, float offset, uint32_t out_coord, float *weights, uint32_t cap, uint32_t *taps,
+                             float *inv);
 
 smr_status smr_debug_tile_plan(const int32_t *boxes, uint32_t n_layers, uint32_t width, uint32_t height, int32_t sorted,
                                int32_t *owner_layer, uint32_t owner_cap, uint32_t *tiles, uint32_t tiles_cap, uint32_t *n_tiles);
diff --git a/smelter_b200/_ffi.py b/smelter_b200/_ffi.py
--- a/smelter_b200/_ffi.py
+++ b/smelter_b200/_ffi.py
@@ -123,7 +123,7 @@
 
 EXPORTS = [
     "smr_create", "smr_destroy", "smr_register_input", "smr_unregister_input", "smr_update_scene",
-    "smr_unregister_output", "smr_set_layouts", "smr_render", "smr_render_begin", "smr_render_end", "smr_preprocess_frame", "smr_premultiply_rgba8", "smr_render_text", "smr_debug_partition", "smr_debug_tile_plan", "smr_output_plane_sizes",
+    "smr_unregister_output", "smr_set_layouts", "smr_render", "smr_render_begin", "smr_render_end", "smr_preprocess_frame", "smr_premultiply_rgba8", "smr_render_text", "smr_debug_partition", "smr_debug_tile_plan", "smr_debug_weights", "smr_output_plane_sizes",
     "smr_component_default", "smr_debug_layouts", "smr_debug_set_inputs", "smr_get_stats", "smr_set_profiling", "smr_get_kernel_times",
     "smr_comm_get_unique_id", "smr_comm_init", "smr_comm_broadcast_inputs", "smr_comm_exchange_inputs", "smr_comm_pull_inputs", "smr_peer_pool_alloc", "smr_peer_pool_open", "smr_peer_pool_close", "smr_peer_pool_free", "smr_comm_destroy", "smr_host_register", "smr_host_unregister", "smr_cuda_stream", "smr_last_error",
     "smr_version",
@@ -165,6 +165,9 @@
     L.smr_debug_tile_plan.argtypes = [C.POINTER(C.c_int32), C.c_uint32, C.c_uint32, C.c_uint32, C.c_int32, C.POINTER(C.c_int32), C.c_uint32,
                                       C.POINTER(C.c_uint32), C.c_uint32, C.POINTER(C.c_uint32)]
     L.smr_debug_tile_plan.restype = C.c_int32
+    L.smr_debug_weights.argtypes = [C.c_float, C.c_float, C.c_uint32, C.POINTER(C.c_float), C.c_uint32, C.POINTER(C.c_uint32),
+                                    C.POINTER(C.c_float)]
+    L.smr_debug_weights.restype = C.c_int32
     L.smr_output_plane_sizes.argtypes = [C.c_uint32, C.c_uint32, C.c_int32, C.POINTER(C.c_size_t * 3)]
     L.smr_component_default.argtypes = [C.c_int32, C.POINTER(Component)]
     L.smr_component_default.restype = None
diff --git a/smelter_b200/build.py b/smelter_b200/build.py
--- a/smelter_b200/build.py
+++ b/smelter_b200/build.py
@@ -6,7 +6,7 @@
 CSRC = os.path.join(HERE, "csrc")
 LIB = os.path.join(HERE, "libsmelter_b200.so")
 SOURCES = ["kernels.cu", "renderer.cpp", "scene.cpp"]
-HEADERS = ["kernels.h", "scene.h", "ptx_helpers.cuh", "resample_tma.cuh", "resample_tma3.cuh", "resample_tma0.cuh", os.path.join("..", "..", "include", "smelter_b200.h")]
+HEADERS = ["kernels.h", "int_weights.h", "scene.h", "ptx_helpers.cuh", "resample_tma.cuh", "resample_tma3.cuh", "resample_tma0.cuh", os.path.join("..", "..", "include", "smelter_b200.h")]
 
 NVCC_FLAGS = [
     "-std=c++17", "-O3",
diff --git a/smelter_b200/csrc/int_weights.h b/smelter_b200/csrc/int_weights.h
--- /dev/null
+++ b/smelter_b200/csrc/int_weights.h
@@ -0,0 +1,39 @@
+#pragma once
+
+namespace smr {
+namespace dev {
+
+template <int S> __host__ __device__ constexpr float int_weight(int t);
+template <int S> __host__ __device__ constexpr float int_inv();
+
+template <>
+__host__ __device__ constexpr float int_weight<2>(int t) {
+    constexpr float w[13] = {
+        0x1.e213ccp-8f, 0x1.ebdda6p-6f, -0x1.15ac52p-4f, -0x1.101eb4p-3f,
+        0x1.14ac9ap-2f, 0x1.c7b6dap-1f, 0x1.c7b6d6p-1f, 0x1.14aca2p-2f,
+        -0x1.101eaap-3f, -0x1.15ac58p-4f, 0x1.ebdd96p-6f, 0x1.e213ep-8f,
+        0x0p+0f,
+    };
+    return w[t];
+}
+template <>
+__host__ __device__ constexpr float int_inv<2>() { return 0x1.00c718p-1f; }
+
+template <>
+__host__ __device__ constexpr float int_weight<4>(int t) {
+    constexpr float w[25] = {
+        0x1.e187c2p-10f, 0x1.ff0e28p-7f, 0x1.f090dp-6f, 0x1.4ed58ep-6f,
+        -0x1.f4d59p-6f, -0x1.afe02p-4f, -0x1.2d9954p-3f, -0x1.5bcd24p-4f,
+        0x1.edb5aep-4f, 0x1.c0267ep-2f, 0x1.8746c2p-1f, 0x1.f1846ep-1f,
+        0x1.f184b6p-1f, 0x1.8746dp-1f, 0x1.c0268p-2f, 0x1.edb5a2p-4f,
+        -0x1.5bcd2ep-4f, -0x1.2d9954p-3f, -0x1.afe016p-4f, -0x1.f4d574p-6f,
+        0x1.4ed59p-6f, 0x1.f090cp-6f, 0x1.ff0e0ep-7f, 0x1.e18772p-10f,
+        0x0p+0f,
+    };
+    return w[t];
+}
+template <>
+__host__ __device__ constexpr float int_inv<4>() { return 0x1.00c1dcp-2f; }
+
+}
+}
diff --git a/smelter_b200/csrc/kernels.cu b/smelter_b200/csrc/kernels.cu
--- a/smelter_b200/csrc/kernels.cu
+++ b/smelter_b200/csrc/kernels.cu
@@ -7,6 +7,7 @@
 #include <cstring>
 
 #include "kernels.h"
+#include "int_weights.h"
 
 namespace smr {
 namespace dev {
@@ -356,6 +357,27 @@
     J.first[o] = (int)fc;
 }
 
+int debug_weights(float scale, float offset, int out_coord, float *w_host, int cap, int *taps_out, float *inv_host) {
+    const float ks = fmaxf(scale, 1.0f);
+    const int taps = (int)ceilf(2.0f * (3.0f * ks)) + 1, n_out = out_coord + 1;
+    *taps_out = taps;
+    if (out_coord < 0 || taps > cap) return 0;
+    const size_t nw = (size_t)n_out * taps;
+    unsigned char *d = nullptr;
+    if (cudaMalloc(&d, sizeof(WeightJob) + sizeof(float) * (nw + n_out) + sizeof(int32_t) * n_out) != cudaSuccess) return -1;
+    WeightJob j{};
+    j.scale = scale; j.offset = offset; j.n_out = n_out; j.taps = taps;
+    j.weights = reinterpret_cast<float *>(d + sizeof(WeightJob));
+    j.inv_wsum = j.weights + nw;
+    j.first = reinterpret_cast<int32_t *>(j.inv_wsum + n_out);
+    bool ok = cudaMemcpy(d, &j, sizeof(j), cudaMemcpyHostToDevice) == cudaSuccess &&
+              launch_weights(reinterpret_cast<const WeightJob *>(d), &j, 1, nullptr) == 1 &&
+              cudaMemcpy(w_host, j.weights + (size_t)out_coord * taps, sizeof(float) * taps, cudaMemcpyDeviceToHost) == cudaSuccess &&
+              cudaMemcpy(inv_host, j.inv_wsum + out_coord, sizeof(float), cudaMemcpyDeviceToHost) == cudaSuccess;
+    cudaFree(d);
+    return ok ? 1 : -1;
+}
+
 int launch_weights(const WeightJob *jobs_dev, const WeightJob *jobs_host, int n, Stream s) {
     if (n <= 0) return 0;
     int max_out = 1;
@@ -448,19 +470,10 @@
 
 __constant__ float c_wint[5][32];
 __constant__ float c_winv[5];
-__constant__ float2 c_wpair[5][32];
 
 void set_int_weights(int S, const float *weights_dev, const float *inv_dev, int taps, Stream s) {
     cudaMemcpyToSymbolAsync(c_wint, weights_dev, sizeof(float) * taps, sizeof(float) * 32 * S, cudaMemcpyDeviceToDevice, (cudaStream_t)s);
     cudaMemcpyToSymbolAsync(c_winv, inv_dev, sizeof(float), sizeof(float) * S, cudaMemcpyDeviceToDevice, (cudaStream_t)s);
-    float *pair = nullptr;
-    cudaGetSymbolAddress((void **)&pair, c_wpair);
-    pair += 2 * 32 * S;
-    cudaMemsetAsync(pair, 0, sizeof(float2) * 32, (cudaStream_t)s);
-    cudaMemcpy2DAsync(pair, sizeof(float2), weights_dev, sizeof(float), sizeof(float), taps, cudaMemcpyDeviceToDevice, (cudaStream_t)s);
-    if (taps > S)
-        cudaMemcpy2DAsync(pair + 2 * S + 1, sizeof(float2), weights_dev, sizeof(float), sizeof(float), taps - S,
-                          cudaMemcpyDeviceToDevice, (cudaStream_t)s);
 }
 
 template <int S>
@@ -842,7 +855,8 @@
 }
 
 template <int S, int SRC>
-static bool launch_tma3(const FusedJob *jobs_dev, const FusedPiece *pieces, const int *piece_begin, int nblocks, cudaStream_t s) {
+static bool launch_tma3(const FusedJob *jobs_dev, const FusedPiece *pieces, const int *piece_begin, int nblocks, int full_range,
+                        cudaStream_t s) {
     static std::atomic<unsigned long long> done{0};
     int dev = 0;
     cudaGetDevice(&dev);
@@ -852,11 +866,12 @@
         done.fetch_or(bit, std::memory_order_release);
     }
     const int grid = (nblocks + tma_int::kGroups - 1) / tma_int::kGroups;
-    tma_int::k_resample_tma3<S, SRC><<<grid, dim3(32, tma::kWarps * tma_int::kGroups), tma_int::Cfg<S>::SMEM, s>>>(jobs_dev, pieces, piece_begin, nblocks);
+    tma_int::k_resample_tma3<S, SRC><<<grid, dim3(32, tma::kWarps * tma_int::kGroups), tma_int::Cfg<S>::SMEM, s>>>(jobs_dev, pieces, piece_begin, nblocks,
+                                                                                                            full_range);
     return check_launch("k_resample_tma3");
 }
 
-int launch_resample_fused(const FusedKernel &k, int src, const FusedJob *jobs_dev, const FusedPiece *pieces_dev,
+int launch_resample_fused(const FusedKernel &k, int src, int full_range, const FusedJob *jobs_dev, const FusedPiece *pieces_dev,
                           const int *piece_begin_dev, int nblocks, Stream s) {
     if (nblocks <= 0) return 0;
     cudaStream_t st = (cudaStream_t)s;
@@ -877,10 +892,10 @@
             }
             break;
         case FusedKernel::TMA_INT:
-            if (k.ratio == 4) ok = src == 1 ? launch_tma3<4, 1>(jobs_dev, pieces_dev, piece_begin_dev, nblocks, st)
-                                            : launch_tma3<4, 0>(jobs_dev, pieces_dev, piece_begin_dev, nblocks, st);
-            else ok = src == 1 ? launch_tma3<2, 1>(jobs_dev, pieces_dev, piece_begin_dev, nblocks, st)
-                               : launch_tma3<2, 0>(jobs_dev, pieces_dev, piece_begin_dev, nblocks, st);
+            if (k.ratio == 4) ok = src == 1 ? launch_tma3<4, 1>(jobs_dev, pieces_dev, piece_begin_dev, nblocks, full_range, st)
+                                            : launch_tma3<4, 0>(jobs_dev, pieces_dev, piece_begin_dev, nblocks, full_range, st);
+            else ok = src == 1 ? launch_tma3<2, 1>(jobs_dev, pieces_dev, piece_begin_dev, nblocks, full_range, st)
+                               : launch_tma3<2, 0>(jobs_dev, pieces_dev, piece_begin_dev, nblocks, full_range, st);
             break;
         default:
             switch (k.ratio) {
diff --git a/smelter_b200/csrc/kernels.h b/smelter_b200/csrc/kernels.h
--- a/smelter_b200/csrc/kernels.h
+++ b/smelter_b200/csrc/kernels.h
@@ -137,6 +137,9 @@
     bool operator==(const FusedKernel &o) const { return kind == o.kind && ratio == o.ratio && window == o.window && box == o.box; }
 };
 struct FusedShape { int strip_cols, groups_per_sm, row_gran; };
+inline int fused_launch_range(const FusedKernel &k, const FusedJob &j) {
+    return k.kind == FusedKernel::TMA_INT && j.src.full_range ? 1 : 0;
+}
 inline FusedShape fused_shape(const FusedKernel &k, const FusedJob &j) {
     switch (k.kind) {
         case FusedKernel::TMA_INT: return {k.ratio == 4 ? kTmaStripCols4 : kTmaStripCols2, 3, 2};
@@ -185,13 +188,14 @@
 
 int launch_convert_to_rgba(const Tex &src, uint8_t *dst, int dst_pitch, Stream s);
 int launch_weights(const WeightJob *jobs_dev, const WeightJob *jobs_host, int n_jobs, Stream s);
+int debug_weights(float scale, float offset, int out_coord, float *w_host, int cap, int *taps, float *inv_host);
 int launch_resample(const ResampleJob *jobs_dev, const ResampleJob *jobs_host, int n_jobs, Stream s);
 inline int fused_source_class(int tex_kind) {
     return tex_kind == TEX_YUV420 ? 0 : tex_kind == TEX_NV12 ? 1 : tex_kind == TEX_UYVY ? 2 : tex_kind == TEX_YUYV ? 3 : -1;
 }
 int launch_preprocess(const Tex &src, int mode, int rescale, uint8_t *out, int out_pitch, int out_w, int out_h, Stream s);
 int launch_text(const TextJob &job, Stream s);
-int launch_resample_fused(const FusedKernel &k, int src, const FusedJob *jobs_dev, const FusedPiece *pieces_dev,
+int launch_resample_fused(const FusedKernel &k, int src, int full_range, const FusedJob *jobs_dev, const FusedPiece *pieces_dev,
                           const int *piece_begin_dev, int nblocks, Stream s);
 void set_int_weights(int S, const float *weights_dev, const float *inv_dev, int taps, Stream s);
 int launch_composite(const CompositeJob *jobs_dev, const CompositeJob *jobs_host, const LayerDev *layers0_host, int n, Stream s);
diff --git a/smelter_b200/csrc/renderer.cpp b/smelter_b200/csrc/renderer.cpp
--- a/smelter_b200/csrc/renderer.cpp
+++ b/smelter_b200/csrc/renderer.cpp
@@ -1652,20 +1652,25 @@
     for (CompositeRec &c : plan_.composites)
         if (c.out_frame_off != SIZE_MAX) c.job.out0 = fb + c.out_frame_off;
 
-    struct FusedLaunch { dev::FusedKernel kernel; int src; size_t pieces_off, begin_off; int nblocks; };
+    struct FusedKey {
+        dev::FusedKernel kernel; int src, range;
+        bool operator==(const FusedKey &o) const { return kernel == o.kernel && src == o.src && range == o.range; }
+    };
+    auto key_of = [](const FusedRec &f) {
+        return FusedKey{f.kernel, dev::fused_source_class(f.job.src.kind), dev::fused_launch_range(f.kernel, f.job)};
+    };
+    struct FusedLaunch { FusedKey key; size_t pieces_off, begin_off; int nblocks; };
     std::vector<FusedLaunch> fused_launches;
     {
-        std::vector<std::pair<dev::FusedKernel, int>> kernels;
-        for (const FusedRec &f : plan_.fused) {
-            std::pair<dev::FusedKernel, int> v{f.kernel, dev::fused_source_class(f.job.src.kind)};
-            if (std::find(kernels.begin(), kernels.end(), v) == kernels.end()) kernels.push_back(v);
-        }
-        for (auto &v : kernels) {
+        std::vector<FusedKey> keys;
+        for (const FusedRec &f : plan_.fused)
+            if (std::find(keys.begin(), keys.end(), key_of(f)) == keys.end()) keys.push_back(key_of(f));
+        for (const FusedKey &v : keys) {
             std::vector<int> idx, widths, heights, cols;
             dev::FusedShape shape{};
             for (size_t ji = 0; ji < plan_.fused.size(); ji++) {
                 const FusedRec &f = plan_.fused[ji];
-                if (!(f.kernel == v.first) || dev::fused_source_class(f.job.src.kind) != v.second) continue;
+                if (!(key_of(f) == v)) continue;
                 shape = dev::fused_shape(f.kernel, f.job);
                 idx.push_back((int)ji); widths.push_back(f.job.dst_w); heights.push_back(f.job.dst_h); cols.push_back(shape.strip_cols);
             }
@@ -1684,7 +1689,7 @@
                                 pc.list.push_back((uint32_t)(t % (size_t)pc.job.map_w) | ((uint32_t)(t / (size_t)pc.job.map_w) << 16));
                             }
                 }
-            fused_launches.push_back({v.first, v.second, param_put(pieces.data(), sizeof(dev::FusedPiece) * pieces.size()),
+            fused_launches.push_back({v, param_put(pieces.data(), sizeof(dev::FusedPiece) * pieces.size()),
                                       param_put(begin.data(), sizeof(int) * begin.size()), (int)begin.size() - 1});
         }
     }
@@ -1751,7 +1756,7 @@
     new_weight_keys_.clear();
     weight_guard.armed = false;
     for (const FusedLaunch &fl : fused_launches) {
-        if (!launched(dev::launch_resample_fused(fl.kernel, fl.src, (const dev::FusedJob *)(pd + fj_off),
+        if (!launched(dev::launch_resample_fused(fl.key.kernel, fl.key.src, fl.key.range, (const dev::FusedJob *)(pd + fj_off),
                                                  (const dev::FusedPiece *)(pd + fl.pieces_off), (const int *)(pd + fl.begin_off),
                                                  fl.nblocks, stream_))) goto fail;
         prof_mark(SMR_KERNEL_RESAMPLE_FUSED);
@@ -2158,6 +2163,13 @@
     for (size_t i = 0; i < bg.size(); i++) begin[i] = bg[i];
     return SMR_OK;
 }
+smr_status smr_debug_weights(float scale, float offset, uint32_t out_coord, float *weights, uint32_t cap, uint32_t *taps, float *inv) {
+    if (!weights || !taps || !inv || out_coord > (1u << 24)) return SMR_ERR_INVALID_ARGUMENT;
+    int n = 0;
+    const int rc = smr::dev::debug_weights(scale, offset, (int)out_coord, weights, (int)cap, &n, inv);
+    *taps = (uint32_t)n;
+    return rc > 0 ? SMR_OK : rc == 0 ? SMR_ERR_BUFFER_TOO_SMALL : SMR_ERR_CUDA;
+}
 smr_status smr_preprocess_frame(smr_renderer *r, const smr_input_frame *f, uint32_t ow, uint32_t oh, void *rgba, uint32_t pitch,
                                 int32_t mem_kind) { SMR_GUARD(r->impl.preprocess_frame(f, ow, oh, rgba, pitch, mem_kind)) }
 smr_status smr_premultiply_rgba8(smr_renderer *r, const smr_input_frame *f, void *rgba, uint32_t pitch, int32_t mem_kind) {
diff --git a/smelter_b200/csrc/resample_tma.cuh b/smelter_b200/csrc/resample_tma.cuh
--- a/smelter_b200/csrc/resample_tma.cuh
+++ b/smelter_b200/csrc/resample_tma.cuh
@@ -20,6 +20,8 @@
 constexpr int kStashOff = kBarOff + 128;
 constexpr int kStashBytes = 1024;
 constexpr int kTailBytes = kStashOff + kStashBytes;
+constexpr int kLumaRep = 16;
+constexpr int kLumaTabBytes = 256 * kLumaRep * 4;
 
 template <int S> constexpr int kStripCols = S == 4 ? kTmaStripCols4 : kTmaStripCols2;
 template <int S> constexpr int kLead = S == 2 ? 1 : 0;
@@ -237,8 +239,25 @@
     }
 }
 
+constexpr uint32_t kDiv255C = 0x3b808081u, kDiv255Lo = 0xaf7efeffu;
+
+__device__ __forceinline__ float luma_of(float ny, float nk16, float rcp_y) {
+    const float y = __fmaf_rn(ny, __uint_as_float(kDiv255C), __fmul_rn(ny, __uint_as_float(kDiv255Lo)));
+    return __saturatef(__fmul_rn(__fadd_rn(y, nk16), rcp_y));
+}
+
+__device__ __forceinline__ void fill_luma_table(unsigned char *tail, float nk16, float rcp_y) {
+    float *s_y = reinterpret_cast<float *>(tail + kTailBytes);
+    const int btid = threadIdx.y * 32 + threadIdx.x, bn = blockDim.x * blockDim.y;
+    for (int i = btid; i < 256 * kLumaRep; i += bn) s_y[i] = luma_of((float)(i / kLumaRep), nk16, rcp_y);
+}
+__device__ __forceinline__ uint32_t luma_base(unsigned char *tail) {
+    return smem_u32(tail + kTailBytes) - (0x4B000000u << 6) + 4u * (threadIdx.x % kLumaRep);
+}
+
+template <bool YTAB = false>
 __device__ __forceinline__ void convert_pair(const uint32_t (&yw)[2], const uint32_t (&v)[6], int p, float nk16, float rcp_y,
-                                             float rcp_c, float2 &qr, float2 &qg, float2 &qb) {
+                                             float rcp_c, float2 &qr, float2 &qg, float2 &qb, uint32_t ybase = 0) {
     const uint32_t ne = v[p] + 3u * v[p + 1], no = 3u * v[p + 1] + v[p + 2];
     const float m23 = -8388608.0f;
     float2 nu = add2(make_float2(__uint_as_float(__byte_perm(ne, 0x4B000000u, 0x7610)),
@@ -246,15 +265,22 @@
     float2 nv = add2(make_float2(__uint_as_float(__byte_perm(ne, 0x4B000000u, 0x7632)),
                                  __uint_as_float(__byte_perm(no, 0x4B000000u, 0x7632))), splat(m23));
     const uint32_t ywd = yw[p >> 1];
-    float2 ny = add2(make_float2(__uint_as_float(__byte_perm(ywd, 0x4B000000u, (p & 1) ? 0x7642 : 0x7640)),
-                                 __uint_as_float(__byte_perm(ywd, 0x4B000000u, (p & 1) ? 0x7643 : 0x7641))), splat(m23));
-    const float c1 = __uint_as_float(0x3b808081u), lo1 = __uint_as_float(0xaf7efeffu);
+    const uint32_t by0 = __byte_perm(ywd, 0x4B000000u, (p & 1) ? 0x7642 : 0x7640);
+    const uint32_t by1 = __byte_perm(ywd, 0x4B000000u, (p & 1) ? 0x7643 : 0x7641);
+    const float c1 = __uint_as_float(kDiv255C), lo1 = __uint_as_float(kDiv255Lo);
     const float c16 = __uint_as_float(0x39808081u), lo16 = __uint_as_float(0xad7efeffu);
-    float2 y = fma2(ny, splat(c1), mul2(ny, splat(lo1)));
+    float2 y;
+    if (YTAB) {
+        y = make_float2(lds_tab((by0 << 6) + ybase), lds_tab((by1 << 6) + ybase));
+    } else {
+        const float2 ny = add2(make_float2(__uint_as_float(by0), __uint_as_float(by1)), splat(m23));
+        y = fma2(ny, splat(c1), mul2(ny, splat(lo1)));
+    }
     float2 u = fma2(nu, splat(c16), mul2(nu, splat(lo16)));
     float2 w = fma2(nv, splat(c16), mul2(nv, splat(lo16)));
-    y = add2(y, splat(nk16)); u = add2(u, splat(nk16)); w = add2(w, splat(nk16));
-    y = make_float2(__saturatef(y.x * rcp_y), __saturatef(y.y * rcp_y));
+    if (!YTAB) y = add2(y, splat(nk16));
+    u = add2(u, splat(nk16)); w = add2(w, splat(nk16));
+    if (!YTAB) y = make_float2(__saturatef(y.x * rcp_y), __saturatef(y.y * rcp_y));
     u = make_float2(__saturatef(u.x * rcp_c), __saturatef(u.y * rcp_c));
     w = make_float2(__saturatef(w.x * rcp_c), __saturatef(w.y * rcp_c));
     const float2 um = add2(u, splat(-0.5f)), vm = add2(w, splat(-0.5f));
@@ -267,12 +293,13 @@
     qb = add2_after_mul(mul2(bb, splat(255.0f)), splat(kMagicRound));
 }
 
+template <bool YTAB = false>
 __device__ __forceinline__ void convert_run(const uint32_t (&yw)[2], const uint32_t (&v)[6], float nk16, float rcp_y, float rcp_c,
-                                            uint32_t kaddr, float2 (&prg)[8], float (&pb)[8]) {
+                                            uint32_t kaddr, float2 (&prg)[8], float (&pb)[8], uint32_t ybase = 0) {
 #pragma unroll
     for (int p = 0; p < 4; p++) {
         float2 qr, qg, qb;
-        convert_pair(yw, v, p, nk16, rcp_y, rcp_c, qr, qg, qb);
+        convert_pair<YTAB>(yw, v, p, nk16, rcp_y, rcp_c, qr, qg, qb, ybase);
         prg[2 * p] = make_float2(lds_tab((__float_as_uint(qr.x) << 7) + kaddr), lds_tab((__float_as_uint(qg.x) << 7) + kaddr));
         prg[2 * p + 1] = make_float2(lds_tab((__float_as_uint(qr.y) << 7) + kaddr), lds_tab((__float_as_uint(qg.y) << 7) + kaddr));
         pb[2 * p] = lds_tab((__float_as_uint(qb.x) << 7) + kaddr);
diff --git a/smelter_b200/csrc/resample_tma3.cuh b/smelter_b200/csrc/resample_tma3.cuh
--- a/smelter_b200/csrc/resample_tma3.cuh
+++ b/smelter_b200/csrc/resample_tma3.cuh
@@ -26,12 +26,12 @@
     static constexpr int RROW_BYTES = 32 * 3 * OUT * 4;
     static constexpr int RING_BYTES = RROWS * RROW_BYTES;
     static constexpr int GROUP_BYTES = kStageBytes + RING_BYTES;
-    static constexpr int SMEM = kGroups * GROUP_BYTES + kTailBytes;
+    static constexpr int SMEM = kGroups * GROUP_BYTES + kTailBytes + kLumaTabBytes;
 };
 
 template <int S, int SRC>
 __global__ void __launch_bounds__(32 * kWarps * kGroups, 1) k_resample_tma3(const FusedJob *jobs, const FusedPiece *pieces, const int *piece_begin,
-                                                                            int n_virtual_blocks) {
+                                                                            int n_virtual_blocks, int full_range) {
     using K = Cfg<S>;
     using It = ChunkIter<S, 1>;
     constexpr int P = K::P, OUT = K::OUT, TAPS = K::TAPS, A = K::A, NST = K::NST;
@@ -44,7 +44,9 @@
     const uint32_t stage0 = smem_u32(smem);
     float *ring = reinterpret_cast<float *>(smem + kStageBytes);
     const uint32_t bar0 = smem_u32(tail + kBarOff) + 16u * (uint32_t)grp;
-    const uint32_t kaddr = setup_block<kGroups>(tail, [] {});
+    const float nk16 = full_range ? 0.0f : -K16, rcp_y = full_range ? 1.0f : RCP_Y, rcp_c = full_range ? 1.0f : RCP_C;
+    const uint32_t kaddr = setup_block<kGroups>(tail, [&] { fill_luma_table(tail, nk16, rcp_y); });
+    const uint32_t ybase = luma_base(tail);
     const int vb = blockIdx.x * kGroups + grp;
     if (vb >= n_virtual_blocks) return;
 
@@ -67,8 +69,6 @@
         const bool cur_tma = cur.nrows > 0;
         const FusedJob &J = jobs[cur.job];
         const int W = J.src.width, H = J.src.height, chei = H >> 1;
-        const bool full_range = J.src.full_range != 0;
-        const float nk16 = full_range ? 0.0f : -K16, rcp_y = full_range ? 1.0f : RCP_Y, rcp_c = full_range ? 1.0f : RCP_C;
         const uint32_t sb = stage0;
         if (cur_tma) {
             mbar_wait(bar0, nchunk & 1u);
@@ -79,7 +79,7 @@
                 fetch_row<NV12>(sb, lw, r, cur.r0, chei, yw, v);
                 float2 prg[P];
                 float pb[P];
-                convert_run(yw, v, nk16, rcp_y, rcp_c, kaddr, prg, pb);
+                convert_run<true>(yw, v, nk16, rcp_y, rcp_c, kaddr, prg, pb, ybase);
                 float2 arg[OUT];
                 float ab[OUT];
 #pragma unroll
@@ -91,19 +91,9 @@
 #pragma unroll
                         for (int j = 0; j < OUT; j++) {
                             const int t = P * s + i - A - S * j;
-                            if (t >= 0 && t < TAPS) arg[j] = fma2(prg[i], splat(c_wint[S][t]), arg[j]);
-                        }
-#pragma unroll
-                        for (int j = 0; j < OUT; j += 2) {
-                            const int t0 = P * s + i - A - S * j, t1 = t0 - S;
-                            const bool a0 = t0 >= 0 && t0 < TAPS, a1 = t1 >= 0 && t1 < TAPS;
-                            if (a0 && a1) {
-                                const float2 d = fma2(splat(pb[i]), c_wpair[S][a0 ? t0 : 0], make_float2(ab[j], ab[j + 1]));
-                                ab[j] = d.x; ab[j + 1] = d.y;
-                            } else if (a0) {
-                                ab[j] = fmaf(pb[i], c_wint[S][a0 ? t0 : 0], ab[j]);
-                            } else if (a1) {
-                                ab[j + 1] = fmaf(pb[i], c_wint[S][a1 ? t1 : 0], ab[j + 1]);
+                            if (t >= 0 && t < TAPS) {
+                                arg[j] = fma2(prg[i], splat(int_weight<S>(t)), arg[j]);
+                                ab[j] = __fmaf_rn(pb[i], int_weight<S>(t), ab[j]);
                             }
                         }
                     }
@@ -118,7 +108,7 @@
                     }
                 }
                 {
-                    const float inv = c_winv[S];
+                    constexpr float inv = int_inv<S>();
                     float *dst = ring + (size_t)(r % K::RROWS) * (K::RROW_BYTES / 4) + lane * 3 * OUT;
 #pragma unroll
                     for (int j = 0; j < OUT; j += 2) {
@@ -194,11 +184,11 @@
                             for (int k = 0; k < 3 * OUT / 2; k++) v[k] = *reinterpret_cast<const float2 *>(p + 2 * k);
                             if (u < TAPS) {
 #pragma unroll
-                                for (int k = 0; k < 3 * OUT / 2; k++) aa[k] = fma2(v[k], splat(c_wint[S][u < TAPS ? u : 0]), aa[k]);
+                                for (int k = 0; k < 3 * OUT / 2; k++) aa[k] = fma2(v[k], splat(int_weight<S>(u < TAPS ? u : 0)), aa[k]);
                             }
                             if (u >= S) {
 #pragma unroll
-                                for (int k = 0; k < 3 * OUT / 2; k++) bb2[k] = fma2(v[k], splat(c_wint[S][u >= S ? u - S : 0]), bb2[k]);
+                                for (int k = 0; k < 3 * OUT / 2; k++) bb2[k] = fma2(v[k], splat(int_weight<S>(u >= S ? u - S : 0)), bb2[k]);
                             }
                         }
                         uint32_t pa[OUT], pb[OUT];
```

Result: faster. 1806 (median of 6 runs) (+5.3%).
